# lucabaldesi/srsRAN

Hardware: AMD Instinct MI355X
Metric: PDSCH decoded Mbps + code-blocks/sec, 20 MHz TM4 QAM256, 1/2/4/8 GPU (higher is better)
Workload: dtype fp32+int16; 1 GPU; srslte_ue_dl chain from time-domain I/Q: 2048 subframes/GPU/batch, 20 MHz (100 PRB), TM4 2x2 spatial multiplexing, 2 codewords QAM256 TBS 97896 (C=16, K=6144), MMSE+CSI, max 10 half-its with CRC early stop, 40 dB crossed 2x2 channel, every subframe distinct (GPU eNodeB generator, keyed by global subframe index); 3 PHY worker threads (own ue_dl / stream / softbuffers each) decode alternate batches,; subframes_per_gpu_batch=2048, code_blocks_per_gpu_batch=65536, workers_per_gpu=3, parallelism=dp1

## Files before the change

### include/srsran_amd/dlsch.h

```cpp
#ifndef SRSRAN_AMD_DLSCH_H
#define SRSRAN_AMD_DLSCH_H

#include <stddef.h>
#include <stdint.h>

#ifdef __cplusplus
extern "C" {
#endif

typedef struct mi355_softbuffer_pool mi355_softbuffer_pool_t;

int  mi355_softbuffer_pool_create(mi355_softbuffer_pool_t** p, uint32_t nof_sb, uint32_t max_cb, int device);
void mi355_softbuffer_pool_destroy(mi355_softbuffer_pool_t* p);
int mi355_softbuffer_reset(mi355_softbuffer_pool_t* p, uint32_t sb, void* stream);
int mi355_softbuffer_reset_tbs(mi355_softbuffer_pool_t* p, uint32_t sb, uint32_t tbs, void* stream);
int mi355_softbuffer_reset_cb(mi355_softbuffer_pool_t* p, uint32_t sb, uint32_t nof_cb, void* stream);
int mi355_softbuffer_reset_all(mi355_softbuffer_pool_t* p, void* stream);
int mi355_softbuffer_reset_range(mi355_softbuffer_pool_t* p, uint32_t first, uint32_t n, void* stream);
int mi355_softbuffer_reset_tbs_batch(mi355_softbuffer_pool_t* p, const uint32_t* sbs, const uint32_t* tbs, uint32_t n,
                                     void* stream);
int mi355_softbuffer_pool_buffer(mi355_softbuffer_pool_t* p, int16_t** buf, uint32_t* stride, uint32_t* max_cb);
int mi355_softbuffer_pool_materialize(mi355_softbuffer_pool_t* p, uint32_t first, uint32_t n, void* stream);

int mi355_softbuffer_pool_data(mi355_softbuffer_pool_t* p, uint8_t** data, uint32_t* stride, uint32_t* nof_sb);
int mi355_softbuffer_get_cb_crc(mi355_softbuffer_pool_t* p, uint32_t sb, uint8_t* cb_crc, void* stream);
int mi355_softbuffer_get_cb_crc_async(mi355_softbuffer_pool_t* p, uint32_t sb, uint8_t* cb_crc, void* stream);
int mi355_softbuffer_cb_crc_dev(mi355_softbuffer_pool_t* p, uint32_t sb, const uint8_t** d_cb_crc);
typedef struct {
  uint32_t tbs;
  uint32_t nof_e_bits;
  uint32_t Qm;
  uint32_t rv;
  uint32_t softbuffer;
  uint64_t e_offset;
  uint64_t data_offset;
} mi355_dlsch_tb_t;

typedef struct mi355_dlsch mi355_dlsch_t;

int  mi355_dlsch_create(mi355_dlsch_t** q, int device);
void mi355_dlsch_destroy(mi355_dlsch_t* q);
int mi355_dlsch_set_max_iterations(mi355_dlsch_t* q, uint32_t max_iterations);
void mi355_dlsch_set_profiling(mi355_dlsch_t* q, int enable);

int mi355_dlsch_set_latency_path(int max_cbs);
int mi355_dlsch_latency_profile(int enable, uint64_t* out);
int  mi355_dlsch_kernel_stats(mi355_dlsch_t* q, double* ms, uint32_t* launches);

int mi355_dlsch_decode_dev(mi355_dlsch_t*           q,
                           mi355_softbuffer_pool_t* pool,
                           const int16_t*           d_e_bits,
                           const mi355_dlsch_tb_t*  tbs,
                           uint32_t                 ntb,
                           uint8_t*                 d_data,
                           int32_t*                 ret,
                           float*                   avg_iterations,
                           void*                    stream);

int mi355_dlsch_decode8_dev(mi355_dlsch_t* q, mi355_softbuffer_pool_t* pool, const int8_t* d_e_bits,
                            const mi355_dlsch_tb_t* tbs, uint32_t ntb, uint8_t* d_data, int32_t* ret,
                            float* avg_iterations, void* stream);

#ifdef __cplusplus
}
#endif
#endif
```

### srsran_amd/csrc/dlsch_internal.h

```cpp
#pragma once
#include <hip/hip_runtime.h>
#include <stdint.h>

#define SB_STRIDE 18600
#define SB_DATA 768
#define SB_CONV8 10240
#define SB_ROWMASK 18544
#define SB_ROWMASK_WORDS 12

namespace mi355 {

struct CbDesc {
  uint32_t tb, cb, C;
  uint32_t rlen;
  uint32_t rp, n_e;
  uint32_t rv;
  uint32_t slot;
  uint64_t e_off;
  uint64_t data_off;
};

struct TbDesc {
  uint32_t tbs, C, C1, K1, K2, slot0, invalid;
  uint32_t Qm, nof_e_bits, rv;
  uint32_t cb_base[2];
  uint64_t e_off;
  uint64_t data_off;
  const uint32_t* crc_scale;
};

struct CrcTable {
  uint32_t t[256];
  uint32_t pw[24];
  uint32_t poly;
};

CrcTable make_crc_table(uint32_t poly);

constexpr uint16_t RM_NONE = 0xffff;

struct DlschRmArgs {
  const CbDesc*   desc;
  int             ncb;
  uint32_t        N;
  uint32_t        buflen;
  const uint16_t* inv[4];
  const int16_t*  e;
  int16_t*        sb;
  size_t          sb_stride;
  const uint8_t*  sb_crc;
  uint8_t*        fresh;
  uint32_t        fold2;
  int             sparse;
};

struct DlschRm8Args {
  const CbDesc*   desc;
  int             ncb;
  uint32_t        N, buflen;
  const uint16_t* inv[4];
  const int8_t*   e;
  int8_t*         sb;
  size_t          sb_stride;
  const uint8_t*  sb_crc;
  const uint8_t*  fresh;
  int16_t*        conv;
};

struct DlschCheckArgs {
  const CbDesc*  desc;
  int            ncb;
  uint32_t       K, h, max_its;
  const uint8_t* dec;
  size_t         dec_stride;
  uint8_t*       data;
  uint8_t*       done;
  const uint32_t* remaining;
  uint32_t*      next;
  uint32_t*      its;
  uint8_t*        sb_crc;
  const CrcTable* crc24a;
  const CrcTable* crc24b;
  const uint32_t* scale;
};

struct DlschTbArgs {
  const TbDesc* tb;
  int           ntb;
  uint8_t*      data;
  uint8_t*      sb_crc;
  uint8_t*      sb_data;
  int32_t*        ret;
  const CrcTable* crc24a;
  CbDesc*   desc;
  uint32_t* slot;
  uint32_t* its;
  uint8_t*  done;
  uint32_t* running;
  float*    avg;
};

struct DlschResetArgs {
  uint8_t* fresh;
  uint8_t* sb_crc;
  size_t   slot0, ncb;
  size_t   ncrc;
};

hipError_t dlsch_launch_rm(const DlschRmArgs& a, hipStream_t s);
hipError_t dlsch_launch_reset_list(const uint2* list, uint32_t n, uint32_t max_cb, uint8_t* fresh, uint8_t* cb_crc,
                                   hipStream_t s);
hipError_t dlsch_launch_check(const DlschCheckArgs& a, hipStream_t s);
hipError_t dlsch_launch_prologue(const DlschTbArgs& a, hipStream_t s);
hipError_t dlsch_launch_epilogue(const DlschTbArgs& a, hipStream_t s);
hipError_t dlsch_launch_reset(const DlschResetArgs& a, hipStream_t s);

hipError_t dlsch_launch_rm8(const DlschRm8Args& a, hipStream_t s);
hipError_t dlsch_launch_materialize(int16_t* sb, size_t stride, const uint8_t* fresh, size_t slot0, uint32_t nslots,
                                    hipStream_t s);

}
```

### srsran_amd/csrc/dlsch_kernels.hip

```cpp
#include <hip/hip_runtime.h>
#include <stdint.h>

#include "crc_device.h"
#include "dlsch_internal.h"
#include "rm_image.h"

namespace mi355 {

constexpr uint32_t RM_LDS     = 3 * 6144 + 12;
constexpr uint32_t RM_THREADS = 512;
constexpr int      RM_Q       = (3 * (6144 + 32) + 12 + 8 * RM_THREADS - 1) / (8 * RM_THREADS);
constexpr int      RM_EQ      = (RM_LDS + 8 * RM_THREADS - 1) / (8 * RM_THREADS);
#ifndef RM_CPB_N
#define RM_CPB_N 1
#endif
constexpr int      RM_CPB     = RM_CPB_N;

__device__ __forceinline__ uint32_t add_pairs(uint32_t a, uint32_t b)
{
  return ((a + b) & 0xffffu) | (((a >> 16) + (b >> 16)) << 16);
}

__device__ __forceinline__ uint4 ld_quad(const uint32_t* p, uint32_t q, uint32_t lim, bool al16, uint32_t fill)
{
  const uint32_t i = 4 * q;
  if (al16 && i + 3 < lim) return *(const uint4*)(p + i);
  return make_uint4(i < lim ? p[i] : fill, i + 1 < lim ? p[i + 1] : fill, i + 2 < lim ? p[i + 2] : fill,
                    i + 3 < lim ? p[i + 3] : fill);
}

__device__ __forceinline__ uint32_t ld_llr_pair(const int16_t* e, uint32_t r2, bool al4)
{
  return al4 ? ((const uint32_t*)e)[r2] : ((uint32_t)(uint16_t)e[2 * r2] | ((uint32_t)(uint16_t)e[2 * r2 + 1] << 16));
}

__global__ __launch_bounds__(RM_THREADS) void dlsch_rm_rx(DlschRmArgs a)
{
  extern __shared__ __attribute__((aligned(16))) uint32_t acc32[];
  const uint16_t* acc   = (const uint16_t*)acc32;
  __shared__ uint32_t obm[2 * SB_ROWMASK_WORDS], nbm[2 * SB_ROWMASK_WORDS];
  const uint32_t  N     = a.N, tid = threadIdx.x, N2 = min(N / 2, a.fold2), K = (N - 12) / 3;
  const uint32_t  pairs = a.buflen / 2;
  uint4           iv[RM_Q];
  uint32_t        iv_rv = 0xffffffffu;
  for (int c = 0; c < RM_CPB; c++) {
    const int b = blockIdx.x * RM_CPB + c;
    if (b >= a.ncb) break;
    const CbDesc& d = a.desc[b];
    if (a.sb_crc[d.slot]) continue;
    const uint32_t n_e = d.n_e, first2 = min(n_e, N) / 2;
    const bool     fresh = a.fresh[d.slot] != 0;
    uint32_t*      sb    = (uint32_t*)(a.sb + (size_t)d.slot * a.sb_stride);
    const bool     sb16  = ((uintptr_t)sb & 15) == 0;
    const int16_t* e     = a.e + d.e_off + d.rp;
    const bool     e4    = ((uintptr_t)e & 3) == 0, e16 = ((uintptr_t)e & 15) == 0;
    if (d.rv != iv_rv) {
      const uint32_t* inv32 = (const uint32_t*)a.inv[d.rv];
#pragma unroll
      for (int k = 0; k < RM_Q; k++) iv[k] = ld_quad(inv32, tid + k * RM_THREADS, pairs, true, 0xffffffffu);
      iv_rv = d.rv;
    }
    uint4 old[RM_Q], ev[RM_EQ];
#pragma unroll
    for (int k = 0; k < RM_EQ; k++) {
      const uint32_t q = tid + k * RM_THREADS;
      if (e16) {
        ev[k] = ld_quad((const uint32_t*)e, q, first2, true, 0u);
      } else {
        ev[k] = make_uint4(4 * q < first2 ? ld_llr_pair(e, 4 * q, e4) : 0u,
                           4 * q + 1 < first2 ? ld_llr_pair(e, 4 * q + 1, e4) : 0u,
                           4 * q + 2 < first2 ? ld_llr_pair(e, 4 * q + 2, e4) : 0u,
                           4 * q + 3 < first2 ? ld_llr_pair(e, 4 * q + 3, e4) : 0u);
      }
    }
#pragma unroll
    for (int k = 0; k < RM_Q; k++)
      old[k] = fresh ? make_uint4(0u, 0u, 0u, 0u) : ld_quad(sb, tid + k * RM_THREADS, pairs, sb16, 0u);
    __syncthreads();
    if (tid < 2 * SB_ROWMASK_WORDS) {
      uint32_t*      bmg = rm_rowmask_of(a.sb + (size_t)d.slot * a.sb_stride);
      const uint32_t nw  = rm_rowmask_word(a.inv[d.rv], a.buflen, fresh ? min(n_e, N) : 0x10000u, tid);
      obm[tid]           = fresh ? 0xffffffffu : bmg[tid];
      nbm[tid]           = nw;
      bmg[tid]           = nw;
    } else if (tid == 2 * SB_ROWMASK_WORDS) {
      rm_rowmask_of(a.sb + (size_t)d.slot * a.sb_stride)[tid] = K;
    }
#pragma unroll
    for (int k = 0; k < RM_EQ; k++) {
      const uint32_t i = 4 * (tid + k * RM_THREADS);
      if (i + 3 < N2) {
        *(uint4*)&acc32[img_u32(i)] = ev[k];
      } else {
        if (i < N2) acc32[img_u32(i)] = ev[k].x;
        if (i + 1 < N2) acc32[img_u32(i + 1)] = ev[k].y;
        if (i + 2 < N2) acc32[img_u32(i + 2)] = ev[k].z;
      }
    }
    for (uint32_t base = N; base < n_e; base += N) {
      __syncthreads();
      const uint32_t lim2 = min(N, n_e - base) / 2;
      for (uint32_t r2 = tid; r2 < lim2; r2 += RM_THREADS)
        acc32[img_u32(r2)] = add_pairs(acc32[img_u32(r2)], ld_llr_pair(e + base, r2, e4));
    }
    __syncthreads();
#pragma unroll
    for (int k = 0; k < RM_Q; k++) {
      const uint32_t q = tid + k * RM_THREADS, i = 4 * q;
      if (i >= pairs) continue;
      if (fresh && a.sparse && !rm_quad_defined(nbm, 2 * i, K)) continue;
      const bool     odef = fresh || rm_quad_defined(obm, 2 * i, K);
      const uint32_t w[4] = {iv[k].x, iv[k].y, iv[k].z, iv[k].w};
      const uint32_t o[4] = {odef ? old[k].x : 0u, odef ? old[k].y : 0u, odef ? old[k].z : 0u, odef ? old[k].w : 0u};
      uint32_t       v[4];
      bool           any = fresh || !odef;
#pragma unroll
      for (int cc = 0; cc < 4; cc++) {
        const uint32_t r0 = w[cc] & 0xffffu, r1 = w[cc] >> 16;
        const bool     h0 = r0 != RM_NONE && r0 < n_e, h1 = r1 != RM_NONE && r1 < n_e;
        any |= h0 || h1;
        v[cc] = add_pairs(o[cc], (h0 ? acc[img_i16(r0)] : 0u) | ((h1 ? acc[img_i16(r1)] : 0u) << 16));
      }
      if (!any) continue;
      if (sb16 && i + 3 < pairs) {
        typedef uint32_t u4v __attribute__((ext_vector_type(4)));
        __builtin_nontemporal_store((u4v){v[0], v[1], v[2], v[3]}, (u4v*)(sb + i));
      } else {
#pragma unroll
        for (int cc = 0; cc < 4; cc++)
          if (i + cc < pairs) sb[i + cc] = v[cc];
      }
    }
  }
}

__global__ __launch_bounds__(256) void dlsch_rm_consume(const CbDesc* desc, int ncb, uint8_t* fresh, const uint8_t* sb_crc)
{
  const int b = blockIdx.x * blockDim.x + threadIdx.x;
  if (b < ncb && !sb_crc[desc[b].slot]) fresh[desc[b].slot] = 0;
}


__global__ __launch_bounds__(1024) void dlsch_cb_check(DlschCheckArgs a)
{
  __shared__ uint32_t unfinished;
  __shared__ uint32_t tl[2][4][256];
  if (threadIdx.x == 0) unfinished = 0;
  if (a.ncb && *a.remaining == 0) return;
  const uint32_t ti = threadIdx.x & 255, tt = (threadIdx.x >> 8) & 1;
  if (threadIdx.x < 512) tl[tt][0][ti] = (tt ? a.crc24b : a.crc24a)->t[ti];
  __syncthreads();
#pragma unroll
  for (int k = 1; k < 4; k++) {
    if (threadIdx.x < 512) tl[tt][k][ti] = crc24_step_table(tl[tt][k - 1][ti], tl[tt][0]);
    __syncthreads();
  }
  const int b    = (blockIdx.x * blockDim.x + threadIdx.x) >> 6;
  const int lane = threadIdx.x & 63;
  if (b < a.ncb && *a.remaining != 0 && !a.done[b]) {
    const CbDesc&  d   = a.desc[b];
    const uint8_t* dec = a.dec + (size_t)b * a.dec_stride;
    const uint32_t crc = wave_crc24_scaled4(dec, a.K / 8, tl[d.C > 1 ? 1 : 0], d.C > 1 ? a.crc24b->poly : a.crc24a->poly,
                                            a.scale + (d.C > 1 ? 64 : 0));
    const bool     ok  = crc == 0;
    const bool     fin = ok || a.h + 1 == a.max_its;
    if (!fin) {
      if (lane == 0) unfinished = 1;
    } else {
      uint8_t*       dst = a.data + d.data_off + (size_t)d.cb * d.rlen / 8;
      const uint32_t nb  = (d.cb + 1 == d.C) ? a.K / 8 : d.rlen / 8;
      for (uint32_t i = lane; i < nb; i += 64) dst[i] = dec[i];
      if (lane == 0) {
        a.its[b] = a.h + 1;
        if (ok) {
          a.done[b]        = 1;
          a.sb_crc[d.slot] = 1;
        } else {
          a.done[b] = 2;
        }
      }
    }
  }
  __syncthreads();
  if (threadIdx.x == 0 && unfinished) flag_set(a.next);
}


__global__ __launch_bounds__(256) void dlsch_tb_prologue(DlschTbArgs a)
{
  __shared__ uint32_t todo_any;
  if (threadIdx.x == 0) todo_any = 0;
  __syncthreads();
  const int t    = (blockIdx.x * blockDim.x + threadIdx.x) >> 6;
  const int lane = threadIdx.x & 63;
  if (t < a.ntb && a.tb[t].C != 0) {
    const TbDesc&  tb    = a.tb[t];
    const uint32_t Gp    = tb.nof_e_bits / tb.Qm, gamma = Gp % tb.C, n_e = tb.Qm * (Gp / tb.C);
    uint8_t*       data  = a.data + tb.data_off;
    bool           todo  = false;
    if (lane < 3) data[tb.tbs / 8 + lane] = 0;
    for (uint32_t c = lane; c < tb.C; c += 64) {
      const uint32_t K    = c < tb.C1 ? tb.K1 : tb.K2;
      const uint32_t rlen = tb.C == 1 ? K : K - 24;
      uint32_t       rp = c * n_e, n_e2 = n_e;
      if (c > tb.C - gamma) {
        n_e2 = n_e + tb.Qm;
        rp   = (tb.C - gamma) * n_e + (c - (tb.C - gamma)) * n_e2;
      }
      const uint32_t g    = c < tb.C1 ? tb.cb_base[0] + c : tb.cb_base[1] + (c - tb.C1);
      const uint32_t slot = tb.slot0 + c;
      a.desc[g]           = CbDesc{(uint32_t)t, c, tb.C, rlen, rp, n_e2, tb.rv, slot, tb.e_off, tb.data_off};
      a.slot[g]           = slot;
      a.its[g]            = 0;
      const bool prior    = a.sb_crc[slot] != 0;
      a.done[g]           = prior ? 3 : 0;
      todo |= !prior;
    }
    if (todo) todo_any = 1;
    for (uint32_t c = 0; c < tb.C; c++) {
      const uint32_t slot = tb.slot0 + c;
      if (!a.sb_crc[slot]) continue;
      const uint32_t K    = c < tb.C1 ? tb.K1 : tb.K2;
      const uint32_t rlen = tb.C == 1 ? K : K - 24;
      const uint32_t o    = c * rlen / 8;
      for (uint32_t i = lane; i < rlen / 8; i += 64) data[o + i] = a.sb_data[(size_t)slot * 768 + i];
    }
  }
  __syncthreads();
  if (threadIdx.x == 0 && todo_any) flag_set(a.running);
}

__global__ __launch_bounds__(256) void dlsch_tb_epilogue(DlschTbArgs a)
{
  const int t   = blockIdx.x;
  const int tid = threadIdx.x;
  if (t >= a.ntb) return;
  __shared__ uint32_t t4[4][256];
  t4[0][tid] = a.crc24a->t[tid];
  __syncthreads();
  const TbDesc& tb = a.tb[t];
  if (tb.crc_scale) {
#pragma unroll
    for (int k = 1; k < 4; k++) {
      t4[k][tid] = crc24_step_table(t4[k - 1][tid], t4[0]);
      __syncthreads();
    }
  }
  if (tid == 0) {
    double sum = 0.0;
    for (uint32_t c = 0; c < tb.C; c++) sum += a.its[c < tb.C1 ? tb.cb_base[0] + c : tb.cb_base[1] + (c - tb.C1)];
    a.avg[t] = tb.C ? (float)(sum / tb.C) : 0.f;
  }
  if (tb.C == 0) {
    if (tid == 0) a.ret[t] = tb.invalid ? -2 : 0;
    return;
  }
  bool ok = true;
  for (uint32_t c = 0; c < tb.C; c++) ok &= a.sb_crc[tb.slot0 + c] != 0;
  uint8_t* data = a.data + tb.data_off;
  if (!ok) {
    for (uint32_t c = 0; c < tb.C; c++) {
      const uint32_t slot = tb.slot0 + c;
      if (!a.sb_crc[slot]) continue;
      const uint32_t K    = c < tb.C1 ? tb.K1 : tb.K2;
      const uint32_t rlen = tb.C == 1 ? K : K - 24;
      for (uint32_t i = tid; i < rlen / 8; i += blockDim.x) a.sb_data[(size_t)slot * 768 + i] = data[c * rlen / 8 + i];
    }
    if (tid == 0) a.ret[t] = -1;
    return;
  }
  const uint32_t par_rx = tb.crc_scale ? block_crc24_scaled4(data, tb.tbs / 8, t4, a.crc24a->poly, tb.crc_scale)
                                        : block_crc24(data, tb.tbs / 8, t4[0], *a.crc24a);
  if (tid == 0) {
    const uint32_t par_tx = ((uint32_t)data[tb.tbs / 8] << 16) | ((uint32_t)data[tb.tbs / 8 + 1] << 8) |
                            (uint32_t)data[tb.tbs / 8 + 2];
    a.ret[t] = (par_rx == par_tx && par_rx) ? 0 : -1;
  }
}

__global__ __launch_bounds__(256) void dlsch_sb_reset(DlschResetArgs a)
{
  const size_t g = (size_t)blockIdx.x * blockDim.x + threadIdx.x;
  if (g < a.ncb) a.fresh[a.slot0 + g] = 1;
  if (g < (a.ncrc ? a.ncrc : a.ncb)) a.sb_crc[a.slot0 + g] = 0;
}

__global__ __launch_bounds__(256) void dlsch_sb_reset_list(const uint2* list, uint32_t n, uint32_t max_cb, uint8_t* fresh,
                                                           uint8_t* cb_crc)
{
  const size_t g = (size_t)blockIdx.x * blockDim.x + threadIdx.x;
  if (g >= (size_t)n * max_cb) return;
  const uint2    e  = list[g / max_cb];
  const uint32_t cb = (uint32_t)(g % max_cb);
  const size_t   k  = (size_t)e.x * max_cb + cb;
  if (cb < e.y) fresh[k] = 1;
  cb_crc[k] = 0;
}

hipError_t dlsch_launch_reset_list(const uint2* list, uint32_t n, uint32_t max_cb, uint8_t* fresh, uint8_t* cb_crc,
                                   hipStream_t s)
{
  const size_t t = (size_t)n * max_cb;
  if (!t) return hipSuccess;
  hipLaunchKernelGGL(dlsch_sb_reset_list, dim3((unsigned)((t + 255) / 256)), dim3(256), 0, s, list, n, max_cb, fresh,
                     cb_crc);
  return hipGetLastError();
}

__global__ __launch_bounds__(256) void dlsch_rm8_rx(DlschRm8Args a)
{
  const size_t t = (size_t)blockIdx.x * blockDim.x + threadIdx.x;
  if (t >= (size_t)a.ncb * a.buflen) return;
  const uint32_t b = (uint32_t)(t / a.buflen), j = (uint32_t)(t % a.buflen);
  const CbDesc&  d = a.desc[b];
  if (a.sb_crc[d.slot]) return;
  int8_t*        o = a.sb + (size_t)d.slot * a.sb_stride;
  const uint16_t r = a.inv[d.rv][j];
  int            v = a.fresh[d.slot] ? 0 : o[j];
  if (r != RM_NONE) {
    const int8_t* e = a.e + d.e_off + d.rp;
    for (uint32_t i = r; i < d.n_e; i += a.N) v += e[i];
  }
  o[j] = (int8_t)v;
  if (a.conv) a.conv[(size_t)d.slot * (a.sb_stride / 2) + j] = (int16_t)(int8_t)v;
  if (j < 2 * SB_ROWMASK_WORDS) ((uint32_t*)(a.sb + (size_t)d.slot * a.sb_stride + 2 * SB_ROWMASK))[j] = 0xffffffffu;
}

__global__ __launch_bounds__(256) void sb_materialize(int16_t* sb, size_t stride, const uint8_t* fresh, size_t slot0)
{
  const size_t slot = slot0 + blockIdx.x;
  if (fresh[slot]) return;
  int16_t*        b  = sb + slot * stride;
  uint32_t*       bm = rm_rowmask_of(b);
  const uint32_t  K  = bm[2 * SB_ROWMASK_WORDS];
  __shared__ uint32_t w[2 * SB_ROWMASK_WORDS];
  if (threadIdx.x < 2 * SB_ROWMASK_WORDS) w[threadIdx.x] = bm[threadIdx.x];
  __syncthreads();
  if (K % 16 == 0 && K > 800 && K <= 6144) {
    const uint32_t L = K / 16;
    for (uint32_t r = threadIdx.x; r < 2 * L; r += blockDim.x) {
      const uint32_t s = r / L, j = r % L;
      if ((w[s * SB_ROWMASK_WORDS + (j >> 5)] >> (j & 31)) & 1u) continue;
      uint4* row = (uint4*)(b + (s + 1) * (K + 32) + 16 * j);
      row[0] = row[1] = make_uint4(0u, 0u, 0u, 0u);
    }
  }
  __syncthreads();
  if (threadIdx.x < 2 * SB_ROWMASK_WORDS) bm[threadIdx.x] = 0xffffffffu;
}

hipError_t dlsch_launch_materialize(int16_t* sb, size_t stride, const uint8_t* fresh, size_t slot0, uint32_t nslots,
                                    hipStream_t s)
{
  if (!nslots) return hipSuccess;
  hipLaunchKernelGGL(sb_materialize, dim3(nslots), dim3(256), 0, s, sb, stride, fresh, slot0);
  return hipGetLastError();
}

hipError_t dlsch_launch_rm8(const DlschRm8Args& a, hipStream_t s)
{
  if (a.ncb <= 0) return hipSuccess;
  const size_t n = (size_t)a.ncb * a.buflen;
  hipLaunchKernelGGL(dlsch_rm8_rx, dim3((unsigned)((n + 255) / 256)), dim3(256), 0, s, a);
  hipLaunchKernelGGL(dlsch_rm_consume, dim3((unsigned)((a.ncb + 255) / 256)), dim3(256), 0, s, a.desc, a.ncb,
                     (uint8_t*)a.fresh, a.sb_crc);
  return hipGetLastError();
}

hipError_t dlsch_launch_rm(const DlschRmArgs& a, hipStream_t s)
{
  if (a.ncb <= 0) return hipSuccess;
  if (a.N > RM_LDS) return hipErrorInvalidValue;
  DlschRmArgs b = a;
  b.fold2       = (a.fold2 && a.fold2 < a.N / 2) ? a.fold2 : a.N / 2;
  const size_t lds = (size_t)img_elems(2 * ((b.fold2 + 3) & ~3u)) * 2;
  hipLaunchKernelGGL(dlsch_rm_rx, dim3((unsigned)((a.ncb + RM_CPB - 1) / RM_CPB)), dim3(RM_THREADS), lds, s, b);
  hipLaunchKernelGGL(dlsch_rm_consume, dim3((unsigned)((a.ncb + 255) / 256)), dim3(256), 0, s, a.desc, a.ncb, a.fresh,
                     a.sb_crc);
  return hipGetLastError();
}

hipError_t dlsch_launch_check(const DlschCheckArgs& a, hipStream_t s)
{
  hipLaunchKernelGGL(dlsch_cb_check, dim3((unsigned)((a.ncb + 15) / 16)), dim3(1024), 0, s, a);
  return hipGetLastError();
}

hipError_t dlsch_launch_prologue(const DlschTbArgs& a, hipStream_t s)
{
  hipLaunchKernelGGL(dlsch_tb_prologue, dim3((unsigned)((a.ntb + 3) / 4)), dim3(256), 0, s, a);
  return hipGetLastError();
}

hipError_t dlsch_launch_epilogue(const DlschTbArgs& a, hipStream_t s)
{
  if (a.ntb <= 0) return hipSuccess;
  hipLaunchKernelGGL(dlsch_tb_epilogue, dim3((unsigned)a.ntb), dim3(256), 0, s, a);
  return hipGetLastError();
}

hipError_t dlsch_launch_reset(const DlschResetArgs& a, hipStream_t s)
{
  const size_t n = a.ncb > a.ncrc ? a.ncb : a.ncrc;
  if (!n) return hipSuccess;
  hipLaunchKernelGGL(dlsch_sb_reset, dim3((unsigned)((n + 255) / 256)), dim3(256), 0, s, a);
  return hipGetLastError();
}

}
```

### srsran_amd/csrc/dlsch_runtime.cpp

```cpp
#include <hip/hip_runtime.h>

#include <algorithm>
#include <chrono>
#include <stdlib.h>
#include <map>
#include <mutex>
#include <stdio.h>
#include <string.h>
#include <vector>

#include "../../include/srsran_amd/dlsch.h"
#include "../../include/srsran_amd/tdec.h"
#include "dlsch_internal.h"
#include "host_staging.h"
#include "tdec8_internal.h"
#include "rm_image.h"
#include "rm_tables.h"
#include "runtime_internal.h"
#include "tdec_internal.h"

using namespace mi355;

#define CHECK_HIP(x)                                                                                                   \
  do {                                                                                                                 \
    hipError_t e_ = (x);                                                                                               \
    if (e_ != hipSuccess) {                                                                                            \
      fprintf(stderr, "[srsran_amd] %s:%d %s: %s\n", __FILE__, __LINE__, #x, hipGetErrorString(e_));                 \
      return MI355_ERROR;                                                                                              \
    }                                                                                                                  \
  } while (0)

struct mi355_softbuffer_pool {
  int      device = 0;
  uint32_t nof_sb = 0, max_cb = 0;
  int16_t* buf    = nullptr;
  uint8_t* cb_crc = nullptr;
  uint8_t* data   = nullptr;
  uint8_t* fresh  = nullptr;
  uint2*     d_list[2]   = {nullptr, nullptr};
  uint32_t   list_cap[2] = {0, 0};
  hipEvent_t ev_list[2]  = {nullptr, nullptr};
  bool       ev_armed[2] = {false, false};
  uint32_t   lpar        = 0;
  mi355::HostStaging st_list;
};

CrcTable mi355::make_crc_table(uint32_t poly)
{
  CrcTable t{};
  t.poly = poly;
  for (uint32_t i = 0; i < 256; i++) {
    uint32_t c = i << 16;
    for (int j = 0; j < 8; j++) c = (c & 0x800000) ? ((c << 1) ^ poly) & 0xffffff : (c << 1) & 0xffffff;
    t.t[i] = c;
  }
  auto mulmod = [&](uint32_t a, uint32_t b) {
    uint32_t r = 0;
    for (int i = 23; i >= 0; i--) {
      r <<= 1;
      if (r & 0x1000000u) r ^= poly;
      if ((b >> i) & 1u) r ^= a;
    }
    return r & 0xffffffu;
  };
  uint32_t p = 1u << 8;
  for (int i = 0; i < 24; i++) {
    t.pw[i] = p;
    p       = mulmod(p, p);
  }
  return t;
}

struct mi355_dlsch {
  int                                    device = 0;
  hipStream_t                            own    = nullptr;
  uint32_t                               max_its = 10;
  std::map<uint32_t, mi355_tdec_batch_t*> dec;
  std::map<uint64_t, uint16_t*>          rm;
  std::map<uint64_t, uint16_t*>          rm8;
  struct Compact {
    uint16_t* d;
    uint32_t  nq, qoff;
  };
  std::map<uint64_t, Compact>            rmc;
  std::map<uint32_t, mi355_tdec8_t*>     dec8;
  std::map<uint32_t, uint32_t*>          scales;
  std::map<uint32_t, uint32_t*>          tb_scales;
  CrcTable*                              crc = nullptr;
  char*      scratch[2]     = {nullptr, nullptr};
  size_t     scratch_cap[2] = {0, 0};
  std::vector<void*> retired;
  hipEvent_t done_ev[2]     = {nullptr, nullptr};
  bool       done_armed[2]  = {false, false};
  uint32_t   par            = 0;
  std::mutex mu;
  bool       prof = false;
  HostStaging stage;
  HostStaging back;
  std::atomic<uint32_t> spec_mask{1u << 1};
};

static std::atomic<int> g_lat_cbs{-1};
static std::atomic<uint64_t*> g_lat_prof{nullptr};
static uint64_t*              g_lat_prof_mem = nullptr;
static std::mutex             g_lat_prof_mu;
static int lat_cbs_now()
{
  int v = g_lat_cbs.load();
  if (v < 0) {
    v = getenv("MI355_DLSCH_LAT_CBS") ? atoi(getenv("MI355_DLSCH_LAT_CBS")) : 256;
    g_lat_cbs.store(v);
  }
  return v;
}

extern "C" int mi355_dlsch_latency_profile(int enable, uint64_t* out)
{
  std::lock_guard<std::mutex> lk(g_lat_prof_mu);
  if (out && g_lat_prof.load()) {
    if (hipDeviceSynchronize() != hipSuccess) return MI355_ERROR;
    if (hipMemcpy(out, g_lat_prof_mem, 11 * 8, hipMemcpyDeviceToHost) != hipSuccess) return MI355_ERROR;
  }
  if (enable) {
    if (!g_lat_prof_mem && hipMalloc(&g_lat_prof_mem, 11 * 8) != hipSuccess) return MI355_ERROR;
    if (hipMemset(g_lat_prof_mem, 0, 11 * 8) != hipSuccess || hipDeviceSynchronize() != hipSuccess) return MI355_ERROR;
    g_lat_prof.store(g_lat_prof_mem);
  } else {
    g_lat_prof.store(nullptr);
  }
  return MI355_SUCCESS;
}

extern "C" int mi355_dlsch_set_latency_path(int max_cbs)
{
  const int old = lat_cbs_now();
  if (max_cbs >= 0) g_lat_cbs.store(max_cbs);
  return old;
}

static bool spec_enabled()
{
  static const bool on = !getenv("MI355_TDEC_SPEC") || atoi(getenv("MI355_TDEC_SPEC")) != 0;
  return on;
}

static bool no_rowmask()
{
  static const bool off = getenv("MI355_NO_ROWMASK") && atoi(getenv("MI355_NO_ROWMASK")) != 0;
  return off;
}

static bool lat_waves4()
{
  static const bool on = getenv("MI355_LAT_WAVES") && atoi(getenv("MI355_LAT_WAVES")) == 4;
  return on;
}
static bool lat_owaves()
{
  static const bool on = !getenv("MI355_LAT_OWAVES") || atoi(getenv("MI355_LAT_OWAVES")) != 0;
  return on;
}

bool mi355::rm_sparse_writes()
{
  static const bool on = !getenv("MI355_RM_SPARSE") || atoi(getenv("MI355_RM_SPARSE")) != 0;
  return on && !no_rowmask();
}

static uint32_t rm_buflen(uint32_t K) { return tdec_subblocks(K) ? 3 * (K + 32) + 12 : 3 * K + 12; }

static int rm_table(mi355_dlsch_t* q, uint32_t K, uint32_t rv, const uint16_t** out)
{
  const uint64_t key = ((uint64_t)K << 2) | rv;
  auto           it  = q->rm.find(key);
  if (it == q->rm.end()) {
    const std::vector<uint16_t> t = rm_rx_table(K, rv);
    const uint32_t              buflen = rm_buflen(K);
    std::vector<uint16_t>       inv(rm_rowmin_off(buflen) + rm_rowmin_len(), 0);
    std::fill(inv.begin(), inv.begin() + buflen + 1, (uint16_t)RM_NONE);
    for (size_t r = 0; r < t.size(); r++) inv[t[r]] = (uint16_t)r;
    if (tdec_subblocks(K) == 16) {
      uint16_t*      rmin = inv.data() + rm_rowmin_off(buflen);
      const uint32_t L    = K / 16;
      for (uint32_t s = 0; s < 2; s++)
        for (uint32_t j = 0; j < L; j++) {
          uint16_t m = RM_NONE;
          for (uint32_t w = 0; w < 16; w++) m = std::min(m, inv[(s + 1) * (K + 32) + j * 16 + w]);
          rmin[s * 32 * SB_ROWMASK_WORDS + j] = m;
        }
    }
    uint16_t* d = nullptr;
    CHECK_HIP(hipMalloc(&d, inv.size() * 2));
    CHECK_HIP(hipMemcpy(d, inv.data(), inv.size() * 2, hipMemcpyHostToDevice));
    it = q->rm.emplace(key, d).first;
  }
  *out = it->second;
  return MI355_SUCCESS;
}

static int rm8_table(mi355_dlsch_t* q, uint32_t K, uint32_t rv, const uint16_t** out)
{
  const uint64_t key = ((uint64_t)K << 2) | rv;
  auto           it  = q->rm8.find(key);
  if (it == q->rm8.end()) {
    const uint32_t              nsb = tdec_subblocks_8bit(K);
    const std::vector<uint16_t> t   = rm_rx_table_nsb(K, rv, nsb);
    std::vector<uint16_t>       inv((nsb ? 3 * (K + 32) + 12 : 3 * K + 12) + 1, RM_NONE);
    for (size_t r = 0; r < t.size(); r++) inv[t[r]] = (uint16_t)r;
    uint16_t* d = nullptr;
    CHECK_HIP(hipMalloc(&d, inv.size() * 2));
    CHECK_HIP(hipMemcpy(d, inv.data(), inv.size() * 2, hipMemcpyHostToDevice));
    it = q->rm8.emplace(key, d).first;
  }
  *out = it->second;
  return MI355_SUCCESS;
}

static uint32_t gf2_mulmod24_host(uint32_t a, uint32_t b, uint32_t poly)
{
  uint32_t r = 0;
  for (int i = 23; i >= 0; i--) {
    r <<= 1;
    if (r & 0x1000000u) r ^= poly;
    if ((b >> i) & 1u) r ^= a;
  }
  return r & 0xffffffu;
}

static int crc_scales(mi355_dlsch_t* q, uint32_t K, const uint32_t** out)
{
  auto it = q->scales.find(K);
  if (it == q->scales.end()) {
    std::vector<uint32_t> t(144, 0u);
    const uint32_t        nbytes = K / 8, chunk = (nbytes + 63) / 64;
    const uint32_t        polys[2] = {0x1864CFB, 0x1800063};
    auto                  xpow = [](uint32_t after, uint32_t poly) {
      uint32_t sc = 1, x8 = 1u << 8;
      for (; after; after >>= 1) {
        if (after & 1) sc = gf2_mulmod24_host(sc, x8, poly);
        x8 = gf2_mulmod24_host(x8, x8, poly);
      }
      return sc;
    };
    const uint32_t nl = std::max(1u, mi355_tdec_autoimp_get_subblocks(K) / 2), cl = nbytes / nl;
    for (int pi = 0; pi < 2; pi++) {
      for (uint32_t lane = 0; lane < 64; lane++) {
        const uint32_t b0 = std::min(nbytes, lane * chunk), b1 = std::min(nbytes, b0 + chunk);
        t[pi * 64 + lane] = xpow(nbytes - b1, polys[pi]);
      }
      for (uint32_t l = 0; l < nl && l < 8; l++) t[128 + 8 * pi + l] = xpow(nbytes - (l + 1) * cl, polys[pi]);
    }
    uint32_t* d = nullptr;
    CHECK_HIP(hipMalloc(&d, t.size() * 4));
    CHECK_HIP(hipMemcpy(d, t.data(), t.size() * 4, hipMemcpyHostToDevice));
    it = q->scales.emplace(K, d).first;
  }
  *out = it->second;
  return MI355_SUCCESS;
}

static int tb_crc_scales(mi355_dlsch_t* q, uint32_t nbytes, const uint32_t** out)
{
  auto it = q->tb_scales.find(nbytes);
  if (it == q->tb_scales.end()) {
    std::vector<uint32_t> t(256);
    const uint32_t        chunk = ((nbytes + 255) / 256 + 3) / 4 * 4, poly = 0x1864CFB;
    for (uint32_t tid = 0; tid < 256; tid++) {
      const uint32_t b0 = std::min(nbytes, tid * chunk), b1 = std::min(nbytes, b0 + chunk);
      uint32_t       sc = 1, x8 = 1u << 8;
      for (uint32_t after = nbytes - b1; after; after >>= 1) {
        if (after & 1) sc = gf2_mulmod24_host(sc, x8, poly);
        x8 = gf2_mulmod24_host(x8, x8, poly);
      }
      t[tid] = sc;
    }
    uint32_t* d = nullptr;
    CHECK_HIP(hipMalloc(&d, t.size() * 4));
    CHECK_HIP(hipMemcpy(d, t.data(), t.size() * 4, hipMemcpyHostToDevice));
    it = q->tb_scales.emplace(nbytes, d).first;
  }
  *out = it->second;
  return MI355_SUCCESS;
}

static int scratch(mi355_dlsch_t* q, uint32_t k, size_t bytes, char** p)
{
  if (bytes > q->scratch_cap[k]) {
    if (q->scratch[k]) {
      q->retired.push_back(q->scratch[k]);
      q->scratch[k]    = nullptr;
      q->done_armed[k] = false;
    }
    size_t cap = bytes + bytes / 4 + 4096;
    CHECK_HIP(hipMalloc(&q->scratch[k], cap));
    q->scratch_cap[k] = cap;
  }
  *p = q->scratch[k];
  return MI355_SUCCESS;
}

extern "C" {

int mi355_softbuffer_pool_create(mi355_softbuffer_pool_t** p, uint32_t nof_sb, uint32_t max_cb, int device)
{
  if (!p || !nof_sb || !max_cb) return MI355_ERROR_INVALID_INPUTS;
  CHECK_HIP(hipSetDevice(device));
  auto*        s  = new mi355_softbuffer_pool;
  const size_t nc = (size_t)nof_sb * max_cb;
  s->device       = device;
  s->nof_sb       = nof_sb;
  s->max_cb       = max_cb;
  if (hipMalloc(&s->buf, nc * SB_STRIDE * 2) != hipSuccess || hipMalloc(&s->cb_crc, nc) != hipSuccess ||
      hipMalloc(&s->data, nc * SB_DATA) != hipSuccess || hipMalloc(&s->fresh, nc) != hipSuccess) {
    mi355_softbuffer_pool_destroy(s);
    return MI355_ERROR;
  }
  (void)hipMemset(s->fresh, 1, nc);
  (void)hipMemset(s->cb_crc, 0, nc);
  (void)hipMemset(s->data, 0, nc * SB_DATA);
  (void)hipDeviceSynchronize();
  *p = s;
  return MI355_SUCCESS;
}

void mi355_softbuffer_pool_destroy(mi355_softbuffer_pool_t* p)
{
  if (!p) return;
  (void)hipFree(p->buf);
  (void)hipFree(p->cb_crc);
  (void)hipFree(p->data);
  (void)hipFree(p->fresh);
  for (int k = 0; k < 2; k++) {
    if (p->ev_armed[k]) (void)hipEventSynchronize(p->ev_list[k]);
    if (p->ev_list[k]) (void)hipEventDestroy(p->ev_list[k]);
    (void)hipFree(p->d_list[k]);
  }
  delete p;
}

int mi355_softbuffer_reset_cb(mi355_softbuffer_pool_t* p, uint32_t sb, uint32_t nof_cb, void* stream)
{
  if (!p || sb >= p->nof_sb) return MI355_ERROR_INVALID_INPUTS;
  CHECK_HIP(hipSetDevice(p->device));
  hipStream_t    s  = (hipStream_t)stream;
  const uint32_t nc = std::min(nof_cb, p->max_cb);
  DlschResetArgs a{p->fresh, p->cb_crc, (size_t)sb * p->max_cb, nc, p->max_cb};
  CHECK_HIP(dlsch_launch_reset(a, s));
  if (!s) CHECK_HIP(hipStreamSynchronize(nullptr));
  return MI355_SUCCESS;
}

int mi355_softbuffer_reset(mi355_softbuffer_pool_t* p, uint32_t sb, void* stream)
{
  return mi355_softbuffer_reset_cb(p, sb, p ? p->max_cb : 0, stream);
}

int mi355_softbuffer_reset_tbs(mi355_softbuffer_pool_t* p, uint32_t sb, uint32_t tbs, void* stream)
{
  return mi355_softbuffer_reset_cb(p, sb, (tbs + 24) / (6144 - 24) + 1, stream);
}

int mi355_softbuffer_reset_tbs_batch(mi355_softbuffer_pool_t* p, const uint32_t* sbs, const uint32_t* tbs, uint32_t n,
                                     void* stream)
{
  if (!p || (n && (!sbs || !tbs))) return MI355_ERROR_INVALID_INPUTS;
  if (!n) return MI355_SUCCESS;
  CHECK_HIP(hipSetDevice(p->device));
  hipStream_t    s = (hipStream_t)stream;
  const uint32_t k = p->lpar;
  p->lpar ^= 1u;
  if (n > p->list_cap[k]) {
    if (p->d_list[k]) {
      if (p->ev_armed[k]) CHECK_HIP(hipEventSynchronize(p->ev_list[k]));
      CHECK_HIP(hipFree(p->d_list[k]));
      p->ev_armed[k] = false;
    }
    p->list_cap[k] = n + n / 2 + 64;
    CHECK_HIP(hipMalloc(&p->d_list[k], p->list_cap[k] * sizeof(uint2)));
  }
  if (!p->ev_list[k]) CHECK_HIP(hipEventCreateWithFlags(&p->ev_list[k], hipEventDisableTiming));
  CHECK_HIP(p->st_list.reserve(n * sizeof(uint2)));
  auto* l = (uint2*)p->st_list.slot(n * sizeof(uint2));
  for (uint32_t i = 0; i < n; i++) {
    if (sbs[i] >= p->nof_sb) return MI355_ERROR_INVALID_INPUTS;
    l[i] = make_uint2(sbs[i], std::min((tbs[i] + 24) / (6144 - 24) + 1, p->max_cb));
  }
  CHECK_HIP(p->st_list.upload(p->d_list[k], s, false, p->ev_armed[k] ? p->ev_list[k] : nullptr));
  CHECK_HIP(dlsch_launch_reset_list(p->d_list[k], n, p->max_cb, p->fresh, p->cb_crc, s));
  CHECK_HIP(hipEventRecord(p->ev_list[k], s));
  p->ev_armed[k] = true;
  if (!s) CHECK_HIP(hipStreamSynchronize(nullptr));
  return MI355_SUCCESS;
}

int mi355_softbuffer_reset_all(mi355_softbuffer_pool_t* p, void* stream)
{
  if (!p) return MI355_ERROR_INVALID_INPUTS;
  for (uint32_t i = 0; i < p->nof_sb; i++) {
    int r = mi355_softbuffer_reset(p, i, stream);
    if (r) return r;
  }
  return MI355_SUCCESS;
}

int mi355_softbuffer_reset_range(mi355_softbuffer_pool_t* p, uint32_t first, uint32_t n, void* stream)
{
  if (!p || first + n > p->nof_sb) return MI355_ERROR_INVALID_INPUTS;
  if (!n) return MI355_SUCCESS;
  CHECK_HIP(hipSetDevice(p->device));
  DlschResetArgs a{p->fresh, p->cb_crc, (size_t)first * p->max_cb, (size_t)n * p->max_cb, 0};
  CHECK_HIP(dlsch_launch_reset(a, (hipStream_t)stream));
  if (!stream) CHECK_HIP(hipStreamSynchronize(nullptr));
  return MI355_SUCCESS;
}

int mi355_softbuffer_pool_buffer(mi355_softbuffer_pool_t* p, int16_t** buf, uint32_t* stride, uint32_t* max_cb)
{
  if (!p) return MI355_ERROR_INVALID_INPUTS;
  if (buf) *buf = p->buf;
  if (stride) *stride = SB_STRIDE;
  if (max_cb) *max_cb = p->max_cb;
  return MI355_SUCCESS;
}

int mi355_softbuffer_pool_materialize(mi355_softbuffer_pool_t* p, uint32_t first, uint32_t n, void* stream)
{
  if (!p || first > p->nof_sb || n > p->nof_sb - first) return MI355_ERROR_INVALID_INPUTS;
  CHECK_HIP(hipSetDevice(p->device));
  CHECK_HIP(dlsch_launch_materialize(p->buf, SB_STRIDE, p->fresh, (size_t)first * p->max_cb, n * p->max_cb,
                                     (hipStream_t)stream));
  if (!stream) CHECK_HIP(hipStreamSynchronize(nullptr));
  return MI355_SUCCESS;
}

int mi355_softbuffer_pool_data(mi355_softbuffer_pool_t* p, uint8_t** data, uint32_t* stride, uint32_t* nof_sb)
{
  if (!p) return MI355_ERROR_INVALID_INPUTS;
  if (data) *data = p->data;
  if (stride) *stride = SB_DATA;
  if (nof_sb) *nof_sb = p->nof_sb;
  return MI355_SUCCESS;
}

int mi355_softbuffer_get_cb_crc(mi355_softbuffer_pool_t* p, uint32_t sb, uint8_t* cb_crc, void* stream)
{
  if (!p || !cb_crc || sb >= p->nof_sb) return MI355_ERROR_INVALID_INPUTS;
  CHECK_HIP(hipSetDevice(p->device));
  hipStream_t s = (hipStream_t)stream;
  CHECK_HIP(hipMemcpyAsync(cb_crc, p->cb_crc + (size_t)sb * p->max_cb, p->max_cb, hipMemcpyDeviceToHost, s));
  CHECK_HIP(wait_stream(s));
  return MI355_SUCCESS;
}

int mi355_softbuffer_get_cb_crc_async(mi355_softbuffer_pool_t* p, uint32_t sb, uint8_t* cb_crc, void* stream)
{
  if (!p || !cb_crc || sb >= p->nof_sb) return MI355_ERROR_INVALID_INPUTS;
  CHECK_HIP(hipSetDevice(p->device));
  CHECK_HIP(hipMemcpyAsync(cb_crc, p->cb_crc + (size_t)sb * p->max_cb, p->max_cb, hipMemcpyDeviceToHost,
                           (hipStream_t)stream));
  return MI355_SUCCESS;
}

int mi355_softbuffer_cb_crc_dev(mi355_softbuffer_pool_t* p, uint32_t sb, const uint8_t** d_cb_crc)
{
  if (!p || !d_cb_crc || sb >= p->nof_sb) return MI355_ERROR_INVALID_INPUTS;
  *d_cb_crc = p->cb_crc + (size_t)sb * p->max_cb;
  return MI355_SUCCESS;
}

int mi355_dlsch_create(mi355_dlsch_t** q, int device)
{
  if (!q) return MI355_ERROR_INVALID_INPUTS;
  CHECK_HIP(hipSetDevice(device));
  auto* d   = new mi355_dlsch;
  d->device = device;
  if (hipStreamCreateWithFlags(&d->own, hipStreamNonBlocking) != hipSuccess ||
      hipMalloc(&d->crc, 2 * sizeof(CrcTable)) != hipSuccess) {
    mi355_dlsch_destroy(d);
    return MI355_ERROR;
  }
  const CrcTable t[2] = {make_crc_table(0x1864CFB), make_crc_table(0x1800063)};
  if (hipMemcpy(d->crc, t, sizeof(t), hipMemcpyHostToDevice) != hipSuccess) {
    mi355_dlsch_destroy(d);
    return MI355_ERROR;
  }
  *q = d;
  return MI355_SUCCESS;
}

void mi355_dlsch_destroy(mi355_dlsch_t* q)
{
  if (!q) return;
  (void)hipSetDevice(q->device);
  (void)hipDeviceSynchronize();
  for (auto& kv : q->dec) mi355_tdec_batch_destroy(kv.second);
  for (auto& kv : q->rm) (void)hipFree(kv.second);
  for (auto& kv : q->rm8) (void)hipFree(kv.second);
  for (auto& kv : q->rmc) (void)hipFree(kv.second.d);
  for (auto& kv : q->dec8) mi355_tdec8_destroy(kv.second);
  for (auto& kv : q->scales) (void)hipFree(kv.second);
  for (auto& kv : q->tb_scales) (void)hipFree(kv.second);
  (void)hipFree(q->crc);
  for (void* r : q->retired) (void)hipFree(r);
  for (int k = 0; k < 2; k++) {
    (void)hipFree(q->scratch[k]);
    if (q->done_ev[k]) (void)hipEventDestroy(q->done_ev[k]);
  }
  if (q->own) (void)hipStreamDestroy(q->own);
  delete q;
}

int mi355_dlsch_set_max_iterations(mi355_dlsch_t* q, uint32_t max_iterations)
{
  if (!q || max_iterations == 0) return MI355_ERROR_INVALID_INPUTS;
  q->max_its = max_iterations;
  return MI355_SUCCESS;
}

void mi355_dlsch_set_profiling(mi355_dlsch_t* q, int enable)
{
  if (!q) return;
  q->prof = enable != 0;
  for (auto& kv : q->dec) mi355_tdec_batch_set_profiling(kv.second, enable);
}

int mi355_dlsch_kernel_stats(mi355_dlsch_t* q, double* ms, uint32_t* launches)
{
  if (!q) return MI355_ERROR_INVALID_INPUTS;
  double   tot = 0;
  uint32_t n   = 0;
  for (auto& kv : q->dec) {
    double   m = 0;
    uint32_t l = 0;
    int      r = mi355_tdec_batch_kernel_stats(kv.second, &m, &l);
    if (r) return r;
    tot += m;
    n += l;
  }
  if (ms) *ms = tot;
  if (launches) *launches = n;
  return MI355_SUCCESS;
}

int mi355_dlsch_decode_dev(mi355_dlsch_t*           q,
                           mi355_softbuffer_pool_t* pool,
                           const int16_t*           d_e_bits,
                           const mi355_dlsch_tb_t*  tbs,
                           uint32_t                 ntb,
                           uint8_t*                 d_data,
                           int32_t*                 ret,
                           float*                   avg_iterations,
                           void*                    stream)
{
  return mi355::dlsch_decode_dev_hook(q, pool, d_e_bits, tbs, ntb, d_data, ret, avg_iterations, stream, mi355::WaitHook{});
}

int mi355_dlsch_decode8_dev(mi355_dlsch_t* q, mi355_softbuffer_pool_t* pool, const int8_t* d_e_bits,
                            const mi355_dlsch_tb_t* tbs, uint32_t ntb, uint8_t* d_data, int32_t* ret,
                            float* avg_iterations, void* stream)
{
  return mi355::dlsch_decode_dev_hook(q, pool, d_e_bits, tbs, ntb, d_data, ret, avg_iterations, stream,
                                      mi355::WaitHook{}, true);
}

}

mi355::DlschPending::~DlschPending()
{
  if (armed && ev) (void)hipEventSynchronize(ev);
  if (ev) (void)hipEventDestroy(ev);
  if (host) (void)hipHostFree(host);
}

static uint32_t spec_policy(const float* avg, const int32_t* ret, uint32_t ntb, uint32_t max_its)
{
  uint32_t mask = 0;
  for (uint32_t h = 0; h + 1 < max_its; h++) {
    uint32_t run = 0, fail = 0;
    for (uint32_t t = 0; t < ntb; t++) {
      if (ret[t] != MI355_SUCCESS && ret[t] != MI355_ERROR) continue;
      const float a = avg[t];
      if (!(a > 0.f)) continue;
      run += a > (float)h + 0.5f;
      fail += a > (float)h + 1.5f;
    }
    if (run && fail * 10 <= run) mask |= 1u << h;
  }
  return mask;
}

int mi355::DlschPending::collect()
{
  if (!armed) return MI355_SUCCESS;
  armed = false;
  CHECK_HIP(wait_event(ev));
  memcpy(ret, host, ntb * 4);
  for (uint32_t t = 0; t < ntb; t++) {
    if (invalid[t]) ret[t] = MI355_ERROR_INVALID_INPUTS;
  }
  if (avg) memcpy(avg, host + avg_off, ntb * 4);
  if (spec_mask) spec_mask->store(spec_policy((const float*)(host + avg_off), ret, ntb, max_its));
  return MI355_SUCCESS;
}

int mi355::dlsch_rm_inv(mi355_dlsch_t* q, uint32_t K, uint32_t rv, const uint16_t** out)
{
  if (!q || rv > 3) return MI355_ERROR_INVALID_INPUTS;
  std::lock_guard<std::mutex> lock(q->mu);
  CHECK_HIP(hipSetDevice(q->device));
  return rm_table(q, K, rv, out);
}

uint32_t mi355::dlsch_rm_buflen(uint32_t K) { return rm_buflen(K); }

int mi355::dlsch_rm_compact(mi355_dlsch_t* q, uint32_t K, uint32_t rv, uint32_t E, const uint16_t** tab, uint32_t* nq,
                            uint32_t* qoff)
{
  if (!q || rv > 3 || E == 0 || E > 3 * K + 12) return MI355_ERROR_INVALID_INPUTS;
  std::lock_guard<std::mutex> lock(q->mu);
  CHECK_HIP(hipSetDevice(q->device));
  const uint64_t key = ((((uint64_t)K << 2) | rv) << 16) | E;
  auto           it  = q->rmc.find(key);
  if (it == q->rmc.end()) {
    const std::vector<uint16_t> t      = rm_rx_table(K, rv);
    const uint32_t              buflen = rm_buflen(K), nquad = (buflen + 7) / 8;
    std::vector<uint16_t>       inv(buflen, (uint16_t)RM_NONE);
    for (size_t r = 0; r < t.size(); r++) inv[t[r]] = (uint16_t)r;
    auto defined = [&](uint32_t pos) {
      if (tdec_subblocks(K) != 16) return true;
      const uint32_t sl = K + 32, s = pos / sl;
      if (s == 0 || s > 2) return true;
      const uint32_t j = (pos - s * sl) >> 4;
      if (j >= 32 * SB_ROWMASK_WORDS || j >= K / 16) return true;
      for (uint32_t w = 0; w < 16; w++)
        if (inv[s * sl + j * 16 + w] < E) return true;
      return false;
    };
    std::vector<uint16_t> rank(nquad, 0xffff);
    std::vector<uint32_t> qlist;
    for (uint32_t qd = 0; qd < nquad; qd++) {
      if (!defined(8 * qd)) continue;
      uint32_t m = 0;
      for (uint32_t p = 0; p < 8 && 8 * qd + p < buflen; p++) m |= (uint32_t)(inv[8 * qd + p] < E) << p;
      rank[qd] = (uint16_t)qlist.size();
      qlist.push_back(qd | m << 16);
    }
    const uint32_t        off = (E + 7) / 8 * 8;
    std::vector<uint16_t> all(off + 2 * qlist.size() + 8, 0);
    for (uint32_t r = 0; r < E; r++) {
      const uint32_t pos = t[r];
      if (rank[pos / 8] == 0xffff) return MI355_ERROR;
      all[r] = (uint16_t)(8 * rank[pos / 8] + pos % 8);
    }
    memcpy(all.data() + off, qlist.data(), qlist.size() * 4);
    uint16_t* d = nullptr;
    CHECK_HIP(hipMalloc(&d, all.size() * 2));
    CHECK_HIP(hipMemcpy(d, all.data(), all.size() * 2, hipMemcpyHostToDevice));
    CHECK_HIP(hipStreamSynchronize(nullptr));
    it = q->rmc.emplace(key, mi355_dlsch::Compact{d, (uint32_t)qlist.size(), off}).first;
  }
  *tab  = it->second.d;
  *nq   = it->second.nq;
  *qoff = it->second.qoff;
  return MI355_SUCCESS;
}

mi355::SoftbufferView mi355::softbuffer_view(mi355_softbuffer_pool_t* p)
{
  return SoftbufferView{p->buf, SB_STRIDE, p->cb_crc, p->fresh, p->nof_sb, p->max_cb};
}

int mi355::dlsch_decode_dev_hook(mi355_dlsch_t* q, mi355_softbuffer_pool_t* pool, const void* d_e_bits,
                                 const mi355_dlsch_tb_t* tbs, uint32_t ntb, uint8_t* d_data, int32_t* ret,
                                 float* avg_iterations, void* stream, mi355::WaitHook hook, bool llr8,
                                 mi355::DlschPending* pend, bool after_s, bool rm_done)
{
  if (!q || !pool || !tbs || !ret || (ntb && !d_e_bits)) return MI355_ERROR_INVALID_INPUTS;
  if (ntb == 0) return MI355_SUCCESS;
  std::lock_guard<std::mutex> lock(q->mu);
  static const bool prof = getenv("MI355_HOST_PROF") != nullptr;
  auto              now  = [] { return std::chrono::steady_clock::now(); };
  const auto        t0   = now();
  CHECK_HIP(hipSetDevice(q->device));
  hipStream_t s = stream ? (hipStream_t)stream : q->own;

  std::vector<TbDesc>                        tbd(ntb);
  std::vector<std::pair<uint32_t, uint32_t>> kcount;
  std::vector<uint32_t>                      rvmask;
  std::vector<uint32_t>                      fold2;
  auto group_of = [&](uint32_t K) {
    for (uint32_t i = 0; i < kcount.size(); i++)
      if (kcount[i].first == K) return i;
    kcount.push_back({K, 0u});
    rvmask.push_back(0u);
    return (uint32_t)kcount.size() - 1;
  };
  std::vector<uint8_t> grp(2 * ntb, 0);
  uint32_t             seg_tbs = UINT32_MAX;
  CbSegm               seg{};
  int                  seg_err = 0;
  for (uint32_t t = 0; t < ntb; t++) {
    const mi355_dlsch_tb_t& in = tbs[t];
    TbDesc&                 d  = tbd[t];
    d                          = TbDesc{};
    d.tbs                      = in.tbs;
    d.data_off                 = in.data_offset;
    if (in.tbs != seg_tbs) {
      seg_err = cbsegm(in.tbs, &seg);
      seg_tbs = in.tbs;
    }
    if (in.softbuffer >= pool->nof_sb || in.rv > 3 || in.Qm == 0 || seg_err) {
      d.invalid = 1;
      continue;
    }
    if (in.tbs == 0 || seg.C == 0) continue;
    if (seg.F || seg.C > pool->max_cb) {
      d.invalid = 1;
      continue;
    }
    auto ok8 = [](uint32_t K) { return tdec_subblocks_8bit(K) >= 16 || K <= 400; };
    if (llr8 && ((seg.C1 && !ok8(seg.K1)) || (seg.C > seg.C1 && !ok8(seg.K2)))) {
      d.invalid = 1;
      continue;
    }
    if (int e = tb_crc_scales(q, in.tbs / 8, &d.crc_scale)) return e;
    d.C          = seg.C;
    d.C1         = seg.C1;
    d.K1         = seg.K1;
    d.K2         = seg.K2;
    d.slot0      = in.softbuffer * pool->max_cb;
    d.Qm         = in.Qm;
    d.nof_e_bits = in.nof_e_bits;
    d.rv         = in.rv;
    d.e_off      = in.e_offset;
    const uint32_t emax = in.Qm * (in.nof_e_bits / in.Qm / seg.C + 1);
    auto           fold = [&](uint32_t g, uint32_t K) {
      if (fold2.size() <= g) fold2.resize(g + 1, 0);
      fold2[g] = std::max(fold2[g], std::min(emax, 3 * K + 12) / 2);
    };
    if (seg.C1) {
      const uint32_t g = group_of(seg.K1);
      grp[2 * t]       = (uint8_t)g;
      d.cb_base[0]     = kcount[g].second;
      kcount[g].second += seg.C1;
      rvmask[g] |= 1u << in.rv;
      fold(g, seg.K1);
    }
    if (seg.C > seg.C1) {
      const uint32_t g = group_of(seg.K2);
      grp[2 * t + 1]   = (uint8_t)g;
      d.cb_base[1]     = kcount[g].second;
      kcount[g].second += seg.C - seg.C1;
      rvmask[g] |= 1u << in.rv;
      fold(g, seg.K2);
    }
  }
  std::vector<uint32_t> goff(kcount.size());
  size_t                total_cb = 0, dec_bytes = 0;
  for (size_t g = 0; g < kcount.size(); g++) {
    goff[g] = (uint32_t)total_cb;
    total_cb += kcount[g].second;
    dec_bytes += (size_t)kcount[g].second * (kcount[g].first / 8);
  }
  for (uint32_t t = 0; t < ntb; t++) {
    if (!tbd[t].C) continue;
    tbd[t].cb_base[0] += goff[grp[2 * t]];
    tbd[t].cb_base[1] += goff[grp[2 * t + 1]];
  }

  auto rnd = [](size_t b) { return (b + 255) / 256 * 256; };
  const size_t need = rnd(ntb * sizeof(TbDesc)) + rnd(4 * (q->max_its + 1)) + rnd(total_cb * sizeof(CbDesc)) +
                      3 * rnd(total_cb * 4) + rnd(total_cb) + rnd(dec_bytes) + 2 * rnd(ntb * 4);
  const uint32_t slot = q->par;
  q->par ^= 1u;
  char* base = nullptr;
  int   r    = scratch(q, slot, need, &base);
  if (r) return r;
  char* p     = base;
  auto  carve = [&](size_t b) {
    char* c = p;
    p += rnd(b);
    return c;
  };
  auto*        d_tb    = (TbDesc*)carve(ntb * sizeof(TbDesc));
  auto*        d_run   = (uint32_t*)carve(4 * (q->max_its + 1));
  const size_t staged  = (size_t)(p - base);
  auto*        d_cb    = (CbDesc*)carve(total_cb * sizeof(CbDesc));
  auto*        d_slot  = (uint32_t*)carve(total_cb * 4);
  auto*        d_its   = (uint32_t*)carve(total_cb * 4);
  auto*        d_done  = (uint8_t*)carve(total_cb);
  auto*        d_dec   = (uint8_t*)carve(dec_bytes);
  auto*        d_ret   = (int32_t*)carve(ntb * 4);
  auto*        d_avg   = (float*)carve(ntb * 4);

  CHECK_HIP(q->stage.reserve(staged));
  q->stage.put(tbd.data(), ntb * sizeof(TbDesc));
  q->stage.zeros(4 * (q->max_its + 1));
  CHECK_HIP(q->stage.upload(base, s, false, after_s && q->done_armed[slot] ? q->done_ev[slot] : nullptr));

  DlschTbArgs ta{d_tb,  (int)ntb, d_data, pool->cb_crc, pool->data, d_ret, &q->crc[0],
                 d_cb,  d_slot,   d_its,  d_done,       d_run,      d_avg};
  CHECK_HIP(dlsch_launch_prologue(ta, s));

  struct Live {
    uint32_t            K, off, n;
    uint8_t*            dec;
    mi355_tdec_batch_t* td;
    const uint32_t*     scale;
    mi355_tdec8_t*      t8 = nullptr;
  };
  std::vector<Live> live;
  size_t            off = 0, doff = 0;
  for (size_t gi = 0; gi < kcount.size(); gi++) {
    const uint32_t K = kcount[gi].first, n = kcount[gi].second;
    if (llr8) {
      const uint32_t nsb8 = tdec_subblocks_8bit(K);
      DlschRm8Args   ra{};
      ra.desc   = d_cb + off;
      ra.ncb    = (int)n;
      ra.N      = 3 * K + 12;
      ra.buflen = nsb8 ? 3 * (K + 32) + 12 : 3 * K + 12;
      for (uint32_t rv = 0; rv < 4; rv++) {
        ra.inv[rv] = nullptr;
        if (((rvmask[gi] >> rv) & 1u) && (r = rm8_table(q, K, rv, &ra.inv[rv]))) return r;
      }
      ra.e         = (const int8_t*)d_e_bits;
      ra.sb        = (int8_t*)pool->buf;
      ra.sb_stride = SB_STRIDE * sizeof(int16_t);
      ra.sb_crc    = pool->cb_crc;
      ra.fresh     = pool->fresh;
      ra.conv      = nsb8 ? nullptr : pool->buf + SB_CONV8;
      CHECK_HIP(dlsch_launch_rm8(ra, s));
      const uint32_t* sc = nullptr;
      if ((r = crc_scales(q, K, &sc))) return r;
      mi355_tdec_batch_t* td = nullptr;
      mi355_tdec8_t*      t8 = nullptr;
      if (nsb8) {
        auto it8 = q->dec8.find(K);
        if (it8 == q->dec8.end()) {
          if ((r = mi355_tdec8_create(&t8, q->device))) return r;
          it8 = q->dec8.emplace(K, t8).first;
        }
        t8 = it8->second;
      } else {
        auto it = q->dec.find(K);
        if (it == q->dec.end()) {
          if ((r = mi355_tdec_batch_create(&td, q->device))) return r;
          it = q->dec.emplace(K, td).first;
        }
        td = it->second;
      }
      live.push_back(Live{K, (uint32_t)off, n, d_dec + doff, td, sc, t8});
      off += n;
      doff += (size_t)n * (K / 8);
      continue;
    }
    DlschRmArgs    ra{};
    ra.desc = d_cb + off;
    ra.ncb  = (int)n;
    ra.N      = 3 * K + 12;
    ra.buflen = rm_buflen(K);
    for (uint32_t rv = 0; rv < 4; rv++) {
      ra.inv[rv] = nullptr;
      if (((rvmask[gi] >> rv) & 1u) && (r = rm_table(q, K, rv, &ra.inv[rv]))) return r;
    }
    ra.fresh     = pool->fresh;
    ra.e         = (const int16_t*)d_e_bits;
    ra.sb        = pool->buf;
    ra.sb_stride = SB_STRIDE;
    ra.sb_crc    = pool->cb_crc;
    ra.fold2     = gi < fold2.size() ? fold2[gi] : 0;
    ra.sparse    = rm_sparse_writes() ? 1 : 0;
    if (!rm_done) CHECK_HIP(dlsch_launch_rm(ra, s));
    auto it = q->dec.find(K);
    if (it == q->dec.end()) {
      mi355_tdec_batch_t* td = nullptr;
      if ((r = mi355_tdec_batch_create(&td, q->device))) return r;
      mi355_tdec_batch_set_profiling(td, q->prof);
      it = q->dec.emplace(K, td).first;
    }
    const uint32_t* sc = nullptr;
    if ((r = crc_scales(q, K, &sc))) return r;
    live.push_back(Live{K, (uint32_t)off, n, d_dec + doff, it->second, sc, nullptr});
    off += n;
    doff += (size_t)n * (K / 8);
  }

  std::vector<char> lat(live.size(), 0);
  if (!llr8 && total_cb <= (size_t)lat_cbs_now()) {
    for (size_t i = 0; i < live.size(); i++) {
      Live&          lv  = live[i];
      const uint32_t nsb = mi355_tdec_autoimp_get_subblocks(lv.K);
      if (lv.t8 || nsb == 0 || tdec_lat_lds((int)lv.K, (int)nsb) > 160 * 1024 - 64) continue;
      TdecLatArgs la{};
      la.in        = pool->buf;
      la.in_stride = SB_STRIDE;
      la.in_idx    = d_slot + lv.off;
      if ((r = mi355_tdec_win_tables(lv.td, lv.K, &la.dstE, &la.dstA))) return r;
      la.done    = d_done + lv.off;
      la.chk     = DlschCheckArgs{d_cb + lv.off, (int)lv.n, lv.K, 0, q->max_its, lv.dec, lv.K / 8, d_data, d_done + lv.off,
                              d_run, d_run + 1, d_its + lv.off, pool->cb_crc, &q->crc[0], &q->crc[1], lv.scale};
      la.prof    = g_lat_prof.load();
      la.ncb     = (int)lv.n;
      la.K       = (int)lv.K;
      la.rowmask = nsb == 16 && !no_rowmask();
      la.bwave   = lat_waves4() ? 2 : 1;
      la.owaves  = la.bwave == 1 && lat_owaves() ? 1 : 0;
      CHECK_HIP(tdec_lat_launch((int)nsb, la, s));
      lat[i] = 1;
    }
  }
  const uint32_t spec_mask = spec_enabled() ? q->spec_mask.load() : 0u;
  for (uint32_t h = 0; h < q->max_its; h++) {
    const bool spec = h + 1 == q->max_its || ((spec_mask >> h) & 1u);
    for (size_t li = 0; li < live.size(); li++) {
      auto& lv = live[li];
      if (lat[li]) continue;
      if (lv.t8) {
        T8Batch b{};
        b.in = (int8_t*)pool->buf, b.in_stride = SB_STRIDE * sizeof(int16_t), b.slot = d_slot + lv.off;
        b.done = d_done + lv.off, b.running = d_run + h, b.K = lv.K, b.ncb = lv.n;
        if ((r = tdec8_halfit_batch(lv.t8, b, h, lv.dec, lv.K / 8, s))) return r;
      }
      DlschCheckArgs ca{d_cb + lv.off, (int)lv.n, lv.K, h, q->max_its, lv.dec, lv.K / 8, d_data,
                        d_done + lv.off, d_run + h, d_run + h + 1, d_its + lv.off, pool->cb_crc, &q->crc[0], &q->crc[1],
                        lv.scale};
      bool fused = false;
      if (!lv.t8) {
        TdecRun rq{llr8 ? pool->buf + SB_CONV8 : pool->buf, SB_STRIDE, d_slot + lv.off, d_done + lv.off, d_run + h, lv.n,
                   lv.K, h, h + 1, lv.dec, lv.K / 8, s, &ca, &fused};
        rq.rowmask = !llr8 && !no_rowmask();
        bool taken = false;
        rq.spec       = spec;
        rq.spec_taken = &taken;
        if ((r = mi355_tdec_run_internal(lv.td, rq))) return r;
        if (!fused) CHECK_HIP(dlsch_launch_check(ca, s));
        if (taken && h + 1 < q->max_its) {
          TdecRun rd = rq;
          rd.remaining  = d_run + h + 1;
          rd.chk        = nullptr;
          rd.chk_fused  = nullptr;
          rd.spec       = false;
          rd.spec_taken = nullptr;
          rd.redo       = true;
          if ((r = mi355_tdec_run_internal(lv.td, rd))) return r;
        }
        continue;
      }
      if (!fused) CHECK_HIP(dlsch_launch_check(ca, s));
    }
  }
  CHECK_HIP(dlsch_launch_epilogue(ta, s));
  if (!q->done_ev[slot]) CHECK_HIP(hipEventCreateWithFlags(&q->done_ev[slot], hipEventDisableTiming));
  CHECK_HIP(hipEventRecord(q->done_ev[slot], s));
  q->done_armed[slot] = true;

  const auto t1 = now();
  if (pend) {
    if (pend->armed) return MI355_ERROR;
    const size_t bytes = rnd(ntb * 4) + ntb * 4;
    if (bytes > pend->cap) {
      if (pend->host) (void)hipHostFree(pend->host);
      pend->host = nullptr;
      pend->cap  = 0;
      CHECK_HIP(stage_host_alloc((void**)&pend->host, bytes + bytes / 2 + 4096));
      pend->cap = bytes + bytes / 2 + 4096;
    }
    if (!pend->ev) CHECK_HIP(hipEventCreateWithFlags(&pend->ev, hipEventDisableTiming));
    CHECK_HIP(stage_copy(pend->host, d_ret, bytes, s));
    CHECK_HIP(hipEventRecord(pend->ev, s));
    pend->invalid.resize(ntb);
    for (uint32_t t = 0; t < ntb; t++) pend->invalid[t] = tbd[t].invalid ? 1 : 0;
    pend->ntb     = ntb;
    pend->avg_off = rnd(ntb * 4);
    pend->ret     = ret;
    pend->avg     = avg_iterations;
    pend->spec_mask = &q->spec_mask;
    pend->max_its   = q->max_its;
    pend->armed   = true;
    return MI355_SUCCESS;
  }
  if (hook.fn) hook.fn(hook.ctx);
  CHECK_HIP(q->back.reserve(rnd(ntb * 4) + ntb * 4));
  CHECK_HIP(stage_copy(q->back.host, d_ret, rnd(ntb * 4) + ntb * 4, s));
  CHECK_HIP(wait_stream(s));
  memcpy(ret, q->back.host, ntb * 4);
  for (uint32_t t = 0; t < ntb; t++) {
    if (tbd[t].invalid) ret[t] = MI355_ERROR_INVALID_INPUTS;
  }
  if (avg_iterations) memcpy(avg_iterations, q->back.host + rnd(ntb * 4), ntb * 4);
  q->spec_mask.store(spec_policy((const float*)(q->back.host + rnd(ntb * 4)), ret, ntb, q->max_its));
  if (prof) {
    auto us = [](auto a, auto b) { return std::chrono::duration<double, std::micro>(b - a).count(); };
    fprintf(stderr, "[mi355 host] dlsch_decode_dev: plan+launch %.1f us, wait+readback %.1f us\n", us(t0, t1), us(t1, now()));
  }
  return MI355_SUCCESS;
}
```

### srsran_amd/csrc/pdsch_internal.h

```cpp
#pragma once
#include <hip/hip_runtime.h>
#include <stdint.h>

namespace mi355 {

constexpr uint32_t EQ_BLOCK_ITEMS = 1024;

constexpr uint32_t PDSCH_GOLD_MAX = 14u * 12u * 110u * 8u;

struct PdschJobDev {
  const float2*   y[2];
  const float2*   h[4][2];
  const uint16_t* map;
  const uint16_t* imap;
  uint32_t        g0;
  float2*         d[2];
  float*          csi[2];
  uint32_t*       cmax;
  uint32_t        cmax_stride;
  uint32_t        nof_re, nof_rx, nof_ports, nof_layers, scheme, cb;
  uint32_t        row;
  uint32_t        row_magic;
  uint32_t        h_invariant;
  uint32_t        rhob_mask;
  float           rhob_inv, scaling, noise;
  const float*    noise_dev;
  uint32_t        units;
  uint32_t                 fused;
  uint32_t                 fused_key;
  const uint16_t*          cols;
  uint32_t                 ncols;
  float4*                  wtab;
  const struct PdschCwDev* cw[2];
};

struct PdschCwDev {
  const float2* d;
  const float*  csi;
  const uint32_t* cmax;
  uint32_t        nparts;
  uint32_t*       cmax_final;
  int16_t*      e;
  const uint32_t* scr;
  uint32_t      nof_re, nof_bits, qm, c_init, csi_enable;
  uint32_t      pairs;
  uint32_t      fused;
  uint32_t      llr8;
  int8_t*       e8;
  float         k8[5];
};

hipError_t pdsch_launch_equalize(const PdschJobDev* jobs, uint32_t njobs, uint32_t max_units, hipStream_t s);
hipError_t pdsch_launch_scr_pack(const uint32_t* c_init, uint32_t* const* dst, uint32_t n, const uint32_t* gold,
                                 uint32_t W, hipStream_t s);
hipError_t pdsch_launch_llr(const PdschCwDev* cws, uint32_t ncw, uint32_t max_pairs, hipStream_t s);
hipError_t pdsch_launch_fused(const PdschJobDev* jobs, uint32_t njobs, uint32_t max_pairs, const uint32_t* keys,
                              uint32_t nkeys, hipStream_t s);

struct EqRmLayer {
  const uint16_t* inv[2];
  uint32_t        N[2];
  uint32_t        buflen[2];
  uint32_t        C1;
  uint32_t        slot0;
};
struct EqRmJob {
  uint32_t  C, Qm, Gp;
  EqRmLayer layer[2];
  const uint16_t* cmp[2][2];
  uint32_t        cnq[2][2], cqoff[2][2];
};
struct EqRmPool {
  int16_t*       sb;
  size_t         sb_stride;
  const uint8_t* sb_crc;
  uint8_t*       fresh;
  int            sparse;
  int            diag = 0;
  unsigned long long* prof = nullptr;
};
hipError_t pdsch_launch_eq_rm(const PdschJobDev* jobs, const EqRmJob* rj, uint32_t njobs, uint32_t max_c, uint32_t img,
                              uint32_t cimg, const uint32_t* keys, uint32_t nkeys, const EqRmPool& pool, hipStream_t s);

}
```

### srsran_amd/csrc/pdsch_kernels.hip

```cpp
#include <hip/hip_runtime.h>

#include <algorithm>
#include <stdint.h>

#include "pdsch_internal.h"
#include "rm_image.h"
#include "xcd.h"

namespace mi355 {

namespace {

struct cf {
  float re, im;
};
__device__ __forceinline__ cf mk(float r, float i) { return cf{r, i}; }
__device__ __forceinline__ cf operator+(cf a, cf b) { return mk(a.re + b.re, a.im + b.im); }
__device__ __forceinline__ cf operator-(cf a, cf b) { return mk(a.re - b.re, a.im - b.im); }
__device__ __forceinline__ cf operator*(cf a, cf b) { return mk(a.re * b.re - a.im * b.im, a.re * b.im + a.im * b.re); }
__device__ __forceinline__ cf operator*(cf a, float s) { return mk(a.re * s, a.im * s); }
__device__ __forceinline__ cf cj(cf a) { return mk(a.re, -a.im); }
__device__ __forceinline__ cf mulj(cf a) { return mk(-a.im, a.re); }
__device__ __forceinline__ float abs2(cf a) { return a.re * a.re + a.im * a.im; }
#define GLB __attribute__((address_space(1)))
// ... 956 lines not shown
#define PDSCH_ER_TPF 0
#endif
constexpr bool     ER_TPF     = PDSCH_ER_TPF;
#ifndef PDSCH_ER_Q
#define PDSCH_ER_Q 5
#endif
constexpr int      ER_Q       = PDSCH_ER_Q;
constexpr int      ER_R       = (3 * (6144 + 32) + 12 + 8 * ER_THREADS * ER_Q - 1) / (8 * ER_THREADS * ER_Q);
constexpr int      ER_Q2      = 3;
constexpr int      ER_R2      = (3 * (6144 + 32) + 12 + 8 * ER_THREADS * ER_Q2 - 1) / (8 * ER_THREADS * ER_Q2);

__device__ __forceinline__ uint4 ldg_u4(const GLB uint32_t* p)
{
  typedef uint32_t v4u __attribute__((ext_vector_type(4)));
  const v4u        v = *(const GLB v4u*)p;
  return make_uint4(v.x, v.y, v.z, v.w);
}

__device__ __forceinline__ uint32_t add_pairs16(uint32_t a, uint32_t b)
{
  return ((a + b) & 0xffffu) | (((a >> 16) + (b >> 16)) << 16);
}

template <int QM> __device__ __forceinline__ void img_put(int16_t* im, uint32_t b, uint32_t n_e, const int16_t (&o)[2 * QM])
{
  auto pk = [&](int k) { return (uint32_t)(uint16_t)o[k] | ((uint32_t)(uint16_t)o[k + 1] << 16); };
  if (b < n_e && b + 2 * QM <= n_e) {
    if constexpr (QM == 8) {
      *(uint4*)&im[img_i16(b)]     = make_uint4(pk(0), pk(2), pk(4), pk(6));
      *(uint4*)&im[img_i16(b + 8)] = make_uint4(pk(8), pk(10), pk(12), pk(14));
      return;
    } else if constexpr (QM == 4) {
      *(uint2*)&im[img_i16(b)]     = make_uint2(pk(0), pk(2));
      *(uint2*)&im[img_i16(b + 4)] = make_uint2(pk(4), pk(6));
      return;
    }
  }
#pragma unroll
  for (int k = 0; k < 2 * QM; k++)
    if (b + k < n_e) im[img_i16(b + k)] = o[k];
}

constexpr int ER_CQ = 4;
struct CmpSlots {
  uint4 v[2];
  bool  whole;
};
template <int QM> __device__ __forceinline__ CmpSlots cmp_slots(const GLB uint16_t* fw, uint32_t b, uint32_t n_e)
{
  CmpSlots s{};
  s.whole = QM == 8 && b < n_e && b + 2 * QM <= n_e;
  if (s.whole) {
    s.v[0] = ldg_u4((const GLB uint32_t*)(fw + b));
    s.v[1] = ldg_u4((const GLB uint32_t*)(fw + b + 8));
  }
  return s;
}
template <int QM>
__device__ __forceinline__ void cmp_put2(uint32_t* im, const GLB uint16_t* fw, const CmpSlots& s, uint32_t b, uint32_t n_e,
                                         const uint32_t (&wd)[2 * QM])
{
  if (s.whole) {
    const uint32_t w[8] = {s.v[0].x, s.v[0].y, s.v[0].z, s.v[0].w, s.v[1].x, s.v[1].y, s.v[1].z, s.v[1].w};
#pragma unroll
    for (int k = 0; k < 2 * QM; k++) im[(w[k >> 1] >> (16 * (k & 1))) & 0xffffu] = wd[k];
    return;
  }
#pragma unroll
  for (int k = 0; k < 2 * QM; k++)
    if (b + k < n_e) im[fw[b + k]] = wd[k];
}

typedef uint16_t u16x2 __attribute__((ext_vector_type(2)));
__device__ __forceinline__ int32_t cvt_trunc(float v)
{
  return fabsf(v) < 2147483648.0f ? (int32_t)v : INT32_MIN;
}
__device__ __forceinline__ void llr2_256qam(uint32_t z, bool csi_on, const float (&csc)[2], uint32_t ns,
                                            const cf (&x)[2][2], const float (&csi)[2][2], uint32_t (&wd)[16])
{
  const float k[4] = {0.f, 0x1.3a261cp-1f, 0x1.3a261cp-2f, 0x1.3a261cp-3f};
#pragma unroll
  for (int e = 0; e < 2; e++) {
    int32_t cv[2] = {0, 0};
    if (csi_on) {
#pragma unroll
      for (int l = 0; l < 2; l++) cv[l] = sat16(x86_cvt_i32(rintf(csi[l][e] * csc[l])));
    }
    float re[2], im[2];
#pragma unroll
    for (int l = 0; l < 2; l++) re[l] = -x[l][e].re, im[l] = -x[l][e].im;
#pragma unroll
    for (int t = 0; t < 4; t++) {
      if (t) {
#pragma unroll
        for (int l = 0; l < 2; l++) re[l] = fabsf(re[l]) - k[t], im[l] = fabsf(im[l]) - k[t];
      }
#pragma unroll
      for (int h = 0; h < 2; h++) {
        const int      b = 8 * e + 2 * t + h;
        const float*   v = h ? im : re;
        uint32_t       w = (uint32_t)e < ns ? __builtin_amdgcn_perm((uint32_t)cvt_trunc(1000.0f * v[1]),
                                                                    (uint32_t)cvt_trunc(1000.0f * v[0]), 0x05040100u)
                                            : 0u;
        const uint32_t m = __mul24((z >> b) & 0x00010001u, 0xffffu);
        w = __builtin_bit_cast(uint32_t, (u16x2)(__builtin_bit_cast(u16x2, w ^ m) - __builtin_bit_cast(u16x2, m)));
        if (csi_on) {
          const int32_t p0 = __mul24((int32_t)(int16_t)(w & 0xffffu), cv[0]);
          const int32_t p1 = __mul24((int32_t)w >> 16, cv[1]);
          w                = __builtin_amdgcn_perm((uint32_t)p1, (uint32_t)p0, 0x07060302u);
        }
        wd[b] = w;
      }
    }
  }
}

template <int QM0, int QM1>
#ifndef PDSCH_ER_WAVES
#define PDSCH_ER_WAVES 5
#endif
__global__ __launch_bounds__(ER_THREADS) __attribute__((amdgpu_waves_per_eu(PDSCH_ER_WAVES, 8))) void pdsch_eq_rm(const PdschJobDev* __restrict__ jobs,
                                                          const EqRmJob* __restrict__ rjobs, uint32_t max_c, uint32_t img,
                                                          EqRmPool P)
{
  extern __shared__ __attribute__((aligned(16))) int16_t imgs[];
  const uint32_t     Lb = xcd_chunk(blockIdx.x, gridDim.x);
  const uint32_t     jn = Lb / max_c, c = Lb % max_c;
  const PdschJobDev& J  = jobs[jn];
  const EqRmJob&     R  = rjobs[jn];
  const uint32_t     tid = threadIdx.x;
  if (!J.fused || J.fused_key != (uint32_t)(QM0 * 16 + QM1) || c >= R.C) return;
  const uint32_t Qm = R.Qm, gamma = R.Gp % R.C, n_e0 = Qm * (R.Gp / R.C);
  uint32_t       rp = c * n_e0, n_e = n_e0;
  if (c > R.C - gamma) {
    n_e = n_e0 + Qm;
    rp  = (R.C - gamma) * n_e0 + (c - (R.C - gamma)) * n_e;
  }
  bool need[2], fresh[2];
  uint32_t slot[2];
#pragma unroll
  for (int l = 0; l < 2; l++) {
    slot[l]  = R.layer[l].slot0 + c;
    need[l]  = J.cw[l] != nullptr && !P.sb_crc[slot[l]];
    fresh[l] = need[l] && P.fresh[slot[l]] != 0;
  }
  if (!need[0] && !need[1]) return;
  const unsigned long long pt0 = P.prof ? clock64() : 0ull;
  const uint32_t      re0 = rp / Qm, re1 = (rp + n_e) / Qm, pairs = (J.nof_re + 1) / 2;
  const uint32_t      p1  = P.diag == 2 ? 0u : min((re1 + 1) / 2, pairs);
  const GLB uint32_t* map2  = (const GLB uint32_t*)gptr(J.map);
  const uint32_t      pb    = re0 / 2 + tid;
  uint32_t            mnext = pb < p1 ? map2[pb] : 0u;
  __shared__ uint32_t obm[2][2 * SB_ROWMASK_WORDS], nbm[2][2 * SB_ROWMASK_WORDS];
  if (tid < 2 * (2 * SB_ROWMASK_WORDS + 1)) {
    const uint32_t l = tid / (2 * SB_ROWMASK_WORDS + 1), w = tid % (2 * SB_ROWMASK_WORDS + 1);
    const uint32_t kx = c < R.layer[l].C1 ? 0u : 1u;
    if (need[l]) {
      uint32_t* bmg = rm_rowmask_of(P.sb + (size_t)slot[l] * P.sb_stride);
      if (w < 2 * SB_ROWMASK_WORDS) {
        const uint32_t nw = rm_rowmask_word(R.layer[l].inv[kx], R.layer[l].buflen[kx], fresh[l] ? n_e : 0x10000u, w);
        obm[l][w] = fresh[l] ? 0xffffffffu : bmg[w];
        nbm[l][w] = nw;
        bmg[w]    = nw;
      } else {
        bmg[w] = (R.layer[l].N[kx] - 12) / 3;
      }
    }
  }
  __shared__ PdschCwDev cwd[2];
  __shared__ uint32_t   cmb[2];
  static_assert(ER_THREADS >= 128 && 2 * (2 * SB_ROWMASK_WORDS + 1) <= 64, "pdsch_eq_rm prologue waves");
  if (tid - 64 < 2 && J.cw[tid - 64]) {
    const uint32_t l = tid - 64;
    cwd[l]           = *J.cw[l];
    cmb[l]           = cwd[l].csi_enable ? *gptr(cwd[l].cmax_final) : 0u;
  }
  __syncthreads();
  const uint32_t kx0 = c < R.layer[0].C1 ? 0u : 1u, kx1 = c < R.layer[1].C1 ? 0u : 1u;
  const bool     lean = need[0] && need[1] && fresh[0] && fresh[1] && R.layer[0].inv[kx0] == R.layer[1].inv[kx1] &&
                    R.layer[0].buflen[kx0] == R.layer[1].buflen[kx1];
  const uint32_t ev = c > R.C - gamma ? 1u : 0u;
  const bool     cm = lean && P.sparse && QM0 == QM1 && R.cmp[kx0][ev] != nullptr;
  const GLB uint16_t* fw  = cm ? gptr(R.cmp[kx0][ev]) : nullptr;
  const uint32_t      cnq = cm ? R.cnq[kx0][ev] : 0u;
  uint32_t* const     im32 = (uint32_t*)imgs;
  const unsigned long long pt1 = P.prof ? clock64() : 0ull;
  const float         noise = J.noise_dev ? *gptr(J.noise_dev) : J.noise;
  const uint32_t      row = J.row, magic = J.row_magic, rmask = J.rhob_mask;
  const float         rinv = J.rhob_inv;
  const GLB float2*   yp[2] = {gptr(J.y[0]), gptr(J.nof_rx > 1 ? J.y[1] : J.y[0])};
  const GLB float2*   hp[4];
  h_ptrs(J, hp);
  const GLB fv4*      wtp = (const GLB fv4*)gptr(J.wtab);
  uint4 iv0[ER_Q];
  if constexpr (ER_TPF) {
    if (lean) {
      const uint32_t  npairs = R.layer[0].buflen[kx0] / 2;
      const GLB uint32_t* inv32 = (const GLB uint32_t*)gptr(R.layer[0].inv[kx0]);
#pragma unroll
      for (int k = 0; k < ER_Q; k++) {
        const uint32_t i = 4 * (tid + k * ER_THREADS);
        iv0[k]           = i + 3 < npairs ? ldg_u4(inv32 + i)
                                          : make_uint4(i < npairs ? inv32[i] : 0xffffffffu,
                                                       i + 1 < npairs ? inv32[i + 1] : 0xffffffffu,
                                                       i + 2 < npairs ? inv32[i + 2] : 0xffffffffu, 0xffffffffu);
      }
    }
  }
  constexpr bool WT = PDSCH_WTAB && QM0 != 0 && QM1 != 0;
  constexpr bool L2 = PDSCH_LLR2 && QM0 == 8 && QM1 == 8;
  bool                l2 = false, l2csi = false;
  float               csc[2] = {0.f, 0.f};
  const GLB uint32_t* scr[2] = {nullptr, nullptr};
  if constexpr (L2) {
    l2 = cm && cwd[0].csi_enable == cwd[1].csi_enable;
    if (l2) {
      l2csi = cwd[0].csi_enable != 0;
#pragma unroll
      for (int l = 0; l < 2; l++) {
        scr[l]           = gptr(cwd[l].scr);
        const float cmax = cwd[l].nof_bits / 8 ? __uint_as_float(cmb[l]) : 1.0f;
        csc[l]           = 32767.0f / cmax;
      }
    }
  }
  for (uint32_t pr = pb; pr < p1; pr += ER_THREADS) {
    const uint32_t m = mnext;
    cf             Y[2][2], H[2][WT ? 1 : 4];
    fv4            W[2][WT ? 2 : 1];
    fv2            WC[2];
#pragma unroll
    for (int e = 0; e < 2; e++) {
      const uint32_t g  = e ? (m >> 16) : (m & 0xffffu);
      const uint32_t gc = g < 14 * row ? g : 0u;
      const uint32_t l  = __umulhi(gc, magic);
      const float    sc = ((rmask >> l) & 1u) ? rinv : 1.0f;
#pragma unroll
      for (int r = 0; r < 2; r++) Y[e][r] = ld(yp[r], gc) * sc;
      if constexpr (WT) {
        const GLB fv4* wt = wtp + 3 * (gc - l * row);
        W[e][0]           = wt[0];
        W[e][1]           = wt[1];
        WC[e]             = *(const GLB fv2*)(wt + 2);
      } else {
#pragma unroll
        for (int q = 0; q < 4; q++) H[e][q] = ld(hp[q], gc - l * row);
      }
    }
    if (pr + ER_THREADS < p1) mnext = map2[pr + ER_THREADS];
    const uint32_t ns = min(2u, J.nof_re - 2 * pr);
    CmpSlots       fws[1];
    if (cm) fws[0] = cmp_slots<(QM0 ? QM0 : QM1)>(fw, 2 * pr * (QM0 ? QM0 : QM1) - rp, n_e);
    uint32_t lo[2] = {0u, 0u};
    if constexpr (L2) {
      if (l2) {
#pragma unroll
        for (int l = 0; l < 2; l++) lo[l] = scr[l][pr >> 1];
      }
    }
    cf    xs[2][2];
    float cs[2][2];
#pragma unroll
    for (int e = 0; e < 2; e++) {
      if constexpr (WT) {
        const fv4* w = W[e];
        mmse_2x2_apply(Y[e][0], Y[e][1], mk(w[0].x, w[0].y), mk(w[0].z, w[0].w), mk(w[1].x, w[1].y),
                       mk(w[1].z, w[1].w), xs[0][e], xs[1][e]);
        cs[0][e] = WC[e].x;
        cs[1][e] = WC[e].y;
      } else {
        eq_re(J, H[e], Y[e], noise, xs[0][e], xs[1][e], cs[0][e], cs[1][e]);
      }
    }
    if constexpr (QM0 != 0 && QM0 == QM1) {
      if (cm) {
        uint32_t wd[2 * QM0];
        if constexpr (L2) {
          if (l2) {
            const uint32_t sh = 16 * (pr & 1);
            llr2_256qam(((lo[0] >> sh) & 0xffffu) | ((lo[1] >> sh) << 16), l2csi, csc, ns, xs, cs, wd);
            cmp_put2<QM0>(im32, fw, fws[0], 2 * pr * QM0 - rp, n_e, wd);
            continue;
          }
        }
        const cf    x0[2] = {xs[0][0], xs[0][1]}, x1[2] = {xs[1][0], xs[1][1]};
        const float c0[2] = {cs[0][0], cs[0][1]}, c1[2] = {cs[1][0], cs[1][1]};
        int16_t     o0[2 * QM0], o1[2 * QM0];
        llr_compute<QM0>(cwd[0], pr, ns, x0, c0, cmb[0], o0);
        llr_compute<QM0>(cwd[1], pr, ns, x1, c1, cmb[1], o1);
#pragma unroll
        for (int k = 0; k < 2 * QM0; k++) wd[k] = (uint32_t)(uint16_t)o0[k] | ((uint32_t)(uint16_t)o1[k] << 16);
        cmp_put2<QM0>(im32, fw, fws[0], 2 * pr * QM0 - rp, n_e, wd);
        continue;
      }
    }
    if constexpr (QM0 != 0) {
      const cf    x[2]   = {xs[0][0], xs[0][1]};
      const float csi[2] = {cs[0][0], cs[0][1]};
      int16_t     o[2 * QM0];
      llr_compute<QM0>(cwd[0], pr, ns, x, csi, cmb[0], o);
      img_put<QM0>(imgs, 2 * pr * QM0 - rp, n_e, o);
    }
    if constexpr (QM1 != 0) {
      const cf    x[2]   = {xs[1][0], xs[1][1]};
      const float csi[2] = {cs[1][0], cs[1][1]};
      int16_t     o[2 * QM1];
      llr_compute<QM1>(cwd[1], pr, ns, x, csi, cmb[1], o);
      img_put<QM1>(imgs + img, 2 * pr * QM1 - rp, n_e, o);
    }
  }
  if (tid < 2 && !cm) imgs[tid * img + n_e] = 0;
  __syncthreads();
  const unsigned long long pt2 = P.prof ? clock64() : 0ull;
  if (P.diag == 1) {
    if (imgs[tid] == 12345 && imgs[img + tid] == 777) P.sb[tid] = 1;
    return;
  }
  {
    if (cm) {
      const GLB uint32_t* ql     = (const GLB uint32_t*)(fw + R.cqoff[kx0][ev]);
      const uint32_t      npairs = R.layer[0].buflen[kx0] / 2;
      GLB uint32_t*       sb[2]  = {(GLB uint32_t*)gptr(P.sb + (size_t)slot[0] * P.sb_stride),
                                    (GLB uint32_t*)gptr(P.sb + (size_t)slot[1] * P.sb_stride)};
      const bool          al     = (((uintptr_t)sb[0] | (uintptr_t)sb[1]) & 15) == 0;
      typedef uint32_t u4v __attribute__((ext_vector_type(4)));
#pragma unroll 1
      for (uint32_t q0 = tid; q0 < cnq; q0 += ER_CQ * ER_THREADS) {
        uint32_t qd[ER_CQ];
#pragma unroll
        for (int k = 0; k < ER_CQ; k++) {
          const uint32_t qi = q0 + k * ER_THREADS;
          qd[k]             = qi < cnq ? ql[qi] : 0u;
        }
#pragma unroll
        for (int k = 0; k < ER_CQ; k++) {
          const uint32_t qi = q0 + k * ER_THREADS;
          if (qi >= cnq) continue;
          const uint4    wa = ((const uint4*)im32)[2 * qi], wb = ((const uint4*)im32)[2 * qi + 1];
          const uint32_t m  = qd[k] >> 16;
          uint32_t       w[8] = {wa.x, wa.y, wa.z, wa.w, wb.x, wb.y, wb.z, wb.w};
#pragma unroll
          for (int p = 0; p < 8; p++) w[p] = (m >> p) & 1u ? w[p] : 0u;
          const uint4    v0 = make_uint4(__builtin_amdgcn_perm(w[1], w[0], 0x05040100u), __builtin_amdgcn_perm(w[3], w[2], 0x05040100u),
                                         __builtin_amdgcn_perm(w[5], w[4], 0x05040100u), __builtin_amdgcn_perm(w[7], w[6], 0x05040100u));
          const uint4    v1 = make_uint4(__builtin_amdgcn_perm(w[1], w[0], 0x07060302u), __builtin_amdgcn_perm(w[3], w[2], 0x07060302u),
                                         __builtin_amdgcn_perm(w[5], w[4], 0x07060302u), __builtin_amdgcn_perm(w[7], w[6], 0x07060302u));
          const uint32_t i  = 4 * (qd[k] & 0xffffu);
          if (al && i + 3 < npairs) {
            __builtin_nontemporal_store((u4v){v0.x, v0.y, v0.z, v0.w}, (GLB u4v*)(sb[0] + i));
            __builtin_nontemporal_store((u4v){v1.x, v1.y, v1.z, v1.w}, (GLB u4v*)(sb[1] + i));
          } else {
            const uint32_t a0[4] = {v0.x, v0.y, v0.z, v0.w}, a1[4] = {v1.x, v1.y, v1.z, v1.w};
#pragma unroll
            for (int cc = 0; cc < 4; cc++)
              if (i + cc < npairs) sb[0][i + cc] = a0[cc], sb[1][i + cc] = a1[cc];
          }
        }
      }
      need[0] = need[1] = false;
    } else if (lean) {
      const uint32_t  npairs = R.layer[0].buflen[kx0] / 2, Kc = (R.layer[0].N[kx0] - 12) / 3;
      const GLB uint32_t* inv32 = (const GLB uint32_t*)gptr(R.layer[0].inv[kx0]);
      GLB uint32_t*   sb[2]  = {(GLB uint32_t*)gptr(P.sb + (size_t)slot[0] * P.sb_stride),
                                (GLB uint32_t*)gptr(P.sb + (size_t)slot[1] * P.sb_stride)};
      const bool      al     = (((uintptr_t)sb[0] | (uintptr_t)sb[1]) & 15) == 0;
      const uint16_t* a0     = (const uint16_t*)imgs;
      const uint16_t* a1     = (const uint16_t*)(imgs + img);
#pragma unroll 1
      for (int rd = 0; rd < ER_R; rd++) {
        uint4 iv[ER_Q];
#pragma unroll
        for (int k = 0; k < ER_Q; k++) {
          const uint32_t i = 4 * (tid + (rd * ER_Q + k) * ER_THREADS);
          if (ER_TPF && rd == 0) {
            iv[k] = iv0[k];
            continue;
          }
          iv[k]            = i + 3 < npairs ? ldg_u4(inv32 + i)
                                            : make_uint4(i < npairs ? inv32[i] : 0xffffffffu,
                                                         i + 1 < npairs ? inv32[i + 1] : 0xffffffffu,
                                                         i + 2 < npairs ? inv32[i + 2] : 0xffffffffu, 0xffffffffu);
        }
#pragma unroll
        for (int k = 0; k < ER_Q; k++) {
          const uint32_t i = 4 * (tid + (rd * ER_Q + k) * ER_THREADS);
          if (i >= npairs) continue;
          if (P.sparse && !rm_quad_defined(nbm[0], 2 * i, Kc)) continue;
          const uint32_t w[4] = {iv[k].x, iv[k].y, iv[k].z, iv[k].w};
          uint32_t       v0[4], v1[4];
#pragma unroll
          for (int cc = 0; cc < 4; cc++) {
            const uint32_t r0 = min(w[cc] & 0xffffu, n_e), r1 = min(w[cc] >> 16, n_e);
            v0[cc] = (uint32_t)a0[r0] | ((uint32_t)a0[r1] << 16);
            v1[cc] = (uint32_t)a1[r0] | ((uint32_t)a1[r1] << 16);
          }
          typedef uint32_t u4v __attribute__((ext_vector_type(4)));
          if (al && i + 3 < npairs) {
            __builtin_nontemporal_store((u4v){v0[0], v0[1], v0[2], v0[3]}, (GLB u4v*)(sb[0] + i));
            __builtin_nontemporal_store((u4v){v1[0], v1[1], v1[2], v1[3]}, (GLB u4v*)(sb[1] + i));
          } else {
#pragma unroll
            for (int cc = 0; cc < 4; cc++)
              if (i + cc < npairs) sb[0][i + cc] = v0[cc], sb[1][i + cc] = v1[cc];
          }
        }
      }
      need[0] = need[1] = false;
    } else if (need[0] && need[1] && R.layer[0].inv[kx0] == R.layer[1].inv[kx1] &&
               R.layer[0].buflen[kx0] == R.layer[1].buflen[kx1]) {
      const uint32_t  npairs = R.layer[0].buflen[kx0] / 2, Kc = (R.layer[0].N[kx0] - 12) / 3;
      const GLB uint32_t* inv32 = (const GLB uint32_t*)gptr(R.layer[0].inv[kx0]);
      GLB uint32_t*   sb[2]  = {(GLB uint32_t*)gptr(P.sb + (size_t)slot[0] * P.sb_stride),
                                (GLB uint32_t*)gptr(P.sb + (size_t)slot[1] * P.sb_stride)};
      const bool      al     = (((uintptr_t)sb[0] | (uintptr_t)sb[1]) & 15) == 0;
#pragma unroll 1
      for (int rd = 0; rd < ER_R2; rd++) {
        uint4 iv[ER_Q2], old[2][ER_Q2];
#pragma unroll
        for (int k = 0; k < ER_Q2; k++) {
          const uint32_t i = 4 * (tid + (rd * ER_Q2 + k) * ER_THREADS);
          iv[k]            = i + 3 < npairs ? ldg_u4(inv32 + i)
                                            : make_uint4(i < npairs ? inv32[i] : 0xffffffffu,
                                                         i + 1 < npairs ? inv32[i + 1] : 0xffffffffu,
                                                         i + 2 < npairs ? inv32[i + 2] : 0xffffffffu, 0xffffffffu);
#pragma unroll
          for (int l = 0; l < 2; l++) {
            if (fresh[l] || i >= npairs) {
              old[l][k] = make_uint4(0u, 0u, 0u, 0u);
            } else if (al && i + 3 < npairs) {
              old[l][k] = ldg_u4(sb[l] + i);
            } else {
              old[l][k] = make_uint4(sb[l][i], i + 1 < npairs ? sb[l][i + 1] : 0u, i + 2 < npairs ? sb[l][i + 2] : 0u,
                                     i + 3 < npairs ? sb[l][i + 3] : 0u);
            }
          }
        }
#pragma unroll
        for (int k = 0; k < ER_Q2; k++) {
          const uint32_t i = 4 * (tid + (rd * ER_Q2 + k) * ER_THREADS);
          if (i >= npairs) continue;
          const uint32_t w[4] = {iv[k].x, iv[k].y, iv[k].z, iv[k].w};
          uint32_t       v[2][4];
          const bool     od0 = fresh[0] || rm_quad_defined(obm[0], 2 * i, Kc);
          const bool     od1 = fresh[1] || rm_quad_defined(obm[1], 2 * i, Kc);
          bool           any = fresh[0] || fresh[1] || !od0 || !od1;
#pragma unroll
          for (int cc = 0; cc < 4; cc++) {
            const uint32_t r0 = w[cc] & 0xffffu, r1 = w[cc] >> 16;
            const bool     h0 = r0 != 0xffffu && r0 < n_e, h1 = r1 != 0xffffu && r1 < n_e;
            any |= h0 || h1;
            const uint32_t i0 = img_i16(h0 ? r0 : 0u), i1 = img_i16(h1 ? r1 : 0u);
            const uint32_t o0[4] = {od0 ? old[0][k].x : 0u, od0 ? old[0][k].y : 0u, od0 ? old[0][k].z : 0u,
                                    od0 ? old[0][k].w : 0u};
            const uint32_t o1[4] = {od1 ? old[1][k].x : 0u, od1 ? old[1][k].y : 0u, od1 ? old[1][k].z : 0u,
                                    od1 ? old[1][k].w : 0u};
            v[0][cc] = add_pairs16(o0[cc], (h0 ? (uint16_t)imgs[i0] : 0u) | ((h1 ? (uint16_t)imgs[i1] : 0u) << 16));
            v[1][cc] = add_pairs16(o1[cc], (h0 ? (uint16_t)imgs[img + i0] : 0u) |
                                               ((h1 ? (uint16_t)imgs[img + i1] : 0u) << 16));
          }
          if (!any) continue;
#pragma unroll
          for (int l = 0; l < 2; l++) {
            if (al && i + 3 < npairs) {
              typedef uint32_t u4v __attribute__((ext_vector_type(4)));
              __builtin_nontemporal_store((u4v){v[l][0], v[l][1], v[l][2], v[l][3]}, (GLB u4v*)(sb[l] + i));
            } else {
#pragma unroll
              for (int cc = 0; cc < 4; cc++)
                if (i + cc < npairs) sb[l][i + cc] = v[l][cc];
            }
          }
        }
      }
      need[0] = need[1] = false;
    }
  }
#pragma unroll
  for (int l = 0; l < 2; l++) {
    if (!need[l]) continue;
    const EqRmLayer& T      = R.layer[l];
    const uint32_t   kx     = c < T.C1 ? 0u : 1u;
    const uint32_t   npairs = T.buflen[kx] / 2, Kc = (T.N[kx] - 12) / 3;
    const GLB uint32_t* inv32 = (const GLB uint32_t*)gptr(T.inv[kx]);
    const uint16_t*  acc    = (const uint16_t*)(imgs + l * img);
    GLB uint32_t*    sb     = (GLB uint32_t*)gptr(P.sb + (size_t)slot[l] * P.sb_stride);
    const bool       sb16   = ((uintptr_t)sb & 15) == 0;
#pragma unroll 1
    for (int rd = 0; rd < ER_R; rd++) {
    uint4 iv[ER_Q], old[ER_Q];
#pragma unroll
    for (int k = 0; k < ER_Q; k++) {
      const uint32_t i = 4 * (tid + (rd * ER_Q + k) * ER_THREADS);
      iv[k]            = i + 3 < npairs ? ldg_u4(inv32 + i)
                                        : make_uint4(i < npairs ? inv32[i] : 0xffffffffu,
                                                     i + 1 < npairs ? inv32[i + 1] : 0xffffffffu,
                                                     i + 2 < npairs ? inv32[i + 2] : 0xffffffffu, 0xffffffffu);
      if (fresh[l]) {
        old[k] = make_uint4(0u, 0u, 0u, 0u);
      } else if (sb16 && i + 3 < npairs) {
        old[k] = ldg_u4(sb + i);
      } else {
        old[k] = make_uint4(i < npairs ? sb[i] : 0u, i + 1 < npairs ? sb[i + 1] : 0u, i + 2 < npairs ? sb[i + 2] : 0u,
                            i + 3 < npairs ? sb[i + 3] : 0u);
      }
    }
#pragma unroll
    for (int k = 0; k < ER_Q; k++) {
      const uint32_t i = 4 * (tid + (rd * ER_Q + k) * ER_THREADS);
// ... 105 lines not shown
```

### srsran_amd/csrc/pdsch_runtime.cpp

```cpp
#include <hip/hip_runtime.h>

#include <algorithm>
#include <chrono>
#include <stdlib.h>
#include <cmath>
#include <map>
#include <unordered_map>
#include <atomic>
#include <mutex>
#include <stdio.h>
#include <string.h>
#include <string>
#include <vector>

#include "../../include/srsran_amd/dlsch.h"
#include "../../include/srsran_amd/pdsch.h"
#include "../../include/srsran_amd/tdec.h"
#include "host_staging.h"
#include "lte_common.h"
#include "pdsch_internal.h"
#include "rm_tables.h"
#include "runtime_internal.h"

using namespace mi355;
// ... 568 lines not shown
  return MI355_SUCCESS;
}

void mi355_pdsch_destroy(mi355_pdsch_t* q)
{
  if (!q) return;
  (void)hipSetDevice(q->device);
  (void)hipDeviceSynchronize();
  for (auto& kv : q->maps) (void)hipFree(kv.second.d);
  for (auto& f : q->map_free) (void)hipFree(f.first);
  for (void* r : q->retired) (void)hipFree(r);
  for (auto& kv : q->scr) (void)hipFree(kv.second);
  (void)hipFree(q->gold);
  (void)hipFree(q->scratch);
  if (q->fe_done) (void)hipEventDestroy(q->fe_done);
  mi355_dlsch_destroy(q->dlsch);
  if (q->own) (void)hipStreamDestroy(q->own);
  delete q;
}

mi355_dlsch_t* mi355_pdsch_dlsch(mi355_pdsch_t* q) { return q ? q->dlsch : nullptr; }

int mi355_pdsch_set_llr_8bit(mi355_pdsch_t* q, int enable)
{
  if (!q) return MI355_ERROR_INVALID_INPUTS;
  std::lock_guard<std::mutex> lk(q->mu);
  q->llr8 = enable != 0;
  return MI355_SUCCESS;
}

int mi355_pdsch_set_ce_invariant(mi355_pdsch_t* q, int enable)
{
  if (!q) return MI355_ERROR_INVALID_INPUTS;
  std::lock_guard<std::mutex> lk(q->mu);
  q->ce_inv = enable != 0;
  return MI355_SUCCESS;
}

int mi355_pdsch_frontend(mi355_pdsch_t* q, const mi355_pdsch_job_t* jobs, uint32_t njobs, void* stream)
{
  if (!q || (njobs && !jobs)) return MI355_ERROR_INVALID_INPUTS;
  std::lock_guard<std::mutex> lock(q->mu);
  CHECK_HIP(hipSetDevice(q->device));
  hipStream_t          s = stream ? (hipStream_t)stream : q->own;
  std::vector<JobPlan> plans(njobs);
  int                  r = trim_maps(q);
  if (r) return r;
  for (uint32_t i = 0; i < njobs; i++) {
    r = plan_job(q, jobs[i], nullptr, plans[i]);
    if (r) return r;
    set_invariant(q, plans[i], q->ce_inv);
  }
  r = run_frontend(q, jobs, plans, s);
  if (r) return r;
  CHECK_HIP(wait_stream(s));
  q->last = plans;
  return MI355_SUCCESS;
}

int mi355_pdsch_debug_stage(mi355_pdsch_t* q, uint32_t job, uint32_t cw, const float** d, const float** csi,
                            const int16_t** e)
{
  if (!q || job >= q->last.size() || cw > 1) return MI355_ERROR_INVALID_INPUTS;
  if (q->e_pending) {
    CHECK_HIP(hipSetDevice(q->device));
    CHECK_HIP(hipDeviceSynchronize());
    CHECK_HIP(pdsch_launch_fused(q->last_jobs_dev, q->last_njobs, q->last_max_fpairs, q->last_fkeys.data(),
                                 (uint32_t)q->last_fkeys.size(), q->own));
    CHECK_HIP(hipStreamSynchronize(q->own));
    q->e_pending = false;
  }
  const JobPlan& P = q->last[job];
  if (d) *d = (const float*)(q->d_arena + P.d_off[cw]);
  if (csi) *csi = q->csi_arena + P.csi_off[cw];
  if (e) {
    *e = nullptr;
    for (uint32_t t = 0; t < 2; t++)
      if (P.decode[t] && P.cw_of_tb[t] == cw)
        *e = q->llr8 ? (const int16_t*)((const int8_t*)q->e_arena + P.e_off[t]) : q->e_arena + P.e_off[t];
  }
  return MI355_SUCCESS;
}

int mi355_pdsch_debug_set_cache_limits(mi355_pdsch_t* q, uint32_t max_maps, uint32_t max_scr)
{
  if (!q) return MI355_ERROR_INVALID_INPUTS;
  std::lock_guard<std::mutex> lk(q->mu);
  if (max_maps) q->max_maps = max_maps;
  if (max_scr) q->max_scr = max_scr;
  return MI355_SUCCESS;
}

int mi355_pdsch_debug_job_map(mi355_pdsch_t* q, uint32_t job, const uint16_t** d_map, uint32_t* n)
{
  if (!q || job >= q->last.size() || !d_map || !n) return MI355_ERROR_INVALID_INPUTS;
  *d_map = q->last[job].dev.map;
  *n     = q->last[job].dev.nof_re;
  return MI355_SUCCESS;
}

int mi355_pdsch_decode_batch(mi355_pdsch_t*           q,
                             mi355_softbuffer_pool_t* pool,
                             const mi355_pdsch_job_t* jobs,
                             uint32_t                 njobs,
                             mi355_pdsch_res_t*       res,
                             void*                    stream)
{
  return mi355::pdsch_decode_batch_dev_noise(q, pool, jobs, njobs, res, stream, nullptr, mi355::WaitHook{},
                                             q && q->ce_inv);
}

int mi355_pdsch_decode_launch(mi355_pdsch_t* q, mi355_softbuffer_pool_t* pool, const mi355_pdsch_job_t* jobs,
                              uint32_t njobs, mi355_pdsch_res_t* res, void* stream)
{
  if (!q) return MI355_ERROR_INVALID_INPUTS;
  if (q->api_armed) return MI355_ERROR;
  if (!q->api_pend) q->api_pend.reset(new mi355::PdschPending);
  const int r = mi355::pdsch_decode_batch_dev_noise(q, pool, jobs, njobs, res, stream, nullptr, mi355::WaitHook{},
                                                    q->ce_inv, q->api_pend.get());
  q->api_armed = true;
  return r;
}

int mi355_pdsch_decode_collect(mi355_pdsch_t* q)
{
  if (!q) return MI355_ERROR_INVALID_INPUTS;
  if (!q->api_armed) return MI355_SUCCESS;
  q->api_armed = false;
  return q->api_pend->collect();
}

}

static void fill_results(mi355_pdsch_res_t* res, const std::vector<std::pair<uint32_t, uint32_t>>& who,
                         const std::vector<int32_t>& ret, const std::vector<float>& avg)
{
  for (size_t k = 0; k < who.size(); k++) {
    mi355_pdsch_res_t& o   = res[2 * who[k].first + who[k].second];
    o.crc                  = ret[k] == 0;
    o.ret                  = ret[k] == MI355_ERROR_INVALID_INPUTS ? MI355_ERROR : MI355_SUCCESS;
    o.avg_iterations_block = avg[k];
  }
}

static bool plan_eq_rm(mi355_pdsch_t* q, mi355_softbuffer_pool_t* pool, const mi355_pdsch_job_t* jobs,
                       const std::vector<JobPlan>& plans, EqRmPlan& er)
{
  if (getenv("MI355_NO_EQRM") || q->llr8 || !pool || plans.empty()) return false;
  const SoftbufferView v = softbuffer_view(pool);
  er.rj.assign(plans.size(), EqRmJob{});
  er.max_c = er.img = er.cimg = 0;
  static const bool compact = !getenv("MI355_EQRM_COMPACT") || atoi(getenv("MI355_EQRM_COMPACT")) != 0;
  struct CKey {
    uint32_t        key = UINT32_MAX, E = 0, nq = 0, qoff = 0;
    const uint16_t* tab = nullptr;
  } ck[4];
  uint32_t        seg_tbs = UINT32_MAX, tab_key[2] = {UINT32_MAX, UINT32_MAX};
  CbSegm          seg{};
  int             seg_err = 0;
  const uint16_t* tab[2]  = {nullptr, nullptr};
  auto inv_of = [&](uint32_t K, uint32_t rv, const uint16_t** out) {
    const uint32_t key = K << 2 | rv;
    for (int k = 0; k < 2; k++)
      if (tab_key[k] == key) return *out = tab[k], 0;
    const int e = dlsch_rm_inv(q->dlsch, K, rv, out);
    tab_key[1] = tab_key[0], tab[1] = tab[0], tab_key[0] = key, tab[0] = *out;
    return e;
  };
  for (size_t i = 0; i < plans.size(); i++) {
    const JobPlan&             P   = plans[i];
    const mi355_pdsch_cfg_t&   cfg = jobs[i].cfg;
    const mi355_pdsch_grant_t& g   = cfg.grant;
    if (!P.dev.fused) return false;
    EqRmJob& R  = er.rj[i];
    uint32_t nt = 0, tbs = 0, nbits = 0, n_max = 0, cimg = 0;
    for (uint32_t t = 0; t < 2; t++) {
      if (!P.decode[t]) continue;
      const mi355_ra_tb_t& tb = g.tb[t];
      const uint32_t       qm = mod_bits(tb.mod);
      if (nt && (qm != R.Qm || (uint32_t)tb.tbs != tbs || tb.nof_bits != nbits)) return false;
      if (tb.tbs <= 0) return false;
      if ((uint32_t)tb.tbs != seg_tbs) seg_tbs = (uint32_t)tb.tbs, seg_err = cbsegm(seg_tbs, &seg);
      if (seg_err || seg.F || seg.C == 0 || seg.C > v.max_cb || cfg.softbuffer[t] >= v.nof_sb || tb.rv > 3 || qm == 0)
        return false;
      tbs = (uint32_t)tb.tbs, nbits = tb.nof_bits, nt++;
      R.C = seg.C, R.Qm = qm, R.Gp = nbits / qm;
      n_max                 = qm * (R.Gp / seg.C) + qm;
      const uint32_t kmin   = seg.C1 ? (seg.C1 < seg.C ? std::min(seg.K1, seg.K2) : seg.K1) : seg.K2;
      if (n_max > 3 * kmin + 12) return false;
      EqRmLayer& L = R.layer[P.cw_of_tb[t] & 1];
      for (uint32_t kx = 0; kx < 2; kx++) {
        const uint32_t K = kx ? seg.K2 : seg.K1;
        if (!K || (kx == 0 && !seg.C1) || (kx == 1 && seg.C1 == seg.C)) continue;
        if (inv_of(K, tb.rv, &L.inv[kx])) return false;
        L.N[kx]      = 3 * K + 12;
        L.buflen[kx] = dlsch_rm_buflen(K);
      }
      L.C1    = seg.C1;
      L.slot0 = cfg.softbuffer[t] * v.max_cb;
      if (compact && rm_sparse_writes() && &L == &R.layer[0]) {
        const uint32_t ne0 = qm * (R.Gp / seg.C), gamma = R.Gp % seg.C;
        for (uint32_t kx = 0; kx < 2; kx++) {
          const uint32_t K = kx ? seg.K2 : seg.K1;
          if (!K || (kx == 0 && !seg.C1) || (kx == 1 && seg.C1 == seg.C)) continue;
          for (uint32_t ev = 0; ev < (gamma ? 2u : 1u); ev++) {
            const uint32_t E = ne0 + ev * qm, key = K << 2 | tb.rv;
            CKey*          hit = nullptr;
            for (auto& c : ck)
              if (c.key == key && c.E == E) hit = &c;
            if (!hit) {
              for (int k = 3; k > 0; k--) ck[k] = ck[k - 1];
              hit = &ck[0];
              if (dlsch_rm_compact(q->dlsch, K, tb.rv, E, &hit->tab, &hit->nq, &hit->qoff)) return false;
              hit->key = key, hit->E = E;
            }
            R.cmp[kx][ev] = hit->tab, R.cnq[kx][ev] = hit->nq, R.cqoff[kx][ev] = hit->qoff;
            cimg          = std::max(cimg, 8 * hit->nq);
          }
        }
      }
    }
    if (nt < 2) {
      for (auto& row : R.cmp) row[0] = row[1] = nullptr;
    } else {
      er.cimg = std::max(er.cimg, cimg);
    }
    er.max_c = std::max(er.max_c, nt ? R.C : 0u);
    er.img   = std::max(er.img, n_max);
  }
  er.pool = EqRmPool{v.buf, v.stride, v.cb_crc, v.fresh, rm_sparse_writes() ? 1 : 0};
  static const int eqrm_diag = getenv("MI355_EQRM_DIAG") ? atoi(getenv("MI355_EQRM_DIAG")) : 0;
  er.pool.diag = eqrm_diag;
  er.pool.prof = g_eqrm_prof.load();
  return er.max_c > 0;
}

int mi355::pdsch_decode_batch_dev_noise(mi355_pdsch_t* q, mi355_softbuffer_pool_t* pool, const mi355_pdsch_job_t* jobs,
                                        uint32_t njobs, mi355_pdsch_res_t* res, void* stream, const float* d_noise,
                                        WaitHook hook, bool ce_invariant, PdschPending* pend, bool after_s)
{
  if (!q || !pool || !res || (njobs && !jobs)) return MI355_ERROR_INVALID_INPUTS;
  std::lock_guard<std::mutex> lock(q->mu);
  static const bool prof = getenv("MI355_HOST_PROF") != nullptr;
  auto              now  = [] { return std::chrono::steady_clock::now(); };
  const auto        t0   = now();
  CHECK_HIP(hipSetDevice(q->device));
  hipStream_t          s = stream ? (hipStream_t)stream : q->own;
  std::vector<JobPlan> plans(njobs);
  int                  r = trim_maps(q);
  if (r) return r;
  for (uint32_t i = 0; i < njobs; i++) {
    r = plan_job(q, jobs[i], &res[2 * i], plans[i]);
    if (r) return r;
    if (d_noise && jobs[i].cfg.decoder_type != MI355_MIMO_DECODER_ZF) plans[i].dev.noise_dev = d_noise + i;
    set_invariant(q, plans[i], ce_invariant);
  }
  EqRmPlan   er;
  const bool eqrm = plan_eq_rm(q, pool, jobs, plans, er);
  const auto t1   = now();
  r               = run_frontend(q, jobs, plans, s, after_s, eqrm ? &er : nullptr);
  if (r) return r;
  if (prof) {
    auto us = [](auto a, auto b) { return std::chrono::duration<double, std::micro>(b - a).count(); };
    fprintf(stderr, "[mi355 host] pdsch: plan %.1f us, frontend launch %.1f us\n", us(t0, t1), us(t1, now()));
  }
  q->last.swap(plans);
  const std::vector<JobPlan>& plan = q->last;

  std::map<uint32_t, std::vector<std::pair<uint32_t, uint32_t>>> by_its;
  std::map<uint32_t, std::vector<mi355_dlsch_tb_t>>              tbs;
  for (uint32_t i = 0; i < njobs; i++) {
    const mi355_pdsch_cfg_t& cfg = jobs[i].cfg;
    if (cfg.max_nof_iterations) q->max_its = cfg.max_nof_iterations;
    for (uint32_t t = 0; t < 2; t++) {
      if (!plan[i].decode[t]) continue;
      const mi355_ra_tb_t& tb = cfg.grant.tb[t];
      const uint32_t       Nl = cfg.grant.nof_layers != cfg.grant.nof_tb ? 2 : 1;
      mi355_dlsch_tb_t     d{};
      d.tbs         = (uint32_t)std::max(0, tb.tbs);
      d.nof_e_bits  = tb.nof_bits;
      d.Qm          = mod_bits(tb.mod) * Nl;
      d.rv          = tb.rv;
      d.softbuffer  = cfg.softbuffer[t];
      d.e_offset    = plan[i].e_off[t];
      d.data_offset = (uint64_t)(uintptr_t)jobs[i].payload[t];
      by_its[q->max_its].push_back({i, t});
      tbs[q->max_its].push_back(d);
    }
  }
  if (pend) {
    pend->used = 0;
    pend->res  = res;
  }
  for (auto& kv : tbs) {
    const uint32_t       its = kv.first;
    std::vector<int32_t> ret_local, *ret = &ret_local;
    std::vector<float>   avg_local, *avg = &avg_local;
    DlschPending*        dp = nullptr;
    if (pend) {
      const uint32_t g = pend->used;
      if (pend->groups.size() <= g) {
        pend->groups.emplace_back(new DlschPending);
        pend->ret.emplace_back();
        pend->avg.emplace_back();
        pend->who.emplace_back();
      }
      dp = pend->groups[g].get(), ret = &pend->ret[g], avg = &pend->avg[g];
      pend->who[g] = by_its[its];
    }
    ret->assign(kv.second.size(), 0);
    avg->assign(kv.second.size(), 0.f);
    if ((r = mi355_dlsch_set_max_iterations(q->dlsch, its))) return r;
    const bool after = after_s || (pend && pend->used > 0);
    r = dlsch_decode_dev_hook(q->dlsch, pool, q->e_arena, kv.second.data(), (uint32_t)kv.second.size(), nullptr,
                              ret->data(), avg->data(), s, hook, q->llr8, dp, after, eqrm);
    hook = WaitHook{};
    if (r) return r;
    if (pend)
      pend->used++;
    else
      fill_results(res, by_its[its], *ret, *avg);
  }
  return MI355_SUCCESS;
}

int mi355::PdschPending::collect()
{
  int r = MI355_SUCCESS;
  for (uint32_t g = 0; g < used; g++) {
    const int e = groups[g]->collect();
    if (e) {
      r = e;
      continue;
    }
    fill_results(res, who[g], ret[g], avg[g]);
  }
  used = 0;
  return r;
}
```

### srsran_amd/csrc/runtime_internal.h

```cpp
#pragma once
#include "../../include/srsran_amd/dlsch.h"
#include "../../include/srsran_amd/pdsch.h"

#include <hip/hip_runtime.h>

#include <memory>
#include <utility>
#include <atomic>
#include <vector>

namespace mi355 {

struct WaitHook {
  void (*fn)(void*) = nullptr;
  void* ctx         = nullptr;
};

struct DlschPending {
  char*                host = nullptr;
  size_t               cap  = 0;
  hipEvent_t           ev   = nullptr;
  bool                 armed = false;
  uint32_t             ntb   = 0;
  size_t               avg_off = 0;
  std::vector<uint8_t> invalid;
  int32_t*             ret = nullptr;
  float*               avg = nullptr;
  std::atomic<uint32_t>* spec_mask = nullptr;
  uint32_t             max_its   = 0;
  DlschPending()                    = default;
  DlschPending(const DlschPending&) = delete;
  ~DlschPending();
  int collect();
};

int dlsch_decode_dev_hook(mi355_dlsch_t* q, mi355_softbuffer_pool_t* pool, const void* d_e_bits,
                          const mi355_dlsch_tb_t* tbs, uint32_t ntb, uint8_t* d_data, int32_t* ret, float* avg_iterations,
                          void* stream, WaitHook hook, bool llr8 = false, DlschPending* pend = nullptr,
                          bool after_s = false, bool rm_done = false);

int      dlsch_rm_inv(mi355_dlsch_t* q, uint32_t K, uint32_t rv, const uint16_t** out);
uint32_t dlsch_rm_buflen(uint32_t K);
int      dlsch_rm_compact(mi355_dlsch_t* q, uint32_t K, uint32_t rv, uint32_t E, const uint16_t** tab, uint32_t* nq,
                          uint32_t* qoff);
bool     rm_sparse_writes();
struct SoftbufferView {
  int16_t* buf;
  size_t   stride;
  uint8_t* cb_crc;
  uint8_t* fresh;
  uint32_t nof_sb, max_cb;
};
SoftbufferView softbuffer_view(mi355_softbuffer_pool_t* p);

struct PdschPending {
  std::vector<std::unique_ptr<DlschPending>>                   groups;
  std::vector<std::vector<int32_t>>                            ret;
  std::vector<std::vector<float>>                              avg;
  std::vector<std::vector<std::pair<uint32_t, uint32_t>>>      who;
  uint32_t                                                     used = 0;
  mi355_pdsch_res_t*                                           res  = nullptr;
  int collect();
};

int pdsch_decode_batch_dev_noise(mi355_pdsch_t* q, mi355_softbuffer_pool_t* pool, const mi355_pdsch_job_t* jobs,
                                 uint32_t njobs, mi355_pdsch_res_t* res, void* stream, const float* d_noise,
                                 WaitHook hook = WaitHook{}, bool ce_invariant = false, PdschPending* pend = nullptr,
                                 bool after_s = false);

}
```

### srsran_amd/csrc/tdec_internal.h

```cpp
#pragma once
#include <hip/hip_runtime.h>
#include <stdint.h>

#include "dlsch_internal.h"

#define TDEC_INF 10000
#define TDEC_WARMUP 40
#define TDEC_SEG 8

namespace mi355 {

struct TdecWinArgs {
  const int16_t*  in;
  size_t          in_stride;
  const uint32_t* in_idx;
  const uint8_t*  done;
  const uint32_t* remaining;
  uint32_t*       A1;
  uint32_t*       E;
  uint32_t*       D;
  uint32_t*       ckpt;
  const uint32_t* dstE;
  const uint32_t* dstA;
  int             ncb, L, Lp, nseg, n, write_d;
  uint8_t*        dec;
  size_t          dec_stride;
  const uint32_t* gS;
  const uint32_t* gP;
  DlschCheckArgs  chk;
  int             chk_on;
  int             spec;
  int             rowmask;
};

struct TdecDecideArgs {
  const uint32_t* D;
  uint8_t*        out;
  size_t          out_stride;
  int             ncb, L, Lp;
  const uint8_t*  done;
  const uint32_t* remaining;
};

struct TdecGenArgs {
  const uint32_t* S;
  const uint32_t* P0;
  const uint32_t* P1;
  uint32_t*       A1;
  uint32_t*       E;
  uint32_t*       D;
  uint32_t*       ckpt;
  const uint16_t* pi;
  int             npair, K, Kp, nseg, n, write_d;
};

struct TdecGenPrepArgs {
  const int16_t*  in;
  size_t          stride;
  const uint32_t* in_idx;
  uint32_t *     S, *P0, *P1, *E;
  int            ncb, npair, K, Kp;
};

struct TdecGenDecideArgs {
  const uint32_t* D;
  uint8_t*        out;
  size_t          out_stride;
  int             ncb, K, Kp;
};

#define TDEC_GEN_CB_L 12
#define TDEC_GEN_CB_KP(K) (((K) + 3 + 7) / 8 * 8)
struct TdecGenCbArgs {
  const int16_t*  in;
  size_t          in_stride;
  const uint32_t* in_idx;
  uint16_t*       ws;
  const uint16_t* pi;
  uint8_t*        out;
  size_t          out_stride;
  uint32_t*       reruns;
  int             ncb, K, Kp, h0, h1, warm, persist;
};
int        tdec_gen_cb_threads(int K);
size_t     tdec_gen_cb_lds(int K, int threads);
hipError_t tdec_gen_cb_launch(const TdecGenCbArgs& a, hipStream_t s);

struct TdecLatArgs {
  const int16_t*  in;
  size_t          in_stride;
  const uint32_t* in_idx;
  const uint32_t* dstE;
  const uint32_t* dstA;
  uint8_t*        done;
  DlschCheckArgs  chk;
  uint64_t*       prof;
  int             ncb, K, rowmask;
  int             bwave;
  int             owaves;
};
size_t     tdec_lat_lds(int K, int nsb);
hipError_t tdec_lat_launch(int nsb, const TdecLatArgs& a, hipStream_t s);

struct TdecRun {
  const int16_t*  in;
  size_t          in_stride;
  const uint32_t* in_idx;
  const uint8_t*  done;
  const uint32_t* remaining;
  uint32_t        n, K, h0, h1;
  uint8_t*        out;
  size_t          out_stride;
  hipStream_t     stream;
  const DlschCheckArgs* chk = nullptr;
  bool*                 chk_fused = nullptr;
  bool  spec       = false;
  bool* spec_taken = nullptr;
  bool  redo       = false;
  bool  rowmask    = false;
};

hipError_t tdec_win_launch_halfit(int nsb, const TdecWinArgs& a, hipStream_t s);
bool       tdec_win_spec_ok(int nsb, int L);
int        tdec_set_diag(int mode);
hipError_t tdec_win_launch_decide(int nsb, const TdecDecideArgs& a, hipStream_t s);
hipError_t tdec_gen_launch_prep(const TdecGenPrepArgs& a, hipStream_t s);
hipError_t tdec_gen_launch_halfit(const TdecGenArgs& a, hipStream_t s);
hipError_t tdec_gen_launch_decide(const TdecGenDecideArgs& a, hipStream_t s);

}

struct mi355_tdec_batch;
int mi355_tdec_run_internal(mi355_tdec_batch* q, const mi355::TdecRun& r);
int mi355_tdec_win_tables(mi355_tdec_batch* q, uint32_t K, const uint32_t** dstE, const uint32_t** dstA);
```

### srsran_amd/csrc/tdec_kernels.hip

```cpp
#include <hip/hip_runtime.h>

#include <atomic>
#include <stdint.h>
#include <stdlib.h>

#include "crc_device.h"
#include "tdec_internal.h"

namespace mi355 {

typedef short v2s __attribute__((ext_vector_type(2)));

__device__ __forceinline__ v2s U(uint32_t u) { return __builtin_bit_cast(v2s, u); }
__device__ __forceinline__ uint32_t W(v2s v) { return __builtin_bit_cast(uint32_t, v); }
__device__ __forceinline__ v2s sadd(v2s a, v2s b) { return __builtin_elementwise_add_sat(a, b); }
__device__ __forceinline__ v2s ssub(v2s a, v2s b) { return __builtin_elementwise_sub_sat(a, b); }
__device__ __forceinline__ v2s vmax(v2s a, v2s b) { return __builtin_elementwise_max(a, b); }
__device__ __forceinline__ v2s splat(short s) { return (v2s){s, s}; }
__device__ __forceinline__ uint32_t hi_lo(uint32_t a, uint32_t b) { return __builtin_amdgcn_alignbit(b, a, 16); }
__device__ __forceinline__ uint32_t from_prev(uint32_t v)
{
  return (uint32_t)__builtin_amdgcn_update_dpp(0, (int)v, 0x111, 0xf, 0xf, true);
}
__device__ __forceinline__ uint32_t from_next(uint32_t v)
{
  return (uint32_t)__builtin_amdgcn_update_dpp(0, (int)v, 0x101, 0xf, 0xf, true);
}

__device__ __forceinline__ void bm_set(uint32_t* bm, uint32_t m, bool v)
{
  const uint32_t by = m >> 3;
  if (v) atomicOr(&bm[by >> 2], 1u << (((by & 3) << 3) + 7 - (m & 7)));
}


template <bool SAT>
__device__ __forceinline__ v2s add(v2s a, v2s b)
{
  if constexpr (SAT) {
    return sadd(a, b);
  } else {
    return a + b;
  }
}

template <bool SAT>
__device__ __forceinline__ void beta_step(const v2s o[8], v2s x, v2s y, v2s n[8])
{
  v2s xy = add<SAT>(x, y);
  n[0]   = vmax(add<SAT>(o[4], xy), o[0]);
  n[1]   = vmax(o[4], add<SAT>(o[0], xy));
  n[2]   = vmax(add<SAT>(o[5], y), add<SAT>(o[1], x));
  n[3]   = vmax(add<SAT>(o[5], x), add<SAT>(o[1], y));
  n[4]   = vmax(add<SAT>(o[6], x), add<SAT>(o[2], y));
  n[5]   = vmax(add<SAT>(o[6], y), add<SAT>(o[2], x));
  n[6]   = vmax(o[7], add<SAT>(o[3], xy));
  n[7]   = vmax(add<SAT>(o[7], xy), o[3]);
}

template <bool SAT>
__device__ __forceinline__ void alpha_cands(const v2s o[8], v2s x, v2s y, v2s c0[8], v2s c1[8])
{
  v2s xy = add<SAT>(x, y);
  c0[0]  = o[0];
  c1[0]  = add<SAT>(o[1], xy);
  c0[1]  = add<SAT>(o[3], y);
  c1[1]  = add<SAT>(o[2], x);
  c0[2]  = add<SAT>(o[4], y);
  c1[2]  = add<SAT>(o[5], x);
  c0[3]  = o[7];
  c1[3]  = add<SAT>(o[6], xy);
  c0[4]  = o[1];
  c1[4]  = add<SAT>(o[0], xy);
  c0[5]  = add<SAT>(o[2], y);
  c1[5]  = add<SAT>(o[3], x);
  c0[6]  = add<SAT>(o[5], y);
  c1[6]  = add<SAT>(o[4], x);
  c0[7]  = o[6];
  c1[7]  = add<SAT>(o[7], xy);
}

template <bool SAT>
__device__ __forceinline__ void normalize(v2s s[8])
{
#pragma unroll
  for (int i = 1; i < 8; i++) {
    if constexpr (SAT) {
      s[i] = ssub(s[i], s[0]);
    } else {
      s[i] = s[i] - s[0];
    }
  }
  s[0] = splat(0);
}

__device__ __forceinline__ void set_minf(v2s s[8])
{
#pragma unroll
  for (int i = 0; i < 8; i++) s[i] = splat(-TDEC_INF);
}

template <int NL>
__device__ __forceinline__ void tdec_fused_check(const TdecWinArgs& a, int cb, int l, int K, const uint32_t* bm,
                                                 const uint32_t (*t4)[4][256])
{
  const DlschCheckArgs& c      = a.chk;
  const CbDesc&         d      = c.desc[cb];
  const uint32_t        nbytes = (uint32_t)K / 8, chunk = nbytes / NL;
  const int             pi     = d.C > 1 ? 1 : 0;
  const uint8_t*        bytes  = (const uint8_t*)bm;
  uint32_t              crc    = crc24_words(bytes + l * chunk, chunk, t4[pi]);
  crc = gf2_mulmod24(crc, c.scale[128 + 8 * pi + l], pi ? c.crc24b->poly : c.crc24a->poly);
#pragma unroll
  for (int o = NL / 2; o >= 1; o >>= 1) crc ^= (uint32_t)__shfl_xor((int)crc, o, 64);
  const bool ok  = crc == 0;
  const bool fin = ok || c.h + 1 == c.max_its;
  if (fin) {
    uint8_t*       dst  = c.data + d.data_off + (size_t)d.cb * d.rlen / 8;
    const uint32_t nb   = (d.cb + 1 == d.C) ? nbytes : d.rlen / 8;
    const uint32_t head = min(nb, (4u - (uint32_t)((uintptr_t)dst & 3u)) & 3u);
    const uint32_t nw   = (nb - head) / 4, tail0 = head + 4 * nw;
    for (uint32_t i = l; i < head; i += NL) dst[i] = bytes[i];
    for (uint32_t i = tail0 + l; i < nb; i += NL) dst[i] = bytes[i];
    uint32_t* dw = (uint32_t*)(dst + head);
    const uint32_t sh = head;
    for (uint32_t w = l; w < nw; w += NL) {
      const uint32_t lo = bm[w + sh / 4], hi = bm[w + sh / 4 + 1];
      dw[w]             = sh ? __builtin_amdgcn_alignbyte(hi, lo, sh) : lo;
    }
    if (l == 0) {
      c.its[cb] = c.h + 1;
      if (ok) {
        c.done[cb]       = 1;
        c.sb_crc[d.slot] = 1;
      } else {
        c.done[cb] = 2;
      }
    }
  }
  const uint64_t un = __builtin_amdgcn_ballot_w64(l == 0 && !fin);
  if (un && (threadIdx.x & 63) == (uint32_t)__builtin_ctzll(un)) flag_set(c.next);
}


#define WG_AT(arr, j) (arr)[((size_t)grp * Lp + (j)) * 64 + q]

#define TDEC_BM_WORDS (8 * 193)
__shared__ uint32_t tdec_tx_lds[4][2][TDEC_SEG * 64];
__shared__ uint32_t tdec_ym_lds[4][8 * SB_ROWMASK_WORDS];
__shared__ uint32_t tdec_bm_lds[4 * TDEC_BM_WORDS];
__shared__ int16_t  tdec_stg_lds[4][TDEC_SEG * 128];
__shared__ uint32_t tdec_stg_row[4][TDEC_SEG];

#ifndef TDEC_WAVES_PER_EU
#define TDEC_WAVES_PER_EU 2
#endif
#ifndef TDEC_NPH
#define TDEC_NPH 1
#endif
#ifndef TDEC_FPF
#define TDEC_FPF 2
#endif
#ifndef TDEC_CLONE_NO_E
#define TDEC_CLONE_NO_E 0
#endif
#ifndef TDEC_CLONE_KEEP
#define TDEC_CLONE_KEEP 0
#endif
#ifndef TDEC_STAGE_OUT
#define TDEC_STAGE_OUT 1
#endif
#ifndef TDEC_CLONE_NO_CK
#define TDEC_CLONE_NO_CK 0
#endif
#ifndef TDEC_DEFER_FLUSH
#define TDEC_DEFER_FLUSH 0
#endif
#ifndef TDEC_NT_OUT
#define TDEC_NT_OUT 0
#endif
#ifndef TDEC_NT_CK
#define TDEC_NT_CK 0
#endif
#ifndef TDEC_OUT_AUX
#define TDEC_OUT_AUX -1
#endif
#ifndef TDEC_CK_AUX
#define TDEC_CK_AUX -1
#endif
#ifndef TDEC_CLONE_NO_FIN
#define TDEC_CLONE_NO_FIN 0
#endif
#ifndef TDEC_CLONE_NO_TAB
#define TDEC_CLONE_NO_TAB 0
#endif
#ifndef TDEC_CLONE_CK_HALF
#define TDEC_CLONE_CK_HALF 0
#endif
template <int NSB, int SEG, int MODE, int DIAG, bool FULL, int OUTK, bool GI = false, bool TX = false>
__device__ __forceinline__ void tdec_win_body(const TdecWinArgs& a, const int gl,
                                              const uint32_t (*crc_t4)[4][256] = nullptr)
{
  constexpr int NL = NSB / 2;
  constexpr int G  = 64 / NL;
  static_assert(!TX || (NSB == 16 && FULL && SEG == 8), "TX loads need 8-lane rows and whole 8-step segments");
  const int     grp = __builtin_amdgcn_readfirstlane(gl >> 6), q = gl & 63;
  const int     cbg = q / NL, l = q % NL;
  if constexpr (!TX) {
    if (grp * G + cbg >= a.ncb) return;
    if (a.done && a.done[grp * G + cbg]) return;
  }
  if (a.remaining && *a.remaining == 0) return;

  const int  L = a.L, Lp = a.Lp, nseg = a.nseg;
  constexpr bool CL     = DIAG == 20;
  constexpr bool dec2   = MODE == 2;
  constexpr bool has_ap = MODE == 1;

  const int       cb   = grp * G + cbg;
  const int       K    = L * NSB;
  const size_t    bidx = a.in_idx ? a.in_idx[cb] : (size_t)cb;
  const uint32_t* in32 = (const uint32_t*)(a.in + bidx * a.in_stride);
  const size_t    wg0  = (size_t)grp * Lp * 64 + q;
  const uint32_t* X    = dec2 ? a.E + wg0 : (GI ? a.gS + wg0 : in32 + l);
  const int       xs   = (dec2 || GI) ? 64 : NL;
  const uint32_t* Y    = GI ? a.gP + wg0 : in32 + (dec2 ? (K + 32) : (K + 32) / 2) + l;
  const int       ys   = GI ? 64 : NL;
  const uint32_t* AP   = a.A1 + wg0;
  uint32_t*       ck   = a.ckpt + (size_t)grp * nseg * 8 * 64 + q;
  [[maybe_unused]] const __amdgpu_buffer_rsrc_t ckr =
      __builtin_amdgcn_make_buffer_rsrc(a.ckpt + (size_t)grp * nseg * 8 * 64, 0, nseg * 8 * 64 * 4, 0x00020000);

  const uint4*    txin  = nullptr;
  if constexpr (TX) {
    const int txc = grp * G + ((q >> 1) & 7);
    txin = (const uint4*)(a.in + (a.in_idx ? (size_t)a.in_idx[txc] : (size_t)txc) * a.in_stride) + (2 * (q >> 4) + (q & 1));
  }
  const int       txoX  = 0;
  const int       txoY  = (dec2 ? (L * NSB + 32) : (L * NSB + 32) / 2) / 4;
  uint32_t*       txb   = nullptr;
  if constexpr (TX) {
    txb = &tdec_tx_lds[threadIdx.x >> 6][0][0];
  }
  constexpr bool RMK = NSB == 16 && !GI;
  uint32_t*      ymask = nullptr;
  if constexpr (RMK) {
    ymask = tdec_ym_lds[threadIdx.x >> 6];
#pragma unroll
    for (int w = l; w < SB_ROWMASK_WORDS; w += NL) {
      uint32_t v = 0xffffffffu;
      if (a.rowmask) v = ((const uint32_t*)(a.in + bidx * a.in_stride + SB_ROWMASK))[(dec2 ? SB_ROWMASK_WORDS : 0) + w];
      ymask[cbg * SB_ROWMASK_WORDS + w] = v;
    }
    __builtin_amdgcn_fence(__ATOMIC_RELEASE, "wavefront");
    __builtin_amdgcn_wave_barrier();
    __builtin_amdgcn_fence(__ATOMIC_ACQUIRE, "wavefront");
  }
  auto yrow = [&](int c, int j) -> bool {
    if constexpr (RMK) {
      return (ymask[c * SB_ROWMASK_WORDS + (j >> 5)] >> (j & 31)) & 1u;
    } else {
      return true;
    }
  };
  auto tx_load = [&](int so, int j0, uint32_t* r, bool par = false) {
    uint4 v0 = make_uint4(0u, 0u, 0u, 0u), v1 = v0;
    const int tc = (q >> 1) & 7, jr = j0 + (q >> 4);
    if (!par || yrow(tc, jr)) v0 = txin[so + j0 * 2];
    if (!par || yrow(tc, jr + 4)) v1 = txin[so + (j0 + 4) * 2];
    r[0] = v0.x; r[1] = v0.y; r[2] = v0.z; r[3] = v0.w;
    r[4] = v1.x; r[5] = v1.y; r[6] = v1.z; r[7] = v1.w;
  };
  auto tx_unpack = [&](int b, const uint32_t* r, uint32_t* o) {
    uint32_t* w = txb + b * SEG * 64;
    ((uint4*)w)[q]      = make_uint4(r[0], r[1], r[2], r[3]);
    ((uint4*)w)[64 + q] = make_uint4(r[4], r[5], r[6], r[7]);
    __builtin_amdgcn_fence(__ATOMIC_RELEASE, "wavefront");
    __builtin_amdgcn_wave_barrier();
    __builtin_amdgcn_fence(__ATOMIC_ACQUIRE, "wavefront");
#pragma unroll
    for (int i = 0; i < SEG; i++) o[i] = w[64 * i + q];
  };

  v2s st[8], nw[8], aw[8];

  set_minf(aw);
#pragma unroll 1
  for (int b = 0; b < TDEC_WARMUP / 8; b++) {
    uint32_t xo[8], yo[8], ao[8] = {};
#pragma unroll
    for (int i = 0; i < 8; i++) {
      const int j = (L - TDEC_WARMUP) + 8 * b + i;
      xo[i]       = X[j * xs];
      yo[i]       = yrow(cbg, j) ? Y[j * ys] : 0u;
      if constexpr (has_ap) ao[i] = AP[j * 64];
    }
#pragma unroll
    for (int i = 0; i < 8; i++) {
      const int k = 8 * b + i;
      v2s       x = U(hi_lo(from_prev(xo[i]), xo[i]));
      if constexpr (has_ap) x = sadd(x, U(hi_lo(from_prev(ao[i]), ao[i])));
      if constexpr (CL) {
        aw[k & 7] = aw[k & 7] ^ x ^ U(yo[i]);
        continue;
      }
      v2s c0[8], c1[8];
      alpha_cands<true>(aw, x, U(hi_lo(from_prev(yo[i]), yo[i])), c0, c1);
#pragma unroll
      for (int s = 0; s < 8; s++) aw[s] = vmax(c0[s], c1[s]);
      if ((k & 1) == 0 && k != 0) normalize<true>(aw);
    }
  }

  if constexpr (DIAG != 2) {
  set_minf(st);
#pragma unroll 1
  for (int b = TDEC_WARMUP / 8 - 1; b >= 0; b--) {
    uint32_t xo[8], yo[8], ao[8] = {};
#pragma unroll
    for (int i = 0; i < 8; i++) {
      const int j = 8 * b + i;
      xo[i]       = X[j * xs];
      yo[i]       = yrow(cbg, j) ? Y[j * ys] : 0u;
      if constexpr (has_ap) ao[i] = AP[j * 64];
    }
#pragma unroll
    for (int i = 7; i >= 0; i--) {
      const int k = 8 * b + i;
      v2s       x = U(hi_lo(xo[i], from_next(xo[i])));
      if constexpr (has_ap) x = sadd(x, U(hi_lo(ao[i], from_next(ao[i]))));
      if constexpr (CL) {
        st[k & 7] = st[k & 7] ^ x ^ U(yo[i]);
        continue;
      }
      beta_step<true>(st, x, U(hi_lo(yo[i], from_next(yo[i]))), nw);
#pragma unroll
      for (int s = 0; s < 8; s++) st[s] = nw[s];
      if ((k & 1) == 0 && k != 0) normalize<true>(st);
    }
  }
  if (l == NL - 1) {
    const int16_t* T = a.in + bidx * a.in_stride + 3 * (K + 32) + (dec2 ? 6 : 0);
    v2s            tr[8], tn[8];
    tr[0] = splat(0);
#pragma unroll
    for (int i = 1; i < 8; i++) tr[i] = splat(-TDEC_INF);
#pragma unroll
    for (int t = 2; t >= 0; t--) {
      beta_step<false>(tr, splat(T[2 * t]), splat(T[2 * t + 1]), tn);
#pragma unroll
      for (int i = 0; i < 8; i++) tr[i] = tn[i];
    }
#pragma unroll
    for (int i = 0; i < 8; i++) st[i] = (v2s){st[i].x, tr[i].y};
  }
#pragma unroll
  for (int s = 0; s < 8; s++) {
    if constexpr (DIAG == 9 || TDEC_NT_CK) {
      __builtin_nontemporal_store(W(st[s]), &ck[((size_t)(nseg - 1) * 8 + s) * 64]);
    } else {
      ck[((size_t)(nseg - 1) * 8 + s) * 64] = W(st[s]);
    }
  }

  {
    uint32_t cx[SEG], cy[SEG], ca[SEG] = {};
    auto     load = [&](int t, uint32_t* x, uint32_t* y, uint32_t* ap) {
      if constexpr (TX) {
        if constexpr (!dec2) tx_load(txoX, t * SEG, x);
        tx_load(txoY, t * SEG, y, true);
      }
#pragma unroll
      for (int i = 0; i < SEG; i++) {
        const int j = FULL ? t * SEG + i : min(t * SEG + i, L - 1);
        if constexpr (!TX || dec2) x[i] = X[j * xs];
        if constexpr (!TX) y[i] = yrow(cbg, j) ? Y[j * ys] : 0u;
        if constexpr (has_ap) ap[i] = AP[j * 64];
      }
    };
    uint32_t bx[SEG], by[SEG], ba[SEG] = {}, dx[SEG], dy[SEG], da[SEG] = {};
    load(nseg - 1, cx, cy, ca);
    if (nseg > 1) load(nseg - 2, bx, by, ba);
    auto seg = [&](int t, const uint32_t* rx, const uint32_t* ry, const uint32_t* sa, uint32_t* lx, uint32_t* ly,
                   uint32_t* la) {
      uint32_t sx[SEG], sy[SEG];
      if constexpr (TX) {
        if constexpr (!dec2) tx_unpack(0, rx, sx);
        tx_unpack(1, ry, sy);
      }
#pragma unroll
      for (int i = 0; i < SEG; i++) {
        if constexpr (!TX || dec2) sx[i] = rx[i];
        if constexpr (!TX) sy[i] = ry[i];
      }
      if (t > 1) load(t - 2, lx, ly, la);
#pragma unroll
      for (int i = SEG - 1; i >= 0; i--) {
        const int k = t * SEG + i;
        if (FULL || k < L) {
          v2s x = U(sx[i]);
          if constexpr (has_ap) x = sadd(x, U(sa[i]));
          if constexpr (DIAG == 4) {
            st[0] = st[0] ^ x ^ U(sy[i]);
            continue;
          }
          if constexpr (CL) {
            st[i] = st[i] ^ x ^ U(sy[i]);
          } else {
            beta_step<true>(st, x, U(sy[i]), nw);
#pragma unroll
            for (int s = 0; s < 8; s++) st[s] = nw[s];
          }
          if (i == 0 && t > 0 && DIAG != 3 && !(CL && TDEC_CLONE_NO_CK) && !(CL && TDEC_CLONE_CK_HALF && (t & 1))) {
#pragma unroll
            for (int s = 0; s < 8; s++) {
              if constexpr (DIAG == 9 || TDEC_NT_CK) {
                __builtin_nontemporal_store(W(st[s]), &ck[((size_t)(t - 1) * 8 + s) * 64]);
              } else if constexpr (DIAG == 10) {
                if (t & 1) ck[((size_t)(t - 1) * 8 + s) * 64] = W(st[s]);
              } else if constexpr (DIAG == 11 || (DIAG >= 100 && (DIAG & 4))) {
// ... 524 lines not shown
```

### srsran_amd/csrc/tdec_runtime.cpp

```cpp
#include <hip/hip_runtime.h>

#include <map>
#include <mutex>
#include <stdio.h>
#include <string.h>
#include <vector>

#include "../../include/srsran_amd/tdec.h"
#include "lte_qpp_table.h"
#include "tdec_internal.h"

using namespace mi355;

#define CHECK_HIP(x)                                                                                                   \
  do {                                                                                                                 \
    hipError_t e_ = (x);                                                                                               \
    if (e_ != hipSuccess) {                                                                                            \
      fprintf(stderr, "[srsran_amd] %s:%d %s: %s\n", __FILE__, __LINE__, #x, hipGetErrorString(e_));                 \
      return MI355_ERROR;                                                                                              \
    }                                                                                                                  \
  } while (0)

namespace {

// ... 123 lines not shown
  }
  size_t cap = bytes + bytes / 8;
  CHECK_HIP(hipMalloc(&q->ws, cap));
  q->ws_cap = cap;
  return MI355_SUCCESS;
}

static hipEvent_t next_event(mi355_tdec_batch_t* q)
{
  if (q->ev_used == q->ev.size()) {
    hipEvent_t e;
    if (hipEventCreate(&e) != hipSuccess) return nullptr;
    q->ev.push_back(e);
  }
  return q->ev[q->ev_used++];
}

extern "C" {

uint32_t mi355_tdec_autoimp_get_subblocks(uint32_t long_cb)
{
  if (!(long_cb % 16) && long_cb > 800) return 16;
  if (!(long_cb % 8) && long_cb > 400) return 8;
  return 0;
}

int mi355_tdec_batch_create(mi355_tdec_batch_t** q, int device)
{
  if (!q) return MI355_ERROR_INVALID_INPUTS;
  int ndev = 0;
  CHECK_HIP(hipGetDeviceCount(&ndev));
  if (device < 0 || device >= ndev) return MI355_ERROR_INVALID_INPUTS;
  CHECK_HIP(hipSetDevice(device));
  auto* b   = new mi355_tdec_batch;
  b->device = device;
  if (hipStreamCreateWithFlags(&b->own, hipStreamNonBlocking) != hipSuccess) {
    delete b;
    return MI355_ERROR;
  }
  *q = b;
  return MI355_SUCCESS;
}

void mi355_tdec_batch_destroy(mi355_tdec_batch_t* q)
{
  if (!q) return;
  (void)hipSetDevice(q->device);
  (void)hipDeviceSynchronize();
  for (auto* m : {&q->tables, &q->gtables}) {
    for (auto& kv : *m) {
      (void)hipFree(kv.second.dstE);
      (void)hipFree(kv.second.dstA);
      (void)hipFree(kv.second.pi);
    }
  }
  for (auto e : q->ev) (void)hipEventDestroy(e);
  if (q->ws) (void)hipFree(q->ws);
  if (q->reruns) (void)hipFree(q->reruns);
  if (q->own) (void)hipStreamDestroy(q->own);
  delete q;
}

int mi355_tdec_set_diag(int mode) { return mi355::tdec_set_diag(mode); }

void mi355_tdec_batch_set_profiling(mi355_tdec_batch_t* q, int enable)
{
  if (q) q->prof = enable != 0;
}

int mi355_tdec_batch_kernel_stats(mi355_tdec_batch_t* q, double* ms, uint32_t* launches)
{
  if (!q) return MI355_ERROR_INVALID_INPUTS;
  double total = 0;
  for (size_t i = 0; i + 1 < q->ev_used; i += 2) {
    CHECK_HIP(hipEventSynchronize(q->ev[i + 1]));
    float t = 0;
    CHECK_HIP(hipEventElapsedTime(&t, q->ev[i], q->ev[i + 1]));
    total += t;
  }
  if (ms) *ms = total;
  if (launches) *launches = (uint32_t)(q->ev_used / 2);
  q->ev_used = 0;
  return MI355_SUCCESS;
}

}

int mi355_tdec_win_tables(mi355_tdec_batch_t* q, uint32_t K, const uint32_t** dstE, const uint32_t** dstA)
{
  if (!q || cb_index(K) < 0 || mi355_tdec_autoimp_get_subblocks(K) == 0) return MI355_ERROR_INVALID_INPUTS;
  std::lock_guard<std::mutex> lock(q->mu);
  const Geometry g = geometry(K, 1, MI355_TDEC_AUTO);
  KTables*       t = nullptr;
  const int      r = get_tables(q, g, &t);
  if (r) return r;
  *dstE = t->dstE;
  *dstA = t->dstA;
  return MI355_SUCCESS;
}

int mi355_tdec_run_internal(mi355_tdec_batch_t* q, const TdecRun& rq)
{
  const int16_t* d_in = rq.in;
  size_t in_stride = rq.in_stride;
  uint32_t n = rq.n, K = rq.K, h0 = rq.h0, h1 = rq.h1;
  uint8_t* d_out = rq.out;
  size_t out_stride = rq.out_stride;
  if (!q || !d_in || !d_out || h1 <= h0 || cb_index(K) < 0) return MI355_ERROR_INVALID_INPUTS;
  const bool generic = q->impl == MI355_TDEC_GENERIC || mi355_tdec_autoimp_get_subblocks(K) == 0;
  const size_t need  = generic ? 3 * (size_t)K + 12 : 3 * (size_t)(K + 32) + 12;
  if (in_stride < need || (in_stride & 1) || out_stride < K / 8) {
    return MI355_ERROR_INVALID_INPUTS;
  }
  if (n == 0) return MI355_SUCCESS;
  std::lock_guard<std::mutex> lock(q->mu);
  CHECK_HIP(hipSetDevice(q->device));
  hipStream_t s = rq.stream ? rq.stream : q->own;

  const Geometry g = geometry(K, n, q->impl);
  if (rq.redo && !g.nsb) return MI355_SUCCESS;
  KTables*       t = nullptr;
  int            r = get_tables(q, g, &t);
  if (r) return r;
  const bool cbk = !g.nsb && !rq.done && !rq.remaining && !rq.chk &&
                   (q->gen_cb == 1 || (q->gen_cb < 0 && (K > 400 || n <= 4096)));
  if (h0 == 0) {
    if ((r = ensure_ws(q, ws_bytes(g, n, cbk)))) return r;
  } else if (ws_bytes(g, n, cbk) > q->ws_cap) {
    return MI355_ERROR;
  }

  char* p     = q->ws;
  auto  carve = [&](size_t bytes) {
    char* c = p;
    p += ((bytes + 255) / 256) * 256;
    return c;
  };

  if (g.nsb) {
    const size_t arr = (size_t)g.ngrp * g.Lp * 64 * 4;
    static const size_t pad = getenv("MI355_TDEC_WS_PAD") ? (size_t)atoll(getenv("MI355_TDEC_WS_PAD")) : 0;
    auto*        A1  = (uint32_t*)carve(arr + pad);
    auto*        E   = (uint32_t*)carve(arr + pad);
    auto*        D   = (uint32_t*)carve(arr + pad);
    auto*        CK  = (uint32_t*)carve((size_t)g.ngrp * g.nseg * 8 * 64 * 4);

    const bool fuse = (g.L % 8 == 0 || (K % 64 == 0 && (K / 8) % (g.nsb / 2) == 0)) && out_stride % 8 == 0 &&
                      (uintptr_t)d_out % 8 == 0;
    for (uint32_t h = h0; h < h1; h++) {
      if (rq.redo) {
        TdecWinArgs wa{d_in, in_stride, rq.in_idx, rq.done, rq.remaining, A1, E, D, CK, t->dstE, t->dstA,
                       (int)n, (int)g.L, (int)g.Lp, (int)g.nseg, (int)h, 0, nullptr, out_stride};
        wa.rowmask = rq.rowmask && g.nsb == 16 && in_stride == SB_STRIDE;
        CHECK_HIP(tdec_win_launch_halfit(g.nsb, wa, s));
        continue;
      }
      TdecWinArgs wa{d_in, in_stride, rq.in_idx, rq.done, rq.remaining, A1, E, D, CK, t->dstE, t->dstA,
                     (int)n, (int)g.L, (int)g.Lp, (int)g.nseg, (int)h, h + 1 == h1,
                     (fuse && h + 1 == h1) ? d_out : nullptr, out_stride};
      wa.rowmask = rq.rowmask && g.nsb == 16 && in_stride == SB_STRIDE;
      if (rq.spec && fuse && h + 1 == h1 && tdec_win_spec_ok(g.nsb, g.L)) {
        wa.spec = 1;
        if (rq.spec_taken) *rq.spec_taken = true;
      }
      if (rq.chk && fuse && h + 1 == h1) {
        wa.chk    = *rq.chk;
        wa.chk.h  = h;
        wa.chk_on = 1;
        if (rq.chk_fused) *rq.chk_fused = true;
      }
      hipEvent_t e0 = nullptr, e1 = nullptr;
      if (q->prof) {
        e0 = next_event(q);
        e1 = next_event(q);
        if (e0) (void)hipEventRecord(e0, s);
      }
      CHECK_HIP(tdec_win_launch_halfit(g.nsb, wa, s));
      if (q->prof && e1) (void)hipEventRecord(e1, s);
    }
    if (!fuse && !rq.redo) {
      TdecDecideArgs da{D, d_out, out_stride, (int)n, (int)g.L, (int)g.Lp, rq.done, rq.remaining};
      CHECK_HIP(tdec_win_launch_decide(g.nsb, da, s));
    }
  } else if (cbk) {
    TdecGenCbArgs ca{};
    ca.in         = d_in;
    ca.in_stride  = in_stride;
    ca.in_idx     = rq.in_idx;
    ca.ws         = (uint16_t*)q->ws;
    ca.pi         = t->pi;
    ca.out        = d_out;
    ca.out_stride = out_stride;
    ca.reruns     = q->reruns;
    ca.ncb        = (int)n;
    ca.K          = (int)K;
    ca.Kp         = TDEC_GEN_CB_KP((int)K);
    ca.h0         = (int)h0;
    ca.h1         = (int)h1;
    ca.warm       = q->gen_warm;
    ca.persist    = 1;
    hipEvent_t e0 = nullptr, e1 = nullptr;
    if (q->prof) {
      e0 = next_event(q);
      e1 = next_event(q);
      if (e0) (void)hipEventRecord(e0, s);
    }
    CHECK_HIP(tdec_gen_cb_launch(ca, s));
    if (q->prof && e1) (void)hipEventRecord(e1, s);
  } else {
    const size_t arr = (size_t)g.npair * g.Kp * 4;
    auto*        S   = (uint32_t*)carve(arr);
    auto*        P0  = (uint32_t*)carve(arr);
    auto*        P1  = (uint32_t*)carve(arr);
    auto*        A1  = (uint32_t*)carve(arr);
    auto*        E   = (uint32_t*)carve(arr);
    auto*        D   = (uint32_t*)carve(arr);
    auto*        CK  = (uint32_t*)carve((size_t)g.npair * g.nseg * 32);

    if (h0 == 0) {
      TdecGenPrepArgs pa{d_in, in_stride, rq.in_idx, S, P0, P1, E, (int)n, (int)g.npair, (int)K, (int)g.Kp};
      CHECK_HIP(tdec_gen_launch_prep(pa, s));
    }
    for (uint32_t h = h0; h < h1; h++) {
      TdecGenArgs ga{S, P0, P1, A1, E, D, CK, t->pi,
                     (int)g.npair, (int)K, (int)g.Kp, (int)g.nseg, (int)h, h + 1 == h1};
      hipEvent_t e0 = nullptr, e1 = nullptr;
      if (q->prof) {
        e0 = next_event(q);
        e1 = next_event(q);
        if (e0) (void)hipEventRecord(e0, s);
      }
      CHECK_HIP(tdec_gen_launch_halfit(ga, s));
      if (q->prof && e1) (void)hipEventRecord(e1, s);
    }
    TdecGenDecideArgs da{D, d_out, out_stride, (int)n, (int)K, (int)g.Kp};
    CHECK_HIP(tdec_gen_launch_decide(da, s));
  }
  return MI355_SUCCESS;
}

extern "C" {

int mi355_tdec_batch_run_dev(mi355_tdec_batch_t* q,
                             const int16_t*      d_in,
                             size_t              in_stride,
                             uint32_t            n,
                             uint32_t            K,
                             uint32_t            nhalf,
                             uint8_t*            d_out,
                             size_t              out_stride,
                             void*               stream)
{
  if (nhalf == 0) return MI355_ERROR_INVALID_INPUTS;
  return mi355_tdec_run_internal(
      q, TdecRun{d_in, in_stride, nullptr, nullptr, nullptr, n, K, 0, nhalf, d_out, out_stride, (hipStream_t)stream});
}

int mi355_tdec_batch_halfit_dev(mi355_tdec_batch_t* q,
                                const int16_t*      d_in,
                                size_t              in_stride,
                                uint32_t            n,
                                uint32_t            K,
                                uint32_t            half_idx,
                                uint8_t*            d_out,
                                size_t              out_stride,
                                void*               stream)
{
  return mi355_tdec_run_internal(q, TdecRun{d_in, in_stride, nullptr, nullptr, nullptr, n, K, half_idx, half_idx + 1, d_out,
                                            out_stride, (hipStream_t)stream});
}

int mi355_tdec_batch_set_generic(mi355_tdec_batch_t* q, int per_cb, int warmup)
{
  if (!q || per_cb < -1 || per_cb > 1 || warmup < 0) return MI355_ERROR_INVALID_INPUTS;
  std::lock_guard<std::mutex> lock(q->mu);
  q->gen_cb   = per_cb;
  q->gen_warm = warmup;
  return MI355_SUCCESS;
}

int mi355_tdec_batch_generic_reruns(mi355_tdec_batch_t* q, uint32_t* reruns)
{
  if (!q || !reruns) return MI355_ERROR_INVALID_INPUTS;
  std::lock_guard<std::mutex> lock(q->mu);
  CHECK_HIP(hipSetDevice(q->device));
  if (!q->reruns) {
    CHECK_HIP(hipMalloc(&q->reruns, 4));
    CHECK_HIP(hipMemset(q->reruns, 0, 4));
    *reruns = 0;
    return MI355_SUCCESS;
  }
  CHECK_HIP(hipDeviceSynchronize());
  CHECK_HIP(hipMemcpy(reruns, q->reruns, 4, hipMemcpyDeviceToHost));
  CHECK_HIP(hipMemset(q->reruns, 0, 4));
  return MI355_SUCCESS;
}

int mi355_tdec_batch_set_impl(mi355_tdec_batch_t* q, int impl)
{
  if (!q || (impl != MI355_TDEC_AUTO && impl != MI355_TDEC_GENERIC)) return MI355_ERROR_INVALID_INPUTS;
  q->impl = impl;
  return MI355_SUCCESS;
}

int mi355_tdec_batch_run(mi355_tdec_batch_t* q,
                         const int16_t*      in,
                         size_t              in_stride,
                         uint32_t            n,
                         uint32_t            K,
                         uint32_t            nhalf,
                         uint8_t*            out,
                         size_t              out_stride)
{
// ... 97 lines not shown
```

### srsran_amd/dlsch.py

```python
from __future__ import annotations

import ctypes as C

import numpy as np

from . import check, lib
from .tdec import DeviceBuffer


class TbDesc(C.Structure):
    _fields_ = [("tbs", C.c_uint32), ("nof_e_bits", C.c_uint32), ("Qm", C.c_uint32), ("rv", C.c_uint32),
                ("softbuffer", C.c_uint32), ("e_offset", C.c_uint64), ("data_offset", C.c_uint64)]


def _declare():
    L = lib()
    if getattr(L, "_dlsch_declared", False):
        return L
    vp, u32, i32 = C.c_void_p, C.c_uint32, C.c_int
    L.mi355_softbuffer_pool_create.argtypes = [C.POINTER(vp), u32, u32, i32]
    L.mi355_softbuffer_pool_destroy.argtypes = [vp]
    L.mi355_softbuffer_reset.argtypes = [vp, u32, vp]
    L.mi355_softbuffer_reset_tbs.argtypes = [vp, u32, u32, vp]
    L.mi355_softbuffer_reset_cb.argtypes = [vp, u32, u32, vp]
    L.mi355_softbuffer_reset_all.argtypes = [vp, vp]
    L.mi355_softbuffer_pool_materialize.argtypes = [vp, u32, u32, vp]
    L.mi355_dlsch_create.argtypes = [C.POINTER(vp), i32]
    L.mi355_dlsch_destroy.argtypes = [vp]
    L.mi355_dlsch_set_max_iterations.argtypes = [vp, u32]
    L.mi355_dlsch_decode_dev.argtypes = [vp, vp, vp, C.POINTER(TbDesc), u32, vp, C.POINTER(C.c_int32),
                                         C.POINTER(C.c_float), vp]
    L.mi355_dlsch_decode8_dev.argtypes = [vp, vp, vp, C.POINTER(TbDesc), u32, vp, C.POINTER(C.c_int32),
                                         C.POINTER(C.c_float), vp]
    L._dlsch_declared = True
    return L


class SoftbufferPool:
    def __init__(self, nof_sb: int, max_cb: int = 32, device: int = 0):
        self.L = _declare()
        h = C.c_void_p()
        check(self.L.mi355_softbuffer_pool_create(C.byref(h), nof_sb, max_cb, device), "softbuffer_pool_create")
        self.h, self.nof_sb, self.max_cb = h, nof_sb, max_cb

    def reset(self, sb: int):
        check(self.L.mi355_softbuffer_reset(self.h, sb, None), "softbuffer_reset")
        lib().mi355_device_sync()

    def reset_all(self):
        check(self.L.mi355_softbuffer_reset_all(self.h, None), "softbuffer_reset_all")
        lib().mi355_device_sync()

    def materialize(self, first: int = 0, n: int | None = None):
        lib().mi355_device_sync()
        n = self.nof_sb - first if n is None else n
        check(self.L.mi355_softbuffer_pool_materialize(self.h, first, n, None), "softbuffer_pool_materialize")
        lib().mi355_device_sync()

    def close(self):
        if getattr(self, "h", None):
            self.L.mi355_softbuffer_pool_destroy(self.h)
            self.h = None

    def __del__(self):
        try:
            self.close()
        except Exception:
            pass


class Dlsch:
    def __init__(self, device: int = 0, max_iterations: int = 10):
        self.L = _declare()
        h = C.c_void_p()
        check(self.L.mi355_dlsch_create(C.byref(h), device), "dlsch_create")
        self.h, self.device = h, device
        check(self.L.mi355_dlsch_set_max_iterations(self.h, max_iterations), "set_max_iterations")

    def set_max_iterations(self, n: int):
        check(self.L.mi355_dlsch_set_max_iterations(self.h, n), "set_max_iterations")

    def decode(self, pool: SoftbufferPool, tbs: list[dict], e_bits: list[np.ndarray], llr8: bool = False):
        n = len(tbs)
        dt = np.int8 if llr8 else np.int16
        offs = np.cumsum([0] + [e.size for e in e_bits])
        allE = np.concatenate([np.ascontiguousarray(e, dt) for e in e_bits]) if n else np.zeros(1, dt)
        doff = np.cumsum([0] + [t["tbs"] // 8 + 8 for t in tbs])
        d_e = DeviceBuffer(max(allE.nbytes, 2), self.device).upload(allE)
        d_data = DeviceBuffer(max(int(doff[-1]), 1), self.device)
        lib().mi355_memset_dev(d_data.ptr, 0, int(doff[-1]))
        desc = (TbDesc * n)()
        for i, t in enumerate(tbs):
            desc[i] = TbDesc(t["tbs"], int(e_bits[i].size), t["Qm"], t.get("rv", 0), t.get("softbuffer", i),
                             int(offs[i]), int(doff[i]))
        ret = (C.c_int32 * n)()
        its = (C.c_float * n)()
        fn = self.L.mi355_dlsch_decode8_dev if llr8 else self.L.mi355_dlsch_decode_dev
        check(fn(self.h, pool.h, d_e.ptr, desc, n, d_data.ptr, ret, its, None), "dlsch_decode_dev")
        host = np.zeros(int(doff[-1]), np.uint8)
        d_data.download(host)
        datas = [host[doff[i]: doff[i] + tbs[i]["tbs"] // 8 + 6].copy() for i in range(n)]
        return [int(r) for r in ret], datas, [float(v) for v in its]

    def close(self):
        if getattr(self, "h", None):
            self.L.mi355_dlsch_destroy(self.h)
            self.h = None

    def __del__(self):
        try:
            self.close()
        except Exception:
            pass
```

Baseline: 125,200 Mbps.

## Add compact parity side-buffer written by eq-RM and read by turbo decoder

The fused equalize/rate-match kernel now also writes the punctured parity rows of each code block into a small dense side buffer, with a per-slot valid flag. The turbo decoder's transpose load then reads parity from this compact buffer, using prefix popcounts over the row mask, instead of gathering sparse rows from the large softbuffer. The aim is to cut scattered global reads in the decoder half-iterations. In exchange it adds extra writes in eq-RM, extra LDS and popcount work, and valid-flag invalidation in the other RM paths and in materialize.

```diff
diff --git a/include/srsran_amd/dlsch.h b/include/srsran_amd/dlsch.h
--- a/include/srsran_amd/dlsch.h
+++ b/include/srsran_amd/dlsch.h
@@ -21,6 +21,8 @@
                                      void* stream);
 int mi355_softbuffer_pool_buffer(mi355_softbuffer_pool_t* p, int16_t** buf, uint32_t* stride, uint32_t* max_cb);
 int mi355_softbuffer_pool_materialize(mi355_softbuffer_pool_t* p, uint32_t first, uint32_t n, void* stream);
+int mi355_softbuffer_pool_pside(mi355_softbuffer_pool_t* p, int16_t** side, uint8_t** valid, uint32_t* stride,
+                                uint32_t* rows);
 
 int mi355_softbuffer_pool_data(mi355_softbuffer_pool_t* p, uint8_t** data, uint32_t* stride, uint32_t* nof_sb);
 int mi355_softbuffer_get_cb_crc(mi355_softbuffer_pool_t* p, uint32_t sb, uint8_t* cb_crc, void* stream);
diff --git a/srsran_amd/csrc/dlsch_internal.h b/srsran_amd/csrc/dlsch_internal.h
--- a/srsran_amd/csrc/dlsch_internal.h
+++ b/srsran_amd/csrc/dlsch_internal.h
@@ -7,6 +7,8 @@
 #define SB_CONV8 10240
 #define SB_ROWMASK 18544
 #define SB_ROWMASK_WORDS 12
+#define SB_PSIDE_ROWS 64
+#define SB_PSIDE_STRIDE (2 * SB_PSIDE_ROWS * 16)
 
 namespace mi355 {
 
@@ -52,6 +54,7 @@
   uint8_t*        fresh;
   uint32_t        fold2;
   int             sparse;
+  uint8_t*        pside_valid;
 };
 
 struct DlschRm8Args {
@@ -65,6 +68,7 @@
   const uint8_t*  sb_crc;
   const uint8_t*  fresh;
   int16_t*        conv;
+  uint8_t*        pside_valid;
 };
 
 struct DlschCheckArgs {
@@ -116,7 +120,7 @@
 hipError_t dlsch_launch_reset(const DlschResetArgs& a, hipStream_t s);
 
 hipError_t dlsch_launch_rm8(const DlschRm8Args& a, hipStream_t s);
-hipError_t dlsch_launch_materialize(int16_t* sb, size_t stride, const uint8_t* fresh, size_t slot0, uint32_t nslots,
-                                    hipStream_t s);
+hipError_t dlsch_launch_materialize(int16_t* sb, size_t stride, const uint8_t* fresh, uint8_t* pside_valid, size_t slot0,
+                                    uint32_t nslots, hipStream_t s);
 
 }
diff --git a/srsran_amd/csrc/dlsch_kernels.hip b/srsran_amd/csrc/dlsch_kernels.hip
--- a/srsran_amd/csrc/dlsch_kernels.hip
+++ b/srsran_amd/csrc/dlsch_kernels.hip
@@ -85,6 +85,7 @@
       bmg[tid]           = nw;
     } else if (tid == 2 * SB_ROWMASK_WORDS) {
       rm_rowmask_of(a.sb + (size_t)d.slot * a.sb_stride)[tid] = K;
+      if (a.pside_valid) a.pside_valid[d.slot] = 0;
     }
 #pragma unroll
     for (int k = 0; k < RM_EQ; k++) {
@@ -324,11 +325,14 @@
   o[j] = (int8_t)v;
   if (a.conv) a.conv[(size_t)d.slot * (a.sb_stride / 2) + j] = (int16_t)(int8_t)v;
   if (j < 2 * SB_ROWMASK_WORDS) ((uint32_t*)(a.sb + (size_t)d.slot * a.sb_stride + 2 * SB_ROWMASK))[j] = 0xffffffffu;
-}
-
-__global__ __launch_bounds__(256) void sb_materialize(int16_t* sb, size_t stride, const uint8_t* fresh, size_t slot0)
+  if (j == 0 && a.pside_valid) a.pside_valid[d.slot] = 0;
+}
+
+__global__ __launch_bounds__(256) void sb_materialize(int16_t* sb, size_t stride, const uint8_t* fresh,
+                                                      uint8_t* pside_valid, size_t slot0)
 {
   const size_t slot = slot0 + blockIdx.x;
+  if (threadIdx.x == 0 && pside_valid) pside_valid[slot] = 0;
   if (fresh[slot]) return;
   int16_t*        b  = sb + slot * stride;
   uint32_t*       bm = rm_rowmask_of(b);
@@ -349,11 +353,11 @@
   if (threadIdx.x < 2 * SB_ROWMASK_WORDS) bm[threadIdx.x] = 0xffffffffu;
 }
 
-hipError_t dlsch_launch_materialize(int16_t* sb, size_t stride, const uint8_t* fresh, size_t slot0, uint32_t nslots,
-                                    hipStream_t s)
+hipError_t dlsch_launch_materialize(int16_t* sb, size_t stride, const uint8_t* fresh, uint8_t* pside_valid, size_t slot0,
+                                    uint32_t nslots, hipStream_t s)
 {
   if (!nslots) return hipSuccess;
-  hipLaunchKernelGGL(sb_materialize, dim3(nslots), dim3(256), 0, s, sb, stride, fresh, slot0);
+  hipLaunchKernelGGL(sb_materialize, dim3(nslots), dim3(256), 0, s, sb, stride, fresh, pside_valid, slot0);
   return hipGetLastError();
 }
 
diff --git a/srsran_amd/csrc/dlsch_runtime.cpp b/srsran_amd/csrc/dlsch_runtime.cpp
--- a/srsran_amd/csrc/dlsch_runtime.cpp
+++ b/srsran_amd/csrc/dlsch_runtime.cpp
@@ -37,6 +37,8 @@
   uint8_t* cb_crc = nullptr;
   uint8_t* data   = nullptr;
   uint8_t* fresh  = nullptr;
+  int16_t* pside       = nullptr;
+  uint8_t* pside_valid = nullptr;
   uint2*     d_list[2]   = {nullptr, nullptr};
   uint32_t   list_cap[2] = {0, 0};
   hipEvent_t ev_list[2]  = {nullptr, nullptr};
@@ -80,7 +82,7 @@
   std::map<uint64_t, uint16_t*>          rm8;
   struct Compact {
     uint16_t* d;
-    uint32_t  nq, qoff;
+    uint32_t  nq, qoff, soff;
   };
   std::map<uint64_t, Compact>            rmc;
   std::map<uint32_t, mi355_tdec8_t*>     dec8;
@@ -165,6 +167,12 @@
 {
   static const bool on = !getenv("MI355_RM_SPARSE") || atoi(getenv("MI355_RM_SPARSE")) != 0;
   return on && !no_rowmask();
+}
+
+bool mi355::pside_enabled()
+{
+  const char* e = getenv("MI355_NO_PSIDE");
+  return !(e && atoi(e) != 0);
 }
 
 static uint32_t rm_buflen(uint32_t K) { return tdec_subblocks(K) ? 3 * (K + 32) + 12 : 3 * K + 12; }
@@ -315,6 +323,13 @@
     mi355_softbuffer_pool_destroy(s);
     return MI355_ERROR;
   }
+  if (rm_sparse_writes()) {
+    if (hipMalloc(&s->pside, nc * SB_PSIDE_STRIDE * 2) != hipSuccess || hipMalloc(&s->pside_valid, nc) != hipSuccess) {
+      mi355_softbuffer_pool_destroy(s);
+      return MI355_ERROR;
+    }
+    (void)hipMemset(s->pside_valid, 0, nc);
+  }
   (void)hipMemset(s->fresh, 1, nc);
   (void)hipMemset(s->cb_crc, 0, nc);
   (void)hipMemset(s->data, 0, nc * SB_DATA);
@@ -330,6 +345,8 @@
   (void)hipFree(p->cb_crc);
   (void)hipFree(p->data);
   (void)hipFree(p->fresh);
+  (void)hipFree(p->pside);
+  (void)hipFree(p->pside_valid);
   for (int k = 0; k < 2; k++) {
     if (p->ev_armed[k]) (void)hipEventSynchronize(p->ev_list[k]);
     if (p->ev_list[k]) (void)hipEventDestroy(p->ev_list[k]);
@@ -427,9 +444,20 @@
 {
   if (!p || first > p->nof_sb || n > p->nof_sb - first) return MI355_ERROR_INVALID_INPUTS;
   CHECK_HIP(hipSetDevice(p->device));
-  CHECK_HIP(dlsch_launch_materialize(p->buf, SB_STRIDE, p->fresh, (size_t)first * p->max_cb, n * p->max_cb,
-                                     (hipStream_t)stream));
+  CHECK_HIP(dlsch_launch_materialize(p->buf, SB_STRIDE, p->fresh, p->pside_valid, (size_t)first * p->max_cb,
+                                     n * p->max_cb, (hipStream_t)stream));
   if (!stream) CHECK_HIP(hipStreamSynchronize(nullptr));
+  return MI355_SUCCESS;
+}
+
+int mi355_softbuffer_pool_pside(mi355_softbuffer_pool_t* p, int16_t** side, uint8_t** valid, uint32_t* stride,
+                                uint32_t* rows)
+{
+  if (!p) return MI355_ERROR_INVALID_INPUTS;
+  if (side) *side = p->pside;
+  if (valid) *valid = p->pside_valid;
+  if (stride) *stride = SB_PSIDE_STRIDE;
+  if (rows) *rows = SB_PSIDE_ROWS;
   return MI355_SUCCESS;
 }
 
@@ -614,7 +642,7 @@
 uint32_t mi355::dlsch_rm_buflen(uint32_t K) { return rm_buflen(K); }
 
 int mi355::dlsch_rm_compact(mi355_dlsch_t* q, uint32_t K, uint32_t rv, uint32_t E, const uint16_t** tab, uint32_t* nq,
-                            uint32_t* qoff)
+                            uint32_t* qoff, uint32_t* soff)
 {
   if (!q || rv > 3 || E == 0 || E > 3 * K + 12) return MI355_ERROR_INVALID_INPUTS;
   std::lock_guard<std::mutex> lock(q->mu);
@@ -638,15 +666,29 @@
     };
     std::vector<uint16_t> rank(nquad, 0xffff);
     std::vector<uint32_t> qlist;
+    std::vector<uint16_t> side;
+    uint32_t              crow[2] = {0, 0};
+    const bool            rows16  = tdec_subblocks(K) == 16;
     for (uint32_t qd = 0; qd < nquad; qd++) {
       if (!defined(8 * qd)) continue;
       uint32_t m = 0;
       for (uint32_t p = 0; p < 8 && 8 * qd + p < buflen; p++) m |= (uint32_t)(inv[8 * qd + p] < E) << p;
       rank[qd] = (uint16_t)qlist.size();
       qlist.push_back(qd | m << 16);
-    }
-    const uint32_t        off = (E + 7) / 8 * 8;
-    std::vector<uint16_t> all(off + 2 * qlist.size() + 8, 0);
+      uint16_t       sd = 0xffff;
+      const uint32_t sl = K + 32, pos = 8 * qd, s = pos / sl;
+      if (rows16 && (s == 1 || s == 2) && (pos - s * sl) / 16 < K / 16) {
+        const uint32_t half = ((pos - s * sl) >> 3) & 1u;
+        sd = (uint16_t)((s - 1) * 2 * SB_PSIDE_ROWS + 2 * crow[s - 1] + half);
+        crow[s - 1] += half;
+      }
+      side.push_back(sd);
+    }
+    const bool side_on = rows16 && crow[0] <= SB_PSIDE_ROWS && crow[1] <= SB_PSIDE_ROWS;
+    const uint32_t        off  = (E + 7) / 8 * 8;
+    const uint32_t        sof  = off + 2 * (uint32_t)qlist.size();
+    std::vector<uint16_t> all(sof + side.size() + 8, 0);
+    memcpy(all.data() + sof, side.data(), side.size() * 2);
     for (uint32_t r = 0; r < E; r++) {
       const uint32_t pos = t[r];
       if (rank[pos / 8] == 0xffff) return MI355_ERROR;
@@ -657,17 +699,18 @@
     CHECK_HIP(hipMalloc(&d, all.size() * 2));
     CHECK_HIP(hipMemcpy(d, all.data(), all.size() * 2, hipMemcpyHostToDevice));
     CHECK_HIP(hipStreamSynchronize(nullptr));
-    it = q->rmc.emplace(key, mi355_dlsch::Compact{d, (uint32_t)qlist.size(), off}).first;
+    it = q->rmc.emplace(key, mi355_dlsch::Compact{d, (uint32_t)qlist.size(), off, side_on ? sof : 0u}).first;
   }
   *tab  = it->second.d;
   *nq   = it->second.nq;
   *qoff = it->second.qoff;
+  if (soff) *soff = it->second.soff;
   return MI355_SUCCESS;
 }
 
 mi355::SoftbufferView mi355::softbuffer_view(mi355_softbuffer_pool_t* p)
 {
-  return SoftbufferView{p->buf, SB_STRIDE, p->cb_crc, p->fresh, p->nof_sb, p->max_cb};
+  return SoftbufferView{p->buf, SB_STRIDE, p->cb_crc, p->fresh, p->nof_sb, p->max_cb, p->pside, p->pside_valid};
 }
 
 int mi355::dlsch_decode_dev_hook(mi355_dlsch_t* q, mi355_softbuffer_pool_t* pool, const void* d_e_bits,
@@ -830,6 +873,7 @@
       ra.sb_crc    = pool->cb_crc;
       ra.fresh     = pool->fresh;
       ra.conv      = nsb8 ? nullptr : pool->buf + SB_CONV8;
+      ra.pside_valid = pool->pside_valid;
       CHECK_HIP(dlsch_launch_rm8(ra, s));
       const uint32_t* sc = nullptr;
       if ((r = crc_scales(q, K, &sc))) return r;
@@ -871,6 +915,7 @@
     ra.sb_crc    = pool->cb_crc;
     ra.fold2     = gi < fold2.size() ? fold2[gi] : 0;
     ra.sparse    = rm_sparse_writes() ? 1 : 0;
+    ra.pside_valid = pool->pside_valid;
     if (!rm_done) CHECK_HIP(dlsch_launch_rm(ra, s));
     auto it = q->dec.find(K);
     if (it == q->dec.end()) {
@@ -930,6 +975,7 @@
         TdecRun rq{llr8 ? pool->buf + SB_CONV8 : pool->buf, SB_STRIDE, d_slot + lv.off, d_done + lv.off, d_run + h, lv.n,
                    lv.K, h, h + 1, lv.dec, lv.K / 8, s, &ca, &fused};
         rq.rowmask = !llr8 && !no_rowmask();
+        if (rq.rowmask && pool->pside && pside_enabled()) rq.pside = pool->pside, rq.pside_valid = pool->pside_valid;
         bool taken = false;
         rq.spec       = spec;
         rq.spec_taken = &taken;
diff --git a/srsran_amd/csrc/pdsch_internal.h b/srsran_amd/csrc/pdsch_internal.h
--- a/srsran_amd/csrc/pdsch_internal.h
+++ b/srsran_amd/csrc/pdsch_internal.h
@@ -68,7 +68,7 @@
   uint32_t  C, Qm, Gp;
   EqRmLayer layer[2];
   const uint16_t* cmp[2][2];
-  uint32_t        cnq[2][2], cqoff[2][2];
+  uint32_t        cnq[2][2], cqoff[2][2], csoff[2][2];
 };
 struct EqRmPool {
   int16_t*       sb;
@@ -78,6 +78,8 @@
   int            sparse;
   int            diag = 0;
   unsigned long long* prof = nullptr;
+  int16_t* pside       = nullptr;
+  uint8_t* pside_valid = nullptr;
 };
 hipError_t pdsch_launch_eq_rm(const PdschJobDev* jobs, const EqRmJob* rj, uint32_t njobs, uint32_t max_c, uint32_t img,
                               uint32_t cimg, const uint32_t* keys, uint32_t nkeys, const EqRmPool& pool, hipStream_t s);
diff --git a/srsran_amd/csrc/pdsch_kernels.hip b/srsran_amd/csrc/pdsch_kernels.hip
--- a/srsran_amd/csrc/pdsch_kernels.hip
+++ b/srsran_amd/csrc/pdsch_kernels.hip
@@ -1132,6 +1132,12 @@
   const GLB uint32_t* map2  = (const GLB uint32_t*)gptr(J.map);
   const uint32_t      pb    = re0 / 2 + tid;
   uint32_t            mnext = pb < p1 ? map2[pb] : 0u;
+  const uint32_t kx0 = c < R.layer[0].C1 ? 0u : 1u, kx1 = c < R.layer[1].C1 ? 0u : 1u;
+  const bool     lean = need[0] && need[1] && fresh[0] && fresh[1] && R.layer[0].inv[kx0] == R.layer[1].inv[kx1] &&
+                    R.layer[0].buflen[kx0] == R.layer[1].buflen[kx1];
+  const uint32_t ev = c > R.C - gamma ? 1u : 0u;
+  const bool     cm = lean && P.sparse && QM0 == QM1 && R.cmp[kx0][ev] != nullptr;
+  const bool     psw = cm && P.pside != nullptr && R.csoff[kx0][ev] != 0u;
   __shared__ uint32_t obm[2][2 * SB_ROWMASK_WORDS], nbm[2][2 * SB_ROWMASK_WORDS];
   if (tid < 2 * (2 * SB_ROWMASK_WORDS + 1)) {
     const uint32_t l = tid / (2 * SB_ROWMASK_WORDS + 1), w = tid % (2 * SB_ROWMASK_WORDS + 1);
@@ -1145,6 +1151,7 @@
         bmg[w]    = nw;
       } else {
         bmg[w] = (R.layer[l].N[kx] - 12) / 3;
+        if (P.pside_valid) P.pside_valid[slot[l]] = psw ? 1 : 0;
       }
     }
   }
@@ -1157,11 +1164,6 @@
     cmb[l]           = cwd[l].csi_enable ? *gptr(cwd[l].cmax_final) : 0u;
   }
   __syncthreads();
-  const uint32_t kx0 = c < R.layer[0].C1 ? 0u : 1u, kx1 = c < R.layer[1].C1 ? 0u : 1u;
-  const bool     lean = need[0] && need[1] && fresh[0] && fresh[1] && R.layer[0].inv[kx0] == R.layer[1].inv[kx1] &&
-                    R.layer[0].buflen[kx0] == R.layer[1].buflen[kx1];
-  const uint32_t ev = c > R.C - gamma ? 1u : 0u;
-  const bool     cm = lean && P.sparse && QM0 == QM1 && R.cmp[kx0][ev] != nullptr;
   const GLB uint16_t* fw  = cm ? gptr(R.cmp[kx0][ev]) : nullptr;
   const uint32_t      cnq = cm ? R.cnq[kx0][ev] : 0u;
   uint32_t* const     im32 = (uint32_t*)imgs;
@@ -1305,13 +1307,20 @@
                                     (GLB uint32_t*)gptr(P.sb + (size_t)slot[1] * P.sb_stride)};
       const bool          al     = (((uintptr_t)sb[0] | (uintptr_t)sb[1]) & 15) == 0;
       typedef uint32_t u4v __attribute__((ext_vector_type(4)));
+      const GLB uint16_t* qs     = fw + R.csoff[kx0][ev];
+      GLB u4v*            ps[2]  = {nullptr, nullptr};
+      if (psw) {
+#pragma unroll
+        for (int l = 0; l < 2; l++) ps[l] = (GLB u4v*)gptr(P.pside + (size_t)slot[l] * SB_PSIDE_STRIDE);
+      }
 #pragma unroll 1
       for (uint32_t q0 = tid; q0 < cnq; q0 += ER_CQ * ER_THREADS) {
-        uint32_t qd[ER_CQ];
+        uint32_t qd[ER_CQ], sd[ER_CQ];
 #pragma unroll
         for (int k = 0; k < ER_CQ; k++) {
           const uint32_t qi = q0 + k * ER_THREADS;
           qd[k]             = qi < cnq ? ql[qi] : 0u;
+          sd[k]             = psw && qi < cnq ? (uint32_t)qs[qi] : 0xffffu;
         }
 #pragma unroll
         for (int k = 0; k < ER_CQ; k++) {
@@ -1335,6 +1344,10 @@
 #pragma unroll
             for (int cc = 0; cc < 4; cc++)
               if (i + cc < npairs) sb[0][i + cc] = a0[cc], sb[1][i + cc] = a1[cc];
+          }
+          if (sd[k] != 0xffffu) {
+            ps[0][sd[k]] = (u4v){v0.x, v0.y, v0.z, v0.w};
+            ps[1][sd[k]] = (u4v){v1.x, v1.y, v1.z, v1.w};
           }
         }
       }
diff --git a/srsran_amd/csrc/pdsch_runtime.cpp b/srsran_amd/csrc/pdsch_runtime.cpp
--- a/srsran_amd/csrc/pdsch_runtime.cpp
+++ b/srsran_amd/csrc/pdsch_runtime.cpp
@@ -744,7 +744,7 @@
   er.max_c = er.img = er.cimg = 0;
   static const bool compact = !getenv("MI355_EQRM_COMPACT") || atoi(getenv("MI355_EQRM_COMPACT")) != 0;
   struct CKey {
-    uint32_t        key = UINT32_MAX, E = 0, nq = 0, qoff = 0;
+    uint32_t        key = UINT32_MAX, E = 0, nq = 0, qoff = 0, soff = 0;
     const uint16_t* tab = nullptr;
   } ck[4];
   uint32_t        seg_tbs = UINT32_MAX, tab_key[2] = {UINT32_MAX, UINT32_MAX};
@@ -803,10 +803,12 @@
             if (!hit) {
               for (int k = 3; k > 0; k--) ck[k] = ck[k - 1];
               hit = &ck[0];
-              if (dlsch_rm_compact(q->dlsch, K, tb.rv, E, &hit->tab, &hit->nq, &hit->qoff)) return false;
+              if (dlsch_rm_compact(q->dlsch, K, tb.rv, E, &hit->tab, &hit->nq, &hit->qoff, &hit->soff))
+                return false;
               hit->key = key, hit->E = E;
             }
             R.cmp[kx][ev] = hit->tab, R.cnq[kx][ev] = hit->nq, R.cqoff[kx][ev] = hit->qoff;
+            R.csoff[kx][ev] = hit->soff;
             cimg          = std::max(cimg, 8 * hit->nq);
           }
         }
@@ -824,6 +826,8 @@
   static const int eqrm_diag = getenv("MI355_EQRM_DIAG") ? atoi(getenv("MI355_EQRM_DIAG")) : 0;
   er.pool.diag = eqrm_diag;
   er.pool.prof = g_eqrm_prof.load();
+  er.pool.pside       = pside_enabled() ? v.pside : nullptr;
+  er.pool.pside_valid = v.pside_valid;
   return er.max_c > 0;
 }
 
diff --git a/srsran_amd/csrc/runtime_internal.h b/srsran_amd/csrc/runtime_internal.h
--- a/srsran_amd/csrc/runtime_internal.h
+++ b/srsran_amd/csrc/runtime_internal.h
@@ -42,14 +42,17 @@
 int      dlsch_rm_inv(mi355_dlsch_t* q, uint32_t K, uint32_t rv, const uint16_t** out);
 uint32_t dlsch_rm_buflen(uint32_t K);
 int      dlsch_rm_compact(mi355_dlsch_t* q, uint32_t K, uint32_t rv, uint32_t E, const uint16_t** tab, uint32_t* nq,
-                          uint32_t* qoff);
+                          uint32_t* qoff, uint32_t* soff);
 bool     rm_sparse_writes();
+bool     pside_enabled();
 struct SoftbufferView {
   int16_t* buf;
   size_t   stride;
   uint8_t* cb_crc;
   uint8_t* fresh;
   uint32_t nof_sb, max_cb;
+  int16_t* pside;
+  uint8_t* pside_valid;
 };
 SoftbufferView softbuffer_view(mi355_softbuffer_pool_t* p);
 
diff --git a/srsran_amd/csrc/tdec_internal.h b/srsran_amd/csrc/tdec_internal.h
--- a/srsran_amd/csrc/tdec_internal.h
+++ b/srsran_amd/csrc/tdec_internal.h
@@ -31,6 +31,8 @@
   int             chk_on;
   int             spec;
   int             rowmask;
+  const int16_t*  pside;
+  const uint8_t*  pside_valid;
 };
 
 struct TdecDecideArgs {
@@ -118,6 +120,8 @@
   bool* spec_taken = nullptr;
   bool  redo       = false;
   bool  rowmask    = false;
+  const int16_t* pside       = nullptr;
+  const uint8_t* pside_valid = nullptr;
 };
 
 hipError_t tdec_win_launch_halfit(int nsb, const TdecWinArgs& a, hipStream_t s);
diff --git a/srsran_amd/csrc/tdec_kernels.hip b/srsran_amd/csrc/tdec_kernels.hip
--- a/srsran_amd/csrc/tdec_kernels.hip
+++ b/srsran_amd/csrc/tdec_kernels.hip
@@ -148,6 +148,7 @@
 #define TDEC_BM_WORDS (8 * 193)
 __shared__ uint32_t tdec_tx_lds[4][2][TDEC_SEG * 64];
 __shared__ uint32_t tdec_ym_lds[4][8 * SB_ROWMASK_WORDS];
+__shared__ uint32_t tdec_yp_lds[4][8 * SB_ROWMASK_WORDS];
 __shared__ uint32_t tdec_bm_lds[4 * TDEC_BM_WORDS];
 __shared__ int16_t  tdec_stg_lds[4][TDEC_SEG * 128];
 __shared__ uint32_t tdec_stg_row[4][TDEC_SEG];
@@ -256,6 +257,27 @@
     __builtin_amdgcn_wave_barrier();
     __builtin_amdgcn_fence(__ATOMIC_ACQUIRE, "wavefront");
   }
+  bool            side   = false;
+  const uint4*    txside = nullptr;
+  uint32_t*       ypre   = nullptr;
+  if constexpr (TX && RMK) {
+    if (a.pside_valid) {
+      side = __builtin_amdgcn_ballot_w64(a.pside_valid[bidx] != 0) == ~0ull;
+      const int txc = grp * G + ((q >> 1) & 7);
+      txside        = (const uint4*)(a.pside + (a.in_idx ? (size_t)a.in_idx[txc] : (size_t)txc) * SB_PSIDE_STRIDE +
+                              (dec2 ? SB_PSIDE_ROWS * 16 : 0)) + (q & 1);
+      ypre          = tdec_yp_lds[threadIdx.x >> 6];
+#pragma unroll
+      for (int w = l; w < SB_ROWMASK_WORDS; w += NL) {
+        uint32_t n = 0;
+        for (int k = 0; k < w; k++) n += (uint32_t)__builtin_popcount(ymask[cbg * SB_ROWMASK_WORDS + k]);
+        ypre[cbg * SB_ROWMASK_WORDS + w] = n;
+      }
+      __builtin_amdgcn_fence(__ATOMIC_RELEASE, "wavefront");
+      __builtin_amdgcn_wave_barrier();
+      __builtin_amdgcn_fence(__ATOMIC_ACQUIRE, "wavefront");
+    }
+  }
   auto yrow = [&](int c, int j) -> bool {
     if constexpr (RMK) {
       return (ymask[c * SB_ROWMASK_WORDS + (j >> 5)] >> (j & 31)) & 1u;
@@ -266,6 +288,24 @@
   auto tx_load = [&](int so, int j0, uint32_t* r, bool par = false) {
     uint4 v0 = make_uint4(0u, 0u, 0u, 0u), v1 = v0;
     const int tc = (q >> 1) & 7, jr = j0 + (q >> 4);
+    if constexpr (TX && RMK) {
+      if (par) {
+        const uint32_t m  = ymask[tc * SB_ROWMASK_WORDS + (jr >> 5)], sh = (uint32_t)jr & 31u;
+        const uint4*   p0 = txin + so + j0 * 2;
+        const uint4*   p1 = txin + so + (j0 + 4) * 2;
+        if (side) {
+          const uint32_t c0 = ypre[tc * SB_ROWMASK_WORDS + (jr >> 5)] + (uint32_t)__builtin_popcount(m & ((1u << sh) - 1u));
+          const uint32_t c1 = c0 + (uint32_t)__builtin_popcount((m >> sh) & 0xfu);
+          p0                = txside + 2 * min(c0, (uint32_t)SB_PSIDE_ROWS - 1u);
+          p1                = txside + 2 * min(c1, (uint32_t)SB_PSIDE_ROWS - 1u);
+        }
+        if ((m >> sh) & 1u) v0 = *p0;
+        if ((m >> (sh + 4)) & 1u) v1 = *p1;
+        r[0] = v0.x; r[1] = v0.y; r[2] = v0.z; r[3] = v0.w;
+        r[4] = v1.x; r[5] = v1.y; r[6] = v1.z; r[7] = v1.w;
+        return;
+      }
+    }
     if (!par || yrow(tc, jr)) v0 = txin[so + j0 * 2];
     if (!par || yrow(tc, jr + 4)) v1 = txin[so + (j0 + 4) * 2];
     r[0] = v0.x; r[1] = v0.y; r[2] = v0.z; r[3] = v0.w;
diff --git a/srsran_amd/csrc/tdec_runtime.cpp b/srsran_amd/csrc/tdec_runtime.cpp
--- a/srsran_amd/csrc/tdec_runtime.cpp
+++ b/srsran_amd/csrc/tdec_runtime.cpp
@@ -299,6 +299,7 @@
         TdecWinArgs wa{d_in, in_stride, rq.in_idx, rq.done, rq.remaining, A1, E, D, CK, t->dstE, t->dstA,
                        (int)n, (int)g.L, (int)g.Lp, (int)g.nseg, (int)h, 0, nullptr, out_stride};
         wa.rowmask = rq.rowmask && g.nsb == 16 && in_stride == SB_STRIDE;
+        if (wa.rowmask && rq.pside_valid) wa.pside = rq.pside, wa.pside_valid = rq.pside_valid;
         CHECK_HIP(tdec_win_launch_halfit(g.nsb, wa, s));
         continue;
       }
@@ -306,6 +307,7 @@
                      (int)n, (int)g.L, (int)g.Lp, (int)g.nseg, (int)h, h + 1 == h1,
                      (fuse && h + 1 == h1) ? d_out : nullptr, out_stride};
       wa.rowmask = rq.rowmask && g.nsb == 16 && in_stride == SB_STRIDE;
+      if (wa.rowmask && rq.pside_valid) wa.pside = rq.pside, wa.pside_valid = rq.pside_valid;
       if (rq.spec && fuse && h + 1 == h1 && tdec_win_spec_ok(g.nsb, g.L)) {
         wa.spec = 1;
         if (rq.spec_taken) *rq.spec_taken = true;
diff --git a/srsran_amd/dlsch.py b/srsran_amd/dlsch.py
--- a/srsran_amd/dlsch.py
+++ b/srsran_amd/dlsch.py
@@ -25,6 +25,7 @@
     L.mi355_softbuffer_reset_cb.argtypes = [vp, u32, u32, vp]
     L.mi355_softbuffer_reset_all.argtypes = [vp, vp]
     L.mi355_softbuffer_pool_materialize.argtypes = [vp, u32, u32, vp]
+    L.mi355_softbuffer_pool_pside.argtypes = [vp, C.POINTER(vp), C.POINTER(vp), C.POINTER(u32), C.POINTER(u32)]
     L.mi355_dlsch_create.argtypes = [C.POINTER(vp), i32]
     L.mi355_dlsch_destroy.argtypes = [vp]
     L.mi355_dlsch_set_max_iterations.argtypes = [vp, u32]
@@ -56,6 +57,21 @@
         n = self.nof_sb - first if n is None else n
         check(self.L.mi355_softbuffer_pool_materialize(self.h, first, n, None), "softbuffer_pool_materialize")
         lib().mi355_device_sync()
+
+    def pside(self):
+        side, valid, stride, rows = C.c_void_p(), C.c_void_p(), C.c_uint32(), C.c_uint32()
+        check(self.L.mi355_softbuffer_pool_pside(self.h, C.byref(side), C.byref(valid), C.byref(stride),
+                                                 C.byref(rows)), "softbuffer_pool_pside")
+        if not side.value or not valid.value:
+            return None, None
+        lib().mi355_device_sync()
+        nslot = self.nof_sb * self.max_cb
+        img = np.zeros((nslot, 2, rows.value, 16), np.int16)
+        assert stride.value == 2 * rows.value * 16
+        val = np.zeros(nslot, np.uint8)
+        check(lib().mi355_memcpy_d2h(img.ctypes.data, side.value, img.nbytes), "mi355_memcpy_d2h")
+        check(lib().mi355_memcpy_d2h(val.ctypes.data, valid.value, val.nbytes), "mi355_memcpy_d2h")
+        return img, val
 
     def close(self):
         if getattr(self, "h", None):
```

After: 125,100 Mbps. No clear change (-0.1%).
